# falcon-computing/bwa-flow

Hardware: AMD Instinct MI355X
Metric: million reads/sec (2×150 bp PE) end-to-end align; SW-extend GCUPS at 1/2/4/8 MI355X (higher is better)
Workload: dtype int32

## Files before the change

### bwa-flow_amd/csrc/capi.hip

```cpp
#include <hip/hip_runtime.h>
#include <string.h>

#include <algorithm>
#include <chrono>
#include <cstdio>
#include <mutex>
#include <new>
#include <string>
#include <thread>
#include <vector>

#include "batch_host.h"
#include "ctx.h"
#include "engine.h"
#include "regpost.h"

using namespace bwagpu;

namespace {


__global__ void side_probe_spin(uint64_t ticks) {
  const uint64_t t0 = __builtin_amdgcn_s_memrealtime();
  while (__builtin_amdgcn_s_memrealtime() - t0 < ticks) __builtin_amdgcn_s_sleep(8);
}
__global__ void side_probe_nop() {}

bool streams_concurrent(hipStream_t a, hipStream_t b) {
  hipEvent_t ea = nullptr, eb = nullptr;
  if (hipEventCreateWithFlags(&ea, hipEventDisableTiming) != hipSuccess) return false;
  if (hipEventCreateWithFlags(&eb, hipEventDisableTiming) != hipSuccess) {
    (void)hipEventDestroy(ea);
    return false;
  }
  hipLaunchKernelGGL(side_probe_spin, dim3(1), dim3(64), 0, a, (uint64_t)15000);
  bool conc = false;
  if (hipGetLastError() == hipSuccess && hipEventRecord(ea, a) == hipSuccess) {
    hipLaunchKernelGGL(side_probe_nop, dim3(1), dim3(64), 0, b);
    if (hipGetLastError() == hipSuccess && hipEventRecord(eb, b) == hipSuccess &&
        hipEventSynchronize(eb) == hipSuccess)
      conc = hipEventQuery(ea) == hipErrorNotReady;
  }
  (void)hipEventSynchronize(ea);
  (void)hipEventDestroy(ea);
  (void)hipEventDestroy(eb);
  return conc;
}

constexpr int kDenseScanBlock = 1024;
__global__ void __launch_bounds__(kDenseScanBlock) dense_scan_kernel(const int32_t* __restrict__ n, int nr,
                                                                     int32_t* __restrict__ off,
                                                                     int32_t* __restrict__ h_off) {
  __shared__ int32_t part[kDenseScanBlock];
  const int t = (int)threadIdx.x;
  const int per = (nr + kDenseScanBlock - 1) / kDenseScanBlock;
  const int r0 = min(t * per, nr), r1 = min(r0 + per, nr);
  int sum = 0;
  for (int r = r0; r < r1; ++r) sum += n[r];
  part[t] = sum;
  __syncthreads();
  for (int d = 1; d < kDenseScanBlock; d <<= 1) {
    const int v = t >= d ? part[t - d] : 0;
    __syncthreads();
    part[t] += v;
    __syncthreads();
  }
  int run = part[t] - sum;
  for (int r = r0; r < r1; ++r) {
    off[r] = run;
    h_off[r] = run;
    run += n[r];
  }
  if (t == kDenseScanBlock - 1) {
    off[nr] = part[t];
    h_off[nr] = part[t];
  }
}

__global__ void __launch_bounds__(256) dense_copy_kernel(const bwagpu_alnreg_t* __restrict__ out,
                                                         const int32_t* __restrict__ n,
                                                         const int32_t* __restrict__ off,
                                                         const int32_t* __restrict__ rco,
                                                         const int32_t* __restrict__ cso, int nr,
                                                         bwagpu_alnreg_t* __restrict__ dense) {
  constexpr int kW = (int)(sizeof(bwagpu_alnreg_t) / 8);
  const int r = (int)((blockIdx.x * 256u + threadIdx.x) >> 4), l = (int)(threadIdx.x & 15);
  if (r >= nr) return;
  const int words = n[r] * kW;
  const uint2* src = reinterpret_cast<const uint2*>(out + cso[rco[r]]);
  uint2* dst = reinterpret_cast<uint2*>(dense + off[r]);
  for (int w = l; w < words; w += 16) dst[w] = src[w];
}

}

namespace {

bool make_opt(const bwagpu_opt_t* o, DevOpt* d, std::string* why) {
  if (!o) { *why = "opt is NULL"; return false; }
  if (o->e_del <= 0 || o->e_ins <= 0) { *why = "gap extension penalties must be > 0"; return false; }
  if (o->w < 0 || o->a < 0) { *why = "negative band width or match score"; return false; }
  if (o->a > 127 || o->e_del > 65535 || o->e_ins > 65535 || o->o_del < 0 || o->o_del > 65535 || o->o_ins < 0 ||
      o->o_ins > 65535 || o->pen_clip5 < 0 || o->pen_clip5 >= (1 << 20) || o->pen_clip3 < 0 ||
      o->pen_clip3 >= (1 << 20) || o->w > (1 << 20)) {
    *why = "scoring option out of range";
    return false;
  }
  memset(d, 0, sizeof(*d));
  d->a = o->a;
  d->o_del = o->o_del;
  d->e_del = o->e_del;
  d->o_ins = o->o_ins;
  d->e_ins = o->e_ins;
  d->oe_del = o->o_del + o->e_del;
  d->oe_ins = o->o_ins + o->e_ins;
  d->pen_clip5 = o->pen_clip5;
  d->pen_clip3 = o->pen_clip3;
  d->w = o->w;
  d->zdrop = o->zdrop;
  int mx = 0;
  for (int i = 0; i < 25; ++i) mx = std::max<int>(mx, o->mat[i]);
  d->max_mat = mx;
  d->row_bound = 1;
  memcpy(d->mat, o->mat, 25);
  for (int q = 0; q < 5; ++q) {
    uint32_t w = 0;
    for (int t = 0; t < 4; ++t) w |= (uint32_t)(uint8_t)o->mat[t * 5 + q] << (8 * t);
    d->qprof[q] = w;
    d->qprof4[q] = o->mat[20 + q];
  }
  return true;
}

int create_common(int device, const bwagpu_opt_t* opt, const bwagpu_bns_t* bns, bwagpu_ctx_t** out,
                  bwagpu_ctx_t** made) {
  if (!out || !bns || bns->l_pac <= 0 || bns->n_seqs <= 0 || !bns->ann_offset || !bns->ann_len)
    return BWAGPU_E_INVAL;
  int n = 0;
  if (hipGetDeviceCount(&n) != hipSuccess || n <= 0) return BWAGPU_E_NODEVICE;
  if (device < 0 || device >= n) return BWAGPU_E_NODEVICE;
  bwagpu_ctx_t* ctx = new (std::nothrow) bwagpu_ctx_t();
  if (!ctx) return BWAGPU_E_NOMEM;
  std::string why;
  if (!make_opt(opt, &ctx->opt, &why)) {
    delete ctx;
    return BWAGPU_E_INVAL;
  }
  ctx->device = device;
  ctx->opt_b = opt->b;
  ctx->ext_form = set_ext_form(-1);
  ctx->ext_short = ext_short_default();
  ctx->ext_short_fill = ext_short_fill_default();
  ctx->light_pack = light_pack_default();
  ctx->ungapped = ungapped_default();
  ctx->emu_finish = emu_finish_default();
  *made = ctx;
  HIPC(hipSetDevice(device), "hipSetDevice");
  HIPC(hipMalloc(&ctx->d_ann_off, sizeof(int64_t) * bns->n_seqs), "hipMalloc(ann_offset)");
  HIPC(hipMalloc(&ctx->d_ann_len, sizeof(int32_t) * bns->n_seqs), "hipMalloc(ann_len)");
  HIPC(hipMemcpy(ctx->d_ann_off, bns->ann_offset, sizeof(int64_t) * bns->n_seqs, hipMemcpyHostToDevice),
       "upload ann_offset");
  HIPC(hipMemcpy(ctx->d_ann_len, bns->ann_len, sizeof(int32_t) * bns->n_seqs, hipMemcpyHostToDevice),
       "upload ann_len");
  for (auto& s : ctx->slot) {
    HIPC(hipEventCreate(&s.ev0), "hipEventCreate");
    HIPC(hipEventCreate(&s.ev1), "hipEventCreate");
    HIPC(hipEventCreate(&s.ev2), "hipEventCreate");
    HIPC(hipEventCreate(&s.ev3), "hipEventCreate");
  }
  ctx->ref.l_pac = bns->l_pac;
  ctx->ref.n_seqs = bns->n_seqs;
  ctx->ref.ann_offset = ctx->d_ann_off;
  ctx->ref.ann_len = ctx->d_ann_len;
  return BWAGPU_OK;
}

std::vector<Slot*> all_slots(bwagpu_ctx_t* ctx) {
  std::vector<Slot*> v;
  for (auto& x : ctx->slot) v.push_back(&x);
  for (auto& x : ctx->dev_scratch) v.push_back(&x);
  v.push_back(&ctx->ch_slot);
  return v;
}

void destroy_ctx(bwagpu_ctx_t* ctx) {
  if (!ctx) return;
  (void)hipSetDevice(ctx->device);
  std::vector<hipStream_t> busy = ctx->side_graveyard;
  for (Slot* s : all_slots(ctx)) busy.insert(busy.end(), {s->stream, s->spec.side});
  busy.insert(busy.end(), ctx->dev_stream, ctx->dev_stream + BWAGPU_NUM_SLOTS);
  busy.insert(busy.end(), ctx->a2_st, ctx->a2_st + bwagpu_ctx::kA2Streams);
  busy.insert(busy.end(), ctx->ch_cs.side, ctx->ch_cs.side + 2);
  for (hipStream_t x : busy)
    if (x) (void)hipStreamSynchronize(x);
  if (ctx->sdh_done) (void)hipEventSynchronize(ctx->sdh_done);
  if (ctx->r2d_done && ctx->r2d_pending) (void)hipEventSynchronize(ctx->r2d_done);
  std::vector<hipStream_t> own = ctx->side_graveyard;
  own.insert(own.end(), ctx->a2_st, ctx->a2_st + bwagpu_ctx::kA2Streams);
  own.insert(own.end(), ctx->ch_cs.side, ctx->ch_cs.side + 2);
  for (hipStream_t x : own)
    if (x) (void)hipStreamDestroy(x);
  std::vector<hipEvent_t> evs = ctx->prof_ev;
  evs.insert(evs.end(), {ctx->sdh_done, ctx->r2d_done, ctx->r2d_ev[0], ctx->r2d_ev[1], ctx->a2_fork, ctx->ch_cs.fork,
                         ctx->ch_cs.join[0], ctx->ch_cs.join[1]});
  evs.insert(evs.end(), ctx->a2_join, ctx->a2_join + bwagpu_ctx::kA2Streams);
  evs.insert(evs.end(), ctx->rs_ev, ctx->rs_ev + 4 * kRescueMaxRounds);
  for (hipEvent_t e : evs)
    if (e) (void)hipEventDestroy(e);
  if (ctx->own_pac && ctx->d_pac) (void)hipFree(ctx->d_pac);
  if (ctx->d_ann_off) (void)hipFree(ctx->d_ann_off);
  if (ctx->d_ann_len) (void)hipFree(ctx->d_ann_len);
  delete ctx;
}

bool use_read_kernels() {
  const char* e = getenv("BWAGPU_C2A_PATH");
  return e && (strcmp(e, "fast") == 0 || strcmp(e, "read") == 0);
}

size_t variant_lds(const DevOpt& o, int v, int lq_max) {
  const Variant& vk = kVariants[v];
  const int lqv = std::min(lq_max, vk.max_len());
  const int tb = tb_bytes_for(o, std::max(lqv, 1));
  return vk.kind == VK_FAST ? (size_t)(kBlock / 64) * fast_wave_lds(tb) : (size_t)tb * (kBlock / vk.G);
}

}

int bwagpu::check_lds(bwagpu_ctx_t* ctx, int lq_max) {
  if (!use_read_kernels()) {
    if (spec_redo_cap(tb_bytes_for(ctx->opt, std::max(lq_max, 1))) < 64)
      return fail(ctx, BWAGPU_E_UNSUPPORTED, "LDS row buffer too large for these options (w, pen_clip, read length)");
    return BWAGPU_OK;
  }
  for (int v = 0; v < kNumVariants; ++v) {
    if (variant_lds(ctx->opt, v, lq_max) > 64 * 1024)
      return fail(ctx, BWAGPU_E_UNSUPPORTED, "LDS row buffer too large for these options (w, pen_clip, read length)");
  }
  return BWAGPU_OK;
}

namespace {

void register_caller_locked(bwagpu_ctx_t* ctx, hipStream_t st) {
  for (hipStream_t c : ctx->callers)
    if (c == st) return;
  for (Slot* x : all_slots(ctx))
    if (x->side_chosen && x->spec.side && hipStreamSynchronize(x->spec.side) == hipSuccess &&
        !streams_concurrent(x->spec.side, st)) {
      ctx->side_graveyard.push_back(x->spec.side);
      x->spec.side = nullptr;
      x->side_chosen = false;
    }
  ctx->callers.push_back(st);
}

hipError_t choose_side(bwagpu_ctx_t* ctx, Slot& s, hipStream_t st, SpecStreams* snap) {
  std::lock_guard<std::mutex> g(ctx->side_mu);
  register_caller_locked(ctx, st);
  if (s.side_chosen) {
    *snap = s.spec;
    return hipSuccess;
  }
  if (!s.spec.fork) {
    hipError_t e = hipEventCreateWithFlags(&s.spec.fork, hipEventDisableTiming);
    if (e == hipSuccess) e = hipEventCreateWithFlags(&s.spec.join, hipEventDisableTiming);
    if (e != hipSuccess) return e;
  }
  std::vector<hipStream_t> avoid = ctx->callers;
  for (Slot* x : all_slots(ctx))
    if (x != &s && x->side_chosen && x->spec.side) avoid.push_back(x->spec.side);
  std::vector<hipStream_t> tried;
  hipStream_t pick = nullptr;
  hipError_t e = hipSuccess;
  for (int t = 0; t < 6 && !pick; ++t) {
    hipStream_t c = nullptr;
    if ((e = hipStreamCreateWithFlags(&c, hipStreamNonBlocking)) != hipSuccess) break;
    bool ok = true;
    for (hipStream_t a : avoid)
      if (!streams_concurrent(c, a)) {
        ok = false;
        break;
      }
    if (ok) pick = c;
    else tried.push_back(c);
  }
  for (hipStream_t c : tried) (void)hipStreamDestroy(c);
  if (e != hipSuccess) return e;
  s.spec.side = pick;
  s.side_chosen = true;
  *snap = s.spec;
  return hipSuccess;
}

int enqueue_spec(bwagpu_ctx_t* ctx, Slot& s, const DevBatch& db, int lq_max, bwagpu_alnreg_t* d_out, int32_t* d_n,
                 int64_t* d_stats, hipStream_t st) {
  const size_t nc = (size_t)std::max(db.n_chains, 1), ns = (size_t)std::max(db.n_seeds, 1),
               nr = (size_t)std::max(db.n_reads, 1);
  const size_t n_tasks = kSpecBins * (nc + (kSpecRounds - 1) * ns);
  SpecArgs a;
  HIPC(s.d_win.get(a.win, nc), "hipMalloc(win)");
  HIPC(s.d_cread.get(a.chain_read, nc), "hipMalloc(chain_read)");
  HIPC(s.d_prog.get(a.prog, ns), "hipMalloc(prog)");
  HIPC(s.d_ext.get(a.ext, ns), "hipMalloc(ext)");
  HIPC(s.d_tasks.get(a.tasks, n_tasks), "hipMalloc(tasks)");
  HIPC(s.d_ctr.get(a.ctr, SPC_WORDS), "hipMalloc(ctr)");
  HIPC(s.d_regpos.get(a.regpos, ns), "hipMalloc(regpos)");
  HIPC(s.d_skipf.get(a.skipf, ns), "hipMalloc(skipf)");
  HIPC(s.d_heavy.get(a.heavy, nr), "hipMalloc(heavy)");
  HIPC(s.d_redo.get(a.redo, nr), "hipMalloc(redo)");
  HIPC(s.d_rbits.get(a.rbits, 2 * (nr / 32 + 1)), "hipMalloc(rbits)");
  a.fbits = a.rbits + (nr / 32 + 1);
  HIPC(s.d_rlist.get(a.rlist, nr), "hipMalloc(rlist)");
  HIPC(s.d_desc.get(a.rdesc, nr), "hipMalloc(desc)");
  HIPC(s.d_schain.get(a.seedchain, ns), "hipMalloc(seedchain)");
  HIPC(s.d_hinfo.get(a.hinfo, nr), "hipMalloc(hinfo)");
  HIPC(s.d_cov.get(a.cov, ns), "hipMalloc(cov)");
  HIPC(s.d_hflag.get(a.hflag, ns), "hipMalloc(hflag)");
  HIPC(s.d_colent.get(a.colent, ns), "hipMalloc(colent)");
  HIPC(s.d_longc.get(a.longc, nc), "hipMalloc(longc)");
  HIPC(s.d_qh.get(a.qh, kQHWords), "hipMalloc(qh)");
  HIPC(s.d_sorth.get(a.sorth, kSortWords), "hipMalloc(sorth)");
  HIPC(s.d_stasks.get(a.stasks, n_tasks), "hipMalloc(stasks)");
  HIPC(s.d_ftask.get(a.ftask, n_tasks), "hipMalloc(ftask)");
  HIPC(s.d_ftaskR.get(a.ftaskR, n_tasks), "hipMalloc(ftaskR)");
  a.ung = nullptr;
  if (ctx->ungapped && ctx->opt.row_bound) HIPC(s.d_ung.get(a.ung, n_tasks), "hipMalloc(ung)");
  HIPC(s.d_mat.get(a.mat, (size_t)std::max<int64_t>(1 << 20, 16 * (int64_t)ns)), "hipMalloc(mat)");
  a.mat_words = (int64_t)(s.d_mat.cap / sizeof(uint64_t));
  static const int ext_prefetch = [] {
    const char* e = getenv("BWAGPU_EXT_PREFETCH");
    return e ? std::max(0, atoi(e)) : 0;
  }();
  a.ext_prefetch = ext_prefetch;
  static const int risky_first = [] {
    const char* e = getenv("BWAGPU_LIGHT_RISKY_FIRST");
    return e && e[0] == '1';
  }();
  a.risky_first = risky_first;
  static const int emu_strict = [] {
    const char* e = getenv("BWAGPU_EMU_STRICT");
    return !(e && e[0] == '0');
  }();
  a.emu_strict = emu_strict;
  a.light_pack = ctx->light_pack;
  a.emu_finish = ctx->emu_finish;
  a.out = d_out;
  a.out_n = d_n;
  a.stats = d_stats;
  SpecStreams ss;
  HIPC(choose_side(ctx, s, st, &ss), "side stream");
  a.lq_bound = lq_max;
  const int tb = tb_bytes_for(ctx->opt, std::max(lq_max, 1));
  ss.form = ctx->ext_form;
  ss.short_q = ctx->ext_short;
  ss.short_fill = ctx->ext_short_fill;
  ss.pool = ctx->prof_ev.empty() ? nullptr : ctx->prof_ev.data();
  ss.pool_n = (int)ctx->prof_ev.size();
  ss.pool_used = &ctx->prof_used;
  HIPC(launch_spec_clear(a, db.n_reads, db.n_seeds, st), "spec clear");
  HIPC(launch_spec_chain2aln(ctx->opt, ctx->ref, db, a, tb, lq_max, st, ss), "spec chain2aln launch");
  return BWAGPU_OK;
}

}

int bwagpu::enqueue_chain2aln(bwagpu_ctx_t* ctx, Slot& s, const DevBatch& db, int lq_max, bwagpu_alnreg_t* d_out,
                              int32_t* d_n, int64_t* d_stats, hipStream_t st) {
  if (!use_read_kernels()) return enqueue_spec(ctx, s, db, lq_max, d_out, d_n, d_stats, st);
  ChainWin* win = nullptr;
  bwagpu_seed_t* prog = nullptr;
  ReadDesc* desc = nullptr;
  C2AArgs a;
  HIPC(s.d_win.get(win, (size_t)db.n_chains), "hipMalloc(win)");
  HIPC(s.d_srt.get(a.srt, (size_t)db.n_seeds), "hipMalloc(srt)");
  HIPC(s.d_prog.get(prog, (size_t)db.n_seeds), "hipMalloc(prog)");
  const size_t nr = (size_t)std::max(db.n_reads, 1);
  HIPC(s.d_desc.get(desc, nr), "hipMalloc(desc)");
  HIPC(s.d_lists.ensure(2 * sizeof(int32_t) * nr), "hipMalloc(lists)");
  int32_t* bins = s.d_lists.as<int32_t>();
  int32_t* read_list = bins + nr;
  HIPC(s.d_counts.get(a.counts, kCountWords), "hipMalloc(counts)");
  HIPC(hipMemsetAsync(a.counts, 0, sizeof(int32_t) * kCountWords, st), "memset counts");
  if (db.n_reads) HIPC(hipMemsetAsync(d_n, 0, sizeof(int32_t) * db.n_reads, st), "memset out_n");
  HIPC(launch_chain_prep(ctx->opt, ctx->ref, db, win, a.srt, prog, d_stats, st), "chain_prep launch");
  HIPC(launch_read_order(db, bins, a.counts + kHistOff, a.counts, desc, read_list, d_stats, st), "read order launch");
  a.read_list = read_list;
  a.desc = desc;
  a.win = win;
  a.prog = prog;
  a.out = d_out;
  a.out_n = d_n;
  a.stats = d_stats;
  for (int v = 0; v < kNumVariants; ++v) {
    const int lqv = std::min(lq_max, kVariants[v].max_len());
    const int tb = tb_bytes_for(ctx->opt, std::max(lqv, 1));
    HIPC(launch_chain2aln(v, ctx->opt, ctx->ref, db, db.n_reads, tb, a, st), "chain2aln launch");
  }
  return BWAGPU_OK;
}

extern "C" {

int bwagpu_abi_version(void) { return BWAGPU_ABI_VERSION; }

int bwagpu_device_count(int* n) {
  if (!n) return BWAGPU_E_INVAL;
  int k = 0;
  if (hipGetDeviceCount(&k) != hipSuccess) k = 0;
  *n = k;
  return k > 0 ? BWAGPU_OK : BWAGPU_E_NODEVICE;
}

int bwagpu_create(int device, const bwagpu_opt_t* opt, const bwagpu_bns_t* bns, const uint8_t* pac_host,
                  bwagpu_ctx_t** out) {
  if (!pac_host) return BWAGPU_E_INVAL;
  bwagpu_ctx_t* ctx = nullptr;
  int rc = create_common(device, opt, bns, out, &ctx);
  if (rc == BWAGPU_OK) {
    const size_t pac_bytes = (size_t)(bns->l_pac / 4 + 1);
    hipError_t e = hipMalloc(&ctx->d_pac, pac_bytes);
    if (e == hipSuccess) {
      ctx->own_pac = true;
      e = hipMemcpy(ctx->d_pac, pac_host, pac_bytes, hipMemcpyHostToDevice);
    }
    if (e != hipSuccess) rc = hip_fail(ctx, e, "pac upload");
    ctx->ref.pac = (const uint8_t*)ctx->d_pac;
  }
  if (rc != BWAGPU_OK) {
    destroy_ctx(ctx);
    return rc;
  }
  *out = ctx;
  return BWAGPU_OK;
}

int bwagpu_create_resident(int device, const bwagpu_opt_t* opt, const bwagpu_bns_t* bns, const void* pac_device,
                           bwagpu_ctx_t** out) {
  if (!pac_device) return BWAGPU_E_INVAL;
  bwagpu_ctx_t* ctx = nullptr;
  int rc = create_common(device, opt, bns, out, &ctx);
  if (rc != BWAGPU_OK) {
    destroy_ctx(ctx);
    return rc;
  }
  ctx->d_pac = (void*)pac_device;
  ctx->own_pac = false;
  ctx->ref.pac = (const uint8_t*)pac_device;
  *out = ctx;
  return BWAGPU_OK;
}

int bwagpu_destroy(bwagpu_ctx_t* ctx) {
  if (!ctx) return BWAGPU_E_INVAL;
  destroy_ctx(ctx);
  return BWAGPU_OK;
}

const char* bwagpu_last_error(const bwagpu_ctx_t* ctx) { return ctx ? ctx->err.c_str() : "NULL context"; }

int bwagpu_set_watchdog_ms(bwagpu_ctx_t* ctx, int ms) {
  if (!ctx || ms < 0) return BWAGPU_E_INVAL;
  ctx->watchdog_ms = ms;
  return BWAGPU_OK;
}

namespace {
void expand_slots(const Slot& s, bwagpu_alnreg_t* dst) {
  const char* h = s.h_in.as<const char>();
  const int32_t* rco = s.kept ? s.keep_rco.data() : (const int32_t*)(h + s.in_rco);
  const int32_t* cso = s.kept ? s.keep_cso.data() : (const int32_t*)(h + s.in_cso);
  const int32_t* n = s.h_n.as<const int32_t>();
  const int32_t* off = s.h_off.as<const int32_t>();
  const bwagpu_alnreg_t* src = s.h_dense.as<const bwagpu_alnreg_t>();
  for (int32_t r = 0; r < s.n_reads; ++r)
    if (n[r]) memcpy(dst + cso[rco[r]], src + off[r], sizeof(bwagpu_alnreg_t) * (size_t)n[r]);
}
}

int bwagpu_chain2aln_submit(bwagpu_ctx_t* ctx, int slot, const bwagpu_batch_t* b) {
// ... 127 lines not shown
  const int64_t* st = s.h_stats.as<int64_t>();
  float k_ms = 0, t_ms = 0;
  (void)hipEventElapsedTime(&k_ms, s.ev1, s.ev2);
  (void)hipEventElapsedTime(&t_ms, s.ev0, s.ev3);
  s.last.kernel_ms = k_ms;
  s.last.total_ms = t_ms;
  s.last.cells = st[ST_CELLS];
  s.last.rows = st[ST_ROWS];
  s.last.ext_calls = st[ST_CALLS];
  const int32_t* off = s.h_off.as<int32_t>();
  s.d2h = (int64_t)sizeof(bwagpu_alnreg_t) * off[s.n_reads] + (int64_t)sizeof(int32_t) * (2 * (int64_t)s.n_reads + 1);
  s.last.h2d_bytes = s.h2d;
  s.last.d2h_bytes = s.d2h;
  if (st[ST_ERR] & ERR_LEN) return fail(ctx, BWAGPU_E_UNSUPPORTED, "read longer than BWAGPU_MAX_READ_LEN");
  if (out_n && s.n_reads) memcpy(out_n, s.h_n.p, sizeof(int32_t) * (size_t)s.n_reads);
  if (out_regs && s.n_seeds) expand_slots(s, out_regs);
  if (st[ST_ERR] & ERR_POST) return fail(ctx, BWAGPU_E_UNSUPPORTED, "a patch candidate's window exceeds 4096 bases");
  if (st[ST_ERR] & ERR_RID)
    return fail(ctx, BWAGPU_E_RESULTS, "a chain's first seed is not inside contig chain_rid (bwamem.c:669 assert)");
  return BWAGPU_OK;
}

int bwagpu_chain2aln_stage(bwagpu_ctx_t* ctx, int slot, int32_t n_reads, int32_t n_chains, int32_t n_seeds,
                           int64_t seq_bytes, bwagpu_batch_t* view) {
  if (!ctx || slot < 0 || slot >= BWAGPU_NUM_SLOTS || !view || n_reads < 0 || n_chains < 0 || n_seeds < 0 ||
      seq_bytes < 0)
    return BWAGPU_E_INVAL;
  Slot& s = ctx->slot[slot];
  if (s.busy) return fail(ctx, BWAGPU_E_INVAL, "slot already has a batch in flight");
  bwagpu_batch_t b{};
  b.n_reads = n_reads;
  b.n_chains = n_chains;
  b.n_seeds = n_seeds;
  b.seq_bytes = seq_bytes;
  InLayout L;
  L.make(b);
  HIPC(hipSetDevice(ctx->device), "hipSetDevice");
  if (s.has_results && !s.slot_view && !s.kept && s.n_reads) {
    const char* hp = s.h_in.as<const char>();
    const int32_t* rco = (const int32_t*)(hp + s.in_rco);
    s.keep_rco.assign(rco, rco + s.n_reads + 1);
    const int32_t* cso = (const int32_t*)(hp + s.in_cso);
    s.keep_cso.assign(cso, cso + s.n_chains + 1);
    s.kept = true;
  }
  HIPC(s.h_in.ensure(L.total), "hipHostMalloc(in)");
  char* h = s.h_in.as<char>();
  b.seq_off = (const int64_t*)(h + L.seq_off);
  b.seq = (const uint8_t*)(h + L.seq);
  b.read_chain_off = (const int32_t*)(h + L.rco);
  b.chain_seed_off = (const int32_t*)(h + L.cso);
  b.chain_rid = (const int32_t*)(h + L.rid);
  b.chain_frac_rep = (const float*)(h + L.frac);
  b.seeds = (const bwagpu_seed_t*)(h + L.seeds);
  *view = b;
  return BWAGPU_OK;
}

int bwagpu_chain2aln_results(bwagpu_ctx_t* ctx, int slot, const bwagpu_alnreg_t** regs, const int32_t** n) {
  if (!ctx || slot < 0 || slot >= BWAGPU_NUM_SLOTS || !regs || !n) return BWAGPU_E_INVAL;
  Slot& s = ctx->slot[slot];
  if (s.busy) return fail(ctx, BWAGPU_E_INVAL, "slot's batch still in flight (wait first)");
  if (!s.has_results) return fail(ctx, BWAGPU_E_INVAL, "slot has no results");
  if (!s.slot_view) {
    bwagpu_alnreg_t* h_out = nullptr;
    HIPC(s.h_out.get(h_out, (size_t)s.n_seeds), "hipHostMalloc(out)");
    if (s.n_seeds) expand_slots(s, h_out);
    s.slot_view = true;
  }
  *regs = s.h_out.as<const bwagpu_alnreg_t>();
  *n = s.h_n.as<const int32_t>();
  return BWAGPU_OK;
}

int bwagpu_chain2aln_results_dense(bwagpu_ctx_t* ctx, int slot, const bwagpu_alnreg_t** regs, const int32_t** n,
                                   const int32_t** off) {
  if (!ctx || slot < 0 || slot >= BWAGPU_NUM_SLOTS || !regs || !n || !off) return BWAGPU_E_INVAL;
  Slot& s = ctx->slot[slot];
  if (s.busy) return fail(ctx, BWAGPU_E_INVAL, "slot's batch still in flight (wait first)");
  if (!s.has_results || !s.h_dense.p || !s.h_off.p) return fail(ctx, BWAGPU_E_INVAL, "slot has no results");
  *regs = s.h_dense.as<const bwagpu_alnreg_t>();
  *n = s.h_n.as<const int32_t>();
  *off = s.h_off.as<const int32_t>();
  return BWAGPU_OK;
}

int bwagpu_chain2aln(bwagpu_ctx_t* ctx, const bwagpu_batch_t* b, bwagpu_alnreg_t* out_regs, int32_t* out_n) {
  int rc = bwagpu_chain2aln_submit(ctx, 0, b);
  if (rc) return rc;
  return bwagpu_chain2aln_wait(ctx, 0, out_regs, out_n);
}

int bwagpu_chain2aln_device(bwagpu_ctx_t* ctx, const bwagpu_batch_t* db_in, bwagpu_alnreg_t* dev_out,
                            int32_t* dev_n, int64_t* dev_stats, void* stream) {
  if (!ctx || !db_in || !dev_out || !dev_n) return BWAGPU_E_INVAL;
  HIPC(hipSetDevice(ctx->device), "hipSetDevice");
  const int lq_bound = use_read_kernels() ? BWAGPU_MAX_READ_LEN : ctx->dev_read_len;
  int rc = check_lds(ctx, lq_bound);
  if (rc) return rc;
  hipStream_t st = (hipStream_t)stream;
  if (!st) HIPC(lazy_stream(ctx->slot[0], &st), "hipStreamCreate");
  int k = 0;
  while (k < BWAGPU_NUM_SLOTS && ctx->dev_stream[k] && ctx->dev_stream[k] != st) ++k;
  if (k == BWAGPU_NUM_SLOTS) return fail(ctx, BWAGPU_E_INVAL, "more than BWAGPU_NUM_SLOTS streams on one context");
  ctx->dev_stream[k] = st;
  Slot& s = ctx->dev_scratch[k];
  DevBatch db;
  db.n_reads = db_in->n_reads;
  db.n_chains = db_in->n_chains;
  db.n_seeds = db_in->n_seeds;
  db.seq_off = db_in->seq_off;
  db.seq = db_in->seq;
  db.read_chain_off = db_in->read_chain_off;
  db.chain_seed_off = db_in->chain_seed_off;
  db.chain_rid = db_in->chain_rid;
  db.chain_frac_rep = db_in->chain_frac_rep;
  db.seeds = db_in->seeds;
  int64_t* stats = dev_stats;
  if (!stats) {
    HIPC(s.d_stats.get(stats, ST_N), "hipMalloc(stats)");
    HIPC(hipMemsetAsync(stats, 0, sizeof(int64_t) * ST_N, st), "memset stats");
  }
  return enqueue_chain2aln(ctx, s, db, lq_bound, dev_out, dev_n, stats, st);
}

int bwagpu_set_device_read_len(bwagpu_ctx_t* ctx, int32_t max_len) {
  if (!ctx || max_len < 1 || max_len > BWAGPU_MAX_READ_LEN) return BWAGPU_E_INVAL;
  ctx->dev_read_len = max_len;
  return BWAGPU_OK;
}

int bwagpu_debug_set_trace(bwagpu_ctx_t* ctx, void* dev_ptr) {
  if (!ctx) return BWAGPU_E_INVAL;
  HIPC(hipSetDevice(ctx->device), "hipSetDevice");
  HIPC(set_trace(dev_ptr), "set trace");
  HIPC(set_trace_spec(dev_ptr), "set trace");
  return BWAGPU_OK;
}

int bwagpu_debug_fail_wait(bwagpu_ctx_t* ctx, int after_n_waits, int code) {
  if (!ctx || code <= 0) return BWAGPU_E_INVAL;
  ctx->fail_after = after_n_waits;
  ctx->fail_code = code;
  return BWAGPU_OK;
}

int bwagpu_debug_live_buffers(int64_t* n, int64_t* bytes) {
  if (!n || !bytes) return BWAGPU_E_INVAL;
  *n = g_live_bufs.load(std::memory_order_relaxed);
  *bytes = g_live_bytes.load(std::memory_order_relaxed);
  return BWAGPU_OK;
}

int bwagpu_debug_occupancy(bwagpu_ctx_t* ctx, void* stream, int64_t* out) {
  if (!ctx || !out) return BWAGPU_E_INVAL;
  hipStream_t st = nullptr;
  if (int rc = entry_stream(ctx, stream, &st)) return rc;
  int k = 0;
  while (k < BWAGPU_NUM_SLOTS && ctx->dev_stream[k] != st) ++k;
  if (k == BWAGPU_NUM_SLOTS || !ctx->dev_scratch[k].d_ctr.p) return fail(ctx, BWAGPU_E_INVAL, "no device-entry batch on this stream");
  HIPC(hipStreamSynchronize(st), "hipStreamSynchronize");
  int32_t c[SPC_WORDS];
  HIPC(hipMemcpy(c, ctx->dev_scratch[k].d_ctr.p, sizeof c, hipMemcpyDeviceToHost), "hipMemcpy(ctr)");
  memcpy(out, c + 32, 14 * sizeof(int64_t));
#ifdef BWAGPU_OCC_DIAG
  return BWAGPU_OK;
#else
  return fail(ctx, BWAGPU_E_UNSUPPORTED, "built without BWAGPU_OCC_DIAG");
#endif
}

int bwagpu_debug_spec_counters(bwagpu_ctx_t* ctx, void* stream, int64_t* out) {
  if (!ctx || !out) return BWAGPU_E_INVAL;
  hipStream_t st = nullptr;
  if (int rc = entry_stream(ctx, stream, &st)) return rc;
  int k = 0;
  while (k < BWAGPU_NUM_SLOTS && ctx->dev_stream[k] != st) ++k;
  if (k == BWAGPU_NUM_SLOTS || !ctx->dev_scratch[k].d_ctr.p) return fail(ctx, BWAGPU_E_INVAL, "no device-entry batch on this stream");
  HIPC(hipStreamSynchronize(st), "hipStreamSynchronize");
  int32_t c[SPC_WORDS];
  HIPC(hipMemcpy(c, ctx->dev_scratch[k].d_ctr.p, sizeof c, hipMemcpyDeviceToHost), "hipMemcpy(ctr)");
  for (int r = 0; r < kSpecRounds; ++r) {
    out[r] = 0;
    for (int b = 0; b < kSpecBins; ++b) out[r] += c[SPC_CNT + r * kSpecBins + b];
  }
  int64_t spec = 0;
  memcpy(&spec, c + SPC_SPEC64, 8);
  out[3] = spec;
  out[4] = c[SPC_MISS];
  out[5] = c[SPC_HEAVY_N];
  out[6] = c[SPC_REDO_N];
  out[7] = c[SPC_HCOLS];
  return BWAGPU_OK;
}

int bwagpu_debug_spec_ext(bwagpu_ctx_t* ctx, void* stream, void* host_out, int32_t n) {
  if (!ctx || !host_out || n < 0) return BWAGPU_E_INVAL;
  hipStream_t st = nullptr;
  if (int rc = entry_stream(ctx, stream, &st)) return rc;
  int k = 0;
  while (k < BWAGPU_NUM_SLOTS && ctx->dev_stream[k] != st) ++k;
  if (k == BWAGPU_NUM_SLOTS || !ctx->dev_scratch[k].d_ext.p || ctx->dev_scratch[k].d_ext.cap < sizeof(SeedExt) * (size_t)n)
    return fail(ctx, BWAGPU_E_INVAL, "no device-entry batch of that size on this stream");
  HIPC(hipStreamSynchronize(st), "hipStreamSynchronize");
  HIPC(hipMemcpy(host_out, ctx->dev_scratch[k].d_ext.p, sizeof(SeedExt) * (size_t)n, hipMemcpyDeviceToHost),
       "hipMemcpy(ext)");
  return BWAGPU_OK;
}

int bwagpu_debug_ext_form(int form) { return set_ext_form(form); }

int bwagpu_streams_concurrent(void* a, void* b) {
  if (!a || !b || a == b) return BWAGPU_E_INVAL;
  return streams_concurrent((hipStream_t)a, (hipStream_t)b) ? 1 : 0;
}

int bwagpu_ctx_ext_form(bwagpu_ctx_t* ctx, int form) {
  if (!ctx) return BWAGPU_E_INVAL;
  const int prev = ctx->ext_form;
  if (form >= 0) ctx->ext_form = form > 2 ? 1 : form;
  return prev;
}

int bwagpu_ctx_ext_short(bwagpu_ctx_t* ctx, int q) {
  if (!ctx) return BWAGPU_E_INVAL;
  const int prev = ctx->ext_short;
  if (q >= 0) ctx->ext_short = q > 63 ? 63 : q;
  return prev;
}

int bwagpu_ctx_ext_short_fill(bwagpu_ctx_t* ctx, int percent) {
  if (!ctx) return BWAGPU_E_INVAL;
  const int prev = ctx->ext_short_fill;
  if (percent >= 0) ctx->ext_short_fill = percent > 100000 ? 100000 : percent;
  return prev;
}

int bwagpu_ctx_light_pack(bwagpu_ctx_t* ctx, int on) {
  if (!ctx) return BWAGPU_E_INVAL;
  const int prev = ctx->light_pack;
  if (on >= 0) ctx->light_pack = on != 0;
  return prev;
}

int bwagpu_debug_spec_short(bwagpu_ctx_t* ctx, void* stream, int64_t* out) {
  if (!ctx || !out) return BWAGPU_E_INVAL;
  hipStream_t st = nullptr;
  if (int rc = entry_stream(ctx, stream, &st)) return rc;
  int k = 0;
  while (k < BWAGPU_NUM_SLOTS && ctx->dev_stream[k] != st) ++k;
  if (k == BWAGPU_NUM_SLOTS || !ctx->dev_scratch[k].d_ctr.p) return fail(ctx, BWAGPU_E_INVAL, "no device-entry batch on this stream");
  HIPC(hipStreamSynchronize(st), "hipStreamSynchronize");
  int32_t c[SPC_WORDS];
  HIPC(hipMemcpy(c, ctx->dev_scratch[k].d_ctr.p, sizeof c, hipMemcpyDeviceToHost), "hipMemcpy(ctr)");
  out[0] = c[SPC_SHORT_N];
  for (int r = 0; r < 2; ++r) {
    const int l = r * kSpecBins;
    out[1 + 4 * r] = c[SPC_LCNT + l];
    out[2 + 4 * r] = c[SPC_LLONG + l];
    out[3 + 4 * r] = c[SPC_RCNT + l];
    out[4 + 4 * r] = c[SPC_RLONG + l];
  }
  return BWAGPU_OK;
}

int bwagpu_ctx_ungapped(bwagpu_ctx_t* ctx, int on) {
  if (!ctx) return BWAGPU_E_INVAL;
  const int prev = ctx->ungapped;
  if (on >= 0) ctx->ungapped = on ? 1 : 0;
  return prev;
}

int bwagpu_debug_spec_ungapped(bwagpu_ctx_t* ctx, void* stream, int64_t* out) {
  if (!ctx || !out) return BWAGPU_E_INVAL;
  hipStream_t st = nullptr;
  if (int rc = entry_stream(ctx, stream, &st)) return rc;
  int k = 0;
  while (k < BWAGPU_NUM_SLOTS && ctx->dev_stream[k] != st) ++k;
  if (k == BWAGPU_NUM_SLOTS || !ctx->dev_scratch[k].d_ctr.p) return fail(ctx, BWAGPU_E_INVAL, "no device-entry batch on this stream");
  HIPC(hipStreamSynchronize(st), "hipStreamSynchronize");
  int32_t c[SPC_WORDS];
  HIPC(hipMemcpy(c, ctx->dev_scratch[k].d_ctr.p, sizeof c, hipMemcpyDeviceToHost), "hipMemcpy(ctr)");
  for (int r = 0; r < kSpecRounds; ++r) {
    out[4 * r + 0] = c[SPC_UNG_N + r];
    out[4 * r + 1] = c[SPC_UNG_Q + r];
    out[4 * r + 2] = out[4 * r + 3] = 0;
    for (int bin = 0; bin < kSpecBins; ++bin) {
      out[4 * r + 2] += c[SPC_LCNT + r * kSpecBins + bin];
      out[4 * r + 3] += c[SPC_RCNT + r * kSpecBins + bin];
    }
  }
  return BWAGPU_OK;
}

int bwagpu_ctx_emu_finish(bwagpu_ctx_t* ctx, int on) {
  if (!ctx) return BWAGPU_E_INVAL;
  const int prev = ctx->emu_finish;
  if (on >= 0) ctx->emu_finish = on ? 1 : 0;
  return prev;
}

int bwagpu_debug_spec_finish(bwagpu_ctx_t* ctx, void* stream, int64_t* out) {
  if (!ctx || !out) return BWAGPU_E_INVAL;
  hipStream_t st = nullptr;
  if (int rc = entry_stream(ctx, stream, &st)) return rc;
  int k = 0;
  while (k < BWAGPU_NUM_SLOTS && ctx->dev_stream[k] != st) ++k;
  if (k == BWAGPU_NUM_SLOTS || !ctx->dev_scratch[k].d_ctr.p) return fail(ctx, BWAGPU_E_INVAL, "no device-entry batch on this stream");
  HIPC(hipStreamSynchronize(st), "hipStreamSynchronize");
  int32_t c[SPC_WORDS];
  HIPC(hipMemcpy(c, ctx->dev_scratch[k].d_ctr.p, sizeof c, hipMemcpyDeviceToHost), "hipMemcpy(ctr)");
  out[0] = c[SPC_FIN_NAR];
  out[1] = c[SPC_FIN_WIDE];
  out[2] = c[SPC_LIST_N];
  out[3] = c[SPC_LIGHT_N];
  return BWAGPU_OK;
}

int bwagpu_ctx_row_bound(bwagpu_ctx_t* ctx, int on) {
  if (!ctx) return BWAGPU_E_INVAL;
  const int prev = ctx->opt.row_bound;
  if (on >= 0) ctx->opt.row_bound = on ? 1 : 0;
  return prev;
}

int bwagpu_debug_ext_kernel(bwagpu_ctx_t* ctx, int32_t lq_max) {
  if (!ctx || lq_max < 1 || lq_max > BWAGPU_MAX_READ_LEN) return BWAGPU_E_INVAL;
  return ext_kernel_for(ctx->opt, ctx->ext_form, tb_bytes_for(ctx->opt, lq_max));
}

int bwagpu_prof_start(bwagpu_ctx_t* ctx, int max_launches) {
  if (!ctx || max_launches < 0) return BWAGPU_E_INVAL;
  HIPC(hipSetDevice(ctx->device), "hipSetDevice");
  for (hipEvent_t e : ctx->prof_ev) HIPC(hipEventSynchronize(e), "hipEventSynchronize");
  for (hipEvent_t e : ctx->prof_ev) (void)hipEventDestroy(e);
  ctx->prof_ev.clear();
  ctx->prof_used = 0;
  for (int i = 0; i < 2 * max_launches; ++i) {
    hipEvent_t e = nullptr;
    HIPC(hipEventCreate(&e), "hipEventCreate");
    ctx->prof_ev.push_back(e);
  }
  return BWAGPU_OK;
}

int bwagpu_prof_read(bwagpu_ctx_t* ctx, double* total_ms, int32_t* launches) {
  if (!ctx || !total_ms || !launches) return BWAGPU_E_INVAL;
  HIPC(hipSetDevice(ctx->device), "hipSetDevice");
  double t = 0;
  for (int i = 0; i + 1 < ctx->prof_used; i += 2) {
    HIPC(hipEventSynchronize(ctx->prof_ev[i + 1]), "hipEventSynchronize");
    float ms = 0;
    HIPC(hipEventElapsedTime(&ms, ctx->prof_ev[i], ctx->prof_ev[i + 1]), "hipEventElapsedTime");
    t += ms;
  }
  *total_ms = t;
  *launches = ctx->prof_used / 2;
  return BWAGPU_OK;
}

int bwagpu_prof_intervals(bwagpu_ctx_t* ctx, double* start_ms, double* end_ms, int32_t max, int32_t* n) {
  if (!ctx || !n || max < 0 || (max && (!start_ms || !end_ms))) return BWAGPU_E_INVAL;
  HIPC(hipSetDevice(ctx->device), "hipSetDevice");
  int k = 0;
  for (int i = 0; i + 1 < ctx->prof_used && k < max; i += 2, ++k) {
    HIPC(hipEventSynchronize(ctx->prof_ev[i + 1]), "hipEventSynchronize");
    float a = 0, b = 0;
    HIPC(hipEventElapsedTime(&a, ctx->prof_ev[0], ctx->prof_ev[i]), "hipEventElapsedTime");
    HIPC(hipEventElapsedTime(&b, ctx->prof_ev[0], ctx->prof_ev[i + 1]), "hipEventElapsedTime");
    start_ms[k] = a;
    end_ms[k] = b;
  }
  *n = k;
  return BWAGPU_OK;
}

int bwagpu_last_stats(const bwagpu_ctx_t* ctx, int slot, bwagpu_stats_t* out) {
  if (!ctx || !out || slot < 0 || slot >= BWAGPU_NUM_SLOTS) return BWAGPU_E_INVAL;
  *out = ctx->slot[slot].last;
  return BWAGPU_OK;
}

}
```

### bwa-flow_amd/csrc/ctx.h

```cpp
#pragma once
#include <hip/hip_runtime.h>
#include <stdint.h>

#include <algorithm>
#include <atomic>
#include <chrono>
#include <mutex>
#include <string>
#include <type_traits>
#include <vector>

#include "bwagpu.h"
#include "chain.h"
#include "engine.h"
#include "rescue.h"
#include "seed.h"
#include "stage_host.h"
#include "task_host.h"

namespace bwagpu {

inline std::atomic<int64_t> g_live_bufs{0}, g_live_bytes{0};

template <bool kPinned>
struct GrowBuf {
  void* p = nullptr;
  size_t cap = 0;
  GrowBuf() = default;
  GrowBuf(const GrowBuf&) = delete;
  GrowBuf& operator=(const GrowBuf&) = delete;
  ~GrowBuf() { release(); }
  hipError_t ensure(size_t n) {
    if (n <= cap) return hipSuccess;
    release();
    const size_t want = std::max<size_t>(n + n / 4, 4096);
    const hipError_t e = kPinned ? hipHostMalloc(&p, want, hipHostMallocDefault) : hipMalloc(&p, want);
    if (e != hipSuccess) {
      p = nullptr;
      return e;
    }
    cap = want;
    g_live_bufs.fetch_add(1, std::memory_order_relaxed);
    g_live_bytes.fetch_add((int64_t)want, std::memory_order_relaxed);
    return e;
  }
  template <class T>
  hipError_t get(T*& out, size_t n) {
    const hipError_t e = ensure(sizeof(T) * std::max<size_t>(n, 1));
    out = e == hipSuccess ? (T*)p : nullptr;
    return e;
  }
  void release() {
    if (p) {
      (void)(kPinned ? hipHostFree(p) : hipFree(p));
      g_live_bufs.fetch_sub(1, std::memory_order_relaxed);
      g_live_bytes.fetch_sub((int64_t)cap, std::memory_order_relaxed);
    }
    p = nullptr;
    cap = 0;
  }
  template <class T>
  T* as() const { return (T*)p; }
};
using DevBuf = GrowBuf<false>;
using HostBuf = GrowBuf<true>;
static_assert(!std::is_copy_constructible<DevBuf>::value, "a copy would free the buffer twice");

struct Slot {
  hipStream_t stream = nullptr;
  std::once_flag stream_once;
  hipError_t stream_err = hipSuccess;
  hipEvent_t ev0 = nullptr, ev1 = nullptr, ev2 = nullptr, ev3 = nullptr;
  DevBuf d_in, d_win, d_srt, d_prog, d_desc, d_out, d_n, d_stats, d_lists, d_counts;
  DevBuf d_cread, d_ext, d_tasks, d_ctr, d_regpos, d_skipf, d_heavy, d_redo, d_rbits, d_rlist;
  DevBuf d_schain, d_hinfo, d_mat, d_cov, d_hflag, d_colent, d_qh, d_longc, d_sorth, d_stasks, d_ftask, d_ftaskR, d_ung;
  SpecStreams spec;
  bool side_chosen = false;
  HostBuf h_in, h_out, h_n, h_stats;
  HostBuf h_dense, h_off;
  DevBuf d_off;
  size_t in_rco = 0, in_cso = 0;
  bool slot_view = false;
  bool busy = false;
  bool has_results = false;
  bool kept = false;
  std::vector<int32_t> keep_rco, keep_cso;
  int32_t n_reads = 0, n_chains = 0, n_seeds = 0;
  std::chrono::steady_clock::time_point t_submit;
  bwagpu_stats_t last{};
  int64_t h2d = 0, d2h = 0;
  ~Slot() {
    for (hipStream_t x : {stream, spec.side})
      if (x) {
        (void)hipStreamSynchronize(x);
        (void)hipStreamDestroy(x);
      }
    for (hipEvent_t e : {ev0, ev1, ev2, ev3, spec.fork, spec.join})
      if (e) (void)hipEventDestroy(e);
  }
};

inline hipError_t lazy_stream(Slot& s, hipStream_t* st) {
  std::call_once(s.stream_once, [&s] { s.stream_err = hipStreamCreateWithFlags(&s.stream, hipStreamNonBlocking); });
  *st = s.stream;
  return s.stream_err;
}

struct Staging {
  DevBuf regs, out_regs;
  DevBuf seq;
  DevBuf seq_off, reg_off, out_off;
  DevBuf n, out_n, n_pri, status, n_sw, mapq, sel;
  DevBuf pes;
};

}

struct bwagpu_ctx {
  using DevBuf = bwagpu::DevBuf;
  using HostBuf = bwagpu::HostBuf;
  using Slot = bwagpu::Slot;
  int device = 0;
  std::mutex side_mu;
  std::vector<hipStream_t> callers, side_graveyard;
  bwagpu::DevOpt opt{};
  bwagpu::DevRef ref{};
  bool own_pac = false;
  void* d_pac = nullptr;
  int64_t* d_ann_off = nullptr;
  int32_t* d_ann_len = nullptr;
  int watchdog_ms = 10000;
  int ext_form = 0;
  int ext_short = 0;
  int light_pack = 0;
  int ext_short_fill = 0;
  int ungapped = 1;
  int emu_finish = 1;
  Slot slot[BWAGPU_NUM_SLOTS];
  hipStream_t dev_stream[BWAGPU_NUM_SLOTS] = {};
  Slot dev_scratch[BWAGPU_NUM_SLOTS];
  DevBuf ex_tasks, ex_list, ex_q, ex_t, ex_res, ex_stats;
  DevBuf a2_tasks, a2_q, a2_t, a2_out, a2_scratch, a2_lists, a2_counts, a2_boff;
  DevBuf r2_tasks, r2_q, r2_out, r2_cig, r2_md, r2_lists, r2_z, r2_stats;
  DevBuf r2d_keys, r2d_lists, r2d_tab, r2d_z, r2d_sums;
  HostBuf r2d_htab;
  hipEvent_t r2d_done = nullptr, r2d_ev[2] = {};
  bool r2d_pending = false, r2d_timing = false, r2d_timed = false;
  double r2d_wait_ms = 0, r2d_call_ms = 0;
  int32_t r2d_jobs = 0;
  static constexpr int kA2Streams = 4;
  hipStream_t a2_st[kA2Streams] = {};
  hipEvent_t a2_fork = nullptr, a2_join[kA2Streams] = {};
  DevBuf bwt_words, sa_d, sa_in, sa_out, occ_d, sup_d, sa_full;
  bwagpu::DevBwt bwt{};
  bool has_bwt = false;
  DevBuf sd_off, sd_seq, sd_out, sd_n, sd_scratch, sd_poff, sd_pack, sd_heavy, sd_dbg;
  DevBuf ch_npos, ch_posoff, ch_frac, ch_nout, ch_noseed, ch_nsw, ch_need, ch_swtab, ch_alt;
  DevBuf ch_kpos, ch_rbeg, ch_qinfo, ch_label, ch_score, ch_slist, ch_ord, ch_chains, ch_nodes;
  DevBuf ch_ochains, ch_oslist, ch_bins, ch_dbg;
  DevBuf ch_swoff, ch_swtasks, ch_swt, ch_swskip, ch_swres, ch_swscr;
  DevBuf ch_ocoff, ch_osoff, ch_rco, ch_cso, ch_rid, ch_cfrac, ch_out, ch_seeds;
  DevBuf ch_regoff, ch_regc;
  HostBuf chh_tot, chh_rco, chh_cso, chh_chains, chh_seeds, chh_regs, chh_n;
  HostBuf sdh_in;
  hipEvent_t sdh_done = nullptr;
  Slot ch_slot;
  bwagpu::ChainStreams ch_cs{};
  bool has_alt = false;
  bwagpu::Staging stg;
  int opt_b = 0;
  bwagpu_postopt_t post_opt{};
  int32_t post_flags = 0;
  int64_t post_id0 = 0;
  DevBuf rp_stats;
  DevBuf pe_isize, pe_cnt;
  DevBuf rs_pair, rs_soff, rs_tab, rs_toff, rs_boff, rs_qpool, rs_ctr, rs_scr;
  DevBuf rs_tasks[bwagpu::kRescueMaxRounds], rs_tpool[bwagpu::kRescueMaxRounds], rs_res[bwagpu::kRescueMaxRounds];
  int32_t rescue_drop = 0;
  hipEvent_t rs_ev[4 * bwagpu::kRescueMaxRounds] = {};
  int rs_ev_rounds = 0;
  hipStream_t rs_ev_stream = nullptr;
  DevBuf ps_scratch, ps_log, ps_erfc;
  bool ps_log_ready = false;
  DevBuf st_buf, st_start, st_q, st_tasks, st_lists, st_seen, st_ctr, st_out;
  int seed_budget = 1024;
  int sup_shift = 32;
  int dev_read_len = BWAGPU_MAX_READ_LEN;
  int fail_after = -1, fail_code = 0;
  std::vector<hipEvent_t> prof_ev;
  int prof_used = 0;
  std::string err;
};

namespace bwagpu {

inline int fail(bwagpu_ctx_t* c, int code, const std::string& msg) {
  if (c) c->err = msg;
  return code;
}

inline int hip_fail(bwagpu_ctx_t* c, hipError_t e, const char* what) {
  std::string m = std::string(what) + ": " + hipGetErrorString(e);
  if (e == hipErrorOutOfMemory || e == hipErrorMemoryAllocation) return fail(c, BWAGPU_E_NOMEM, m);
  return fail(c, BWAGPU_E_DEVICE, m);
}

#define HIPC(call, what)                             \
  do {                                               \
    hipError_t e_ = (call);                          \
    if (e_ != hipSuccess) return hip_fail(ctx, e_, what); \
  } while (0)
#define TRY(call)                     \
  do {                                \
    if (int rc_ = (call)) return rc_; \
  } while (0)

inline int refuse(bwagpu_ctx_t* c, int code, const char* why) { return why && *why ? fail(c, code, why) : code; }

inline int entry_stream(bwagpu_ctx_t* ctx, void* stream, hipStream_t* st) {
  HIPC(hipSetDevice(ctx->device), "hipSetDevice");
  *st = (hipStream_t)stream;
  if (!*st) HIPC(lazy_stream(ctx->slot[0], st), "hipStreamCreate");
  return BWAGPU_OK;
}

inline int side_fork(bwagpu_ctx_t* ctx, hipStream_t st, size_t n_launches, int* used) {
  for (int i = 0; i < bwagpu_ctx::kA2Streams; ++i) {
    if (!ctx->a2_st[i]) HIPC(hipStreamCreateWithFlags(&ctx->a2_st[i], hipStreamNonBlocking), "stream");
    if (!ctx->a2_join[i]) HIPC(hipEventCreateWithFlags(&ctx->a2_join[i], hipEventDisableTiming), "event");
  }
  if (!ctx->a2_fork) HIPC(hipEventCreateWithFlags(&ctx->a2_fork, hipEventDisableTiming), "event");
  *used = (int)std::min<size_t>(bwagpu_ctx::kA2Streams, n_launches);
  HIPC(hipEventRecord(ctx->a2_fork, st), "event");
  for (int i = 0; i < *used; ++i) HIPC(hipStreamWaitEvent(ctx->a2_st[i], ctx->a2_fork, 0), "stream wait");
  return BWAGPU_OK;
}
inline int side_join(bwagpu_ctx_t* ctx, hipStream_t st, int used) {
  for (int i = 0; i < used; ++i) {
    HIPC(hipEventRecord(ctx->a2_join[i], ctx->a2_st[i]), "event");
    HIPC(hipStreamWaitEvent(st, ctx->a2_join[i], 0), "stream wait");
  }
  return BWAGPU_OK;
}

struct EventPair {
  hipEvent_t e0 = nullptr, e1 = nullptr;
  EventPair() = default;
  EventPair(const EventPair&) = delete;
  EventPair& operator=(const EventPair&) = delete;
  ~EventPair() {
    if (e0) (void)hipEventDestroy(e0);
    if (e1) (void)hipEventDestroy(e1);
  }
  hipError_t start(hipStream_t st) {
    hipError_t e = hipEventCreate(&e0);
    if (e == hipSuccess) e = hipEventCreate(&e1);
    return e == hipSuccess ? hipEventRecord(e0, st) : e;
  }
  hipError_t stop(hipStream_t st) { return hipEventRecord(e1, st); }
  float ms() const {
    float t = 0;
    (void)hipEventElapsedTime(&t, e0, e1);
    return t;
  }
};

int enqueue_regpost(bwagpu_ctx_t* ctx, const bwagpu_postopt_t& po, int32_t flags, int64_t id0, int32_t n_reads,
                    const int64_t* seq_off, const uint8_t* seq, const int64_t* reg_off, const int32_t* rco,
                    const int32_t* cso, bwagpu_alnreg_t* regs, int32_t* n, int64_t* stats, hipStream_t st);

int check_lds(bwagpu_ctx_t* ctx, int lq_max);
int enqueue_chain2aln(bwagpu_ctx_t* ctx, Slot& s, const DevBatch& db, int lq_max, bwagpu_alnreg_t* d_out,
                      int32_t* d_n, int64_t* d_stats, hipStream_t st);

struct HostCall {
  bwagpu_ctx_t* ctx;
  Staging& g;
  hipStream_t st = nullptr;
  EventPair ev;
  int64_t h2d = 0, d2h = 0, hs[ST_N] = {};
  std::vector<int64_t> roff, soff, ooff;
  bool open = false;

  explicit HostCall(bwagpu_ctx_t* c) : ctx(c), g(c->stg) {}
  HostCall(const HostCall&) = delete;
  HostCall& operator=(const HostCall&) = delete;
  ~HostCall() {
    if (open) (void)hipStreamSynchronize(st);
  }
// ... 61 lines not shown
```

### bwa-flow_amd/csrc/engine.h

```cpp
#pragma once
#include <hip/hip_runtime.h>
#include <stdint.h>

#include "bwagpu.h"
#include "bwagpu_debug.h"
#include "pure.h"
#include "spec_plan.h"
#include "ungapped.h"

namespace bwagpu {

struct ReadDesc {
  int64_t qoff;
  int32_t rd;
  int32_t lq;
  int32_t c0;
  int32_t nch;
  int32_t s0;
  int32_t ns;
};

struct ChainWin {
  int64_t lo, hi;
};

struct DevBatch {
  int32_t n_reads, n_chains, n_seeds;
  const int64_t* seq_off;
  const uint8_t* seq;
  const int32_t* read_chain_off;
  const int32_t* chain_seed_off;
  const int32_t* chain_rid;
  const float* chain_frac_rep;
  const bwagpu_seed_t* seeds;
};

struct DevRef {
  int64_t l_pac;
  int32_t n_seqs;
  const uint8_t* pac;
  const int64_t* ann_offset;
  const int32_t* ann_len;
};

enum { ST_CELLS = 0, ST_ROWS = 1, ST_CALLS = 2, ST_ERR = 3, ST_N = 4 };
enum { ERR_RID = 1, ERR_LEN = 2, ERR_A2_RANGE = 4 };

constexpr int kFastMaxSeeds = 32;
constexpr int kFastMaxChains = 32;
constexpr int kSeqLds = 256;
constexpr int kNumVariants = 3;
extern const Variant kVariants[kNumVariants];
constexpr int kHistOff = 128;
constexpr int kCountWords = kHistOff + kNumVariants * 256;

hipError_t launch_chain_prep(const DevOpt& o, const DevRef& ref, const DevBatch& b, ChainWin* win, uint64_t* srt,
                             bwagpu_seed_t* prog, int64_t* stats, hipStream_t st);
hipError_t launch_read_order(const DevBatch& b, int32_t* bins, int32_t* hist, int32_t* counts, ReadDesc* desc,
                             int32_t* list, int64_t* stats, hipStream_t st);
struct C2AArgs {
  const int32_t* read_list;
  const ReadDesc* desc;
  int32_t* counts;
  const ChainWin* win;
  uint64_t* srt;
  const bwagpu_seed_t* prog;
  bwagpu_alnreg_t* out;
  int32_t* out_n;
  int64_t* stats;
};
hipError_t launch_chain2aln(int variant, const DevOpt& o, const DevRef& ref, const DevBatch& b, int32_t max_list,
                            int tb_bytes, const C2AArgs& a, hipStream_t st);
size_t fast_wave_lds(int tb);

hipError_t launch_extend(int variant, bool t5, const DevOpt& o, int32_t n_tasks,
                         const bwagpu_ext_task_t* tasks, const int32_t* task_list, int32_t n_list,
                         const uint8_t* qpool, const uint8_t* tpool, int tb_bytes,
                         bwagpu_ext_result_t* res, int64_t* stats, hipStream_t st);
hipError_t launch_extend4(const DevOpt& o, const bwagpu_ext_task_t* tasks, const int32_t* task_list, int32_t n_list,
                          const uint8_t* qpool, const uint8_t* tpool, int tb_bytes, bwagpu_ext_result_t* res,
                          int64_t* stats, hipStream_t st);

struct SeedExt {
  int64_t rb, re;
  int32_t qb, qe, score, truesc, w;
  int32_t cells, rows, calls;
};

constexpr int kSpecRounds = 3;
constexpr int kOrderLane = 8;
constexpr int kSelLight = 64;
constexpr int kSelRegLds = 256;
constexpr int kSelMatMaxSeeds = 4096;
enum {
  SPC_CNT = 0,
  SPC_HEAVY_N = 16,
  SPC_SEL_CUR = 17,
  SPC_REDO_N = 20,
  SPC_SPEC64 = 24,
  SPC_MISS = 26,
  SPC_MATW64 = 28,
  SPC_HCOLS = 30,
  SPC_LONG_N = 31,
  SPC_LCNT = 64,
  SPC_RCNT = 73,
  SPC_LIGHT_CUR = 82,
  SPC_LLONG = 84,
  SPC_RLONG = 93,
  SPC_SHORT_N = 102,
  SPC_UNG_N = 103,
  SPC_UNG_Q = 106,
  SPC_FIN_NAR = 109,
  SPC_FIN_WIDE = 110,
  SPC_LIST_N = 111,
  SPC_LIGHT_N = 112,
  SPC_WORDS = 128
};
constexpr int kQHStride = 32;
constexpr int kQHShort = 2 * kSpecRounds * kSpecBins * 8 * kQHStride;
constexpr int kQHWords = 2 * kQHShort;
constexpr int kSortKeys = 1024;
constexpr int kSortWordsR = kSpecRounds * 2 * kSortKeys;
constexpr int kSortWords = 2 * kSortWordsR;
__host__ __device__ inline size_t spec_list_off(int list, int n_chains, int n_seeds) {
  const int round = list / kSpecBins, bin = list % kSpecBins;
  return round == 0 ? (size_t)bin * n_chains
                    : (size_t)kSpecBins * n_chains + ((size_t)(round - 1) * kSpecBins + bin) * n_seeds;
}
struct FatTask {
  int64_t rbeg, qoff;
  int32_t pos;
  int32_t dlo, dhi;
  uint32_t qls;
};
static_assert(sizeof(FatTask) == 32, "FatTask layout");
static_assert(BWAGPU_MAX_READ_LEN < 1024, "FatTask packs qbeg / len / lq in 10 bits each");
struct UngRec {
  struct Side {
    int32_t ok;
    UngappedSide s;
  } side[2];
};
static_assert(sizeof(UngRec) == 32, "UngRec layout");
struct SpecArgs {
  int lq_bound;
  ChainWin* win;
  int32_t* chain_read;
  bwagpu_seed_t* prog;
  SeedExt* ext;
  int2* tasks;
  int32_t* ctr;
  int32_t* regpos;
  int32_t* skipf;
  int32_t* heavy;
  int32_t* redo;
  uint32_t* rbits;
  uint32_t* fbits;
  int32_t* rlist;
  ReadDesc* rdesc;
  int32_t* seedchain;
  int4* hinfo;
  int32_t* colent;
  int32_t* longc;
  uint64_t* mat;
  int64_t mat_words;
  int32_t* cov;
  int32_t* hflag;
  int32_t* qh;
  int32_t* sorth;
  int2* stasks;
  FatTask* ftask;
  FatTask* ftaskR;
  UngRec* ung;
  int risky_first;
  int emu_strict;
  int light_pack;
  int emu_finish;
  int ext_prefetch;
  bwagpu_alnreg_t* out;
  int32_t* out_n;
  int64_t* stats;
};
struct SpecStreams {
  hipStream_t side = nullptr;
  hipEvent_t fork = nullptr, join = nullptr;
  hipEvent_t* pool = nullptr;
  int pool_n = 0;
  int* pool_used = nullptr;
  int form = 0;
  int short_q = 0;
  int short_fill = 0;
};
int ungapped_default();
int emu_finish_default();
int set_ext_form(int form);
int ext_short_default();
int ext_short_fill_default();
int light_pack_default();
int ext_kernel_for(const DevOpt& o, int form, int tb_bytes);
hipError_t launch_spec_clear(const SpecArgs& a, int n_reads, int n_seeds, hipStream_t st);
hipError_t launch_spec_chain2aln(const DevOpt& o, const DevRef& ref, const DevBatch& b, const SpecArgs& a,
                                 int tb_bytes, int lq_max, hipStream_t st, const SpecStreams& ss);
size_t spec_select_lds(int tb_bytes);
int spec_redo_cap(int tb_bytes);

struct StreamTask {
  bwagpu_seed_t s;
  int64_t lo, hi;
  int64_t qoff;
  int32_t lq, pad_;
};
enum { STR_ERR_RECORD = 1, STR_ERR_TASK = 2, STR_ERR_DUP = 4, STR_ERR_SEED = 8, STR_ERR_BASE = 16 };
enum { kStrDecoded = 4, kStrMax = 5, kStrErr = 6, kStrHeads = 64 };
constexpr int kStrCtrWords = kStrHeads + kSpecBins * 8 * kQHStride;
struct StreamArgs {
  const int32_t* buf;
  const int64_t* rstart;
  int32_t n_reads, cap;
  int64_t l_pac;
  uint8_t* qpool;
  StreamTask* tasks;
  int32_t* lists;
  int32_t* seen;
  int32_t* ctr;
  int32_t* out;
};
hipError_t launch_sw_stream(const DevOpt& o, const DevRef& ref, const StreamArgs& a, int tb_bytes, hipStream_t st);

hipError_t set_trace(void* dev_ptr);
hipError_t set_trace_spec(void* dev_ptr);

}
```

### bwa-flow_amd/csrc/spec.hip

```cpp
#include "spec_dev.h"

namespace bwagpu {

__device__ uint32_t* g_trace = nullptr;
hipError_t set_trace_spec(void* p) { return hipMemcpyToSymbol(HIP_SYMBOL(g_trace), &p, sizeof(p)); }


__global__ void __launch_bounds__(256) spec_chain_kernel(DevOpt o, DevRef ref, DevBatch b, SpecArgs a) {
  sel_prio();
  const int c = blockIdx.x * blockDim.x + threadIdx.x;
  bool task = false, longc = false;
  int bin = 0, s0 = 0;
  if (c < b.n_chains) {
    const int rd = a.chain_read[c];
    s0 = b.chain_seed_off[c];
    const int ns = b.chain_seed_off[c + 1] - s0;
    const int lq = (int)(b.seq_off[rd + 1] - b.seq_off[rd]);
    if (ns <= 0) {
      a.win[c] = ChainWin{0, 0};
    } else {
      int64_t wlo = ref.l_pac << 1, whi = 0;
      longc = ns > kOrderLane;
      if (!longc) {
        uint64_t key[kOrderLane];
// ... 1908 lines not shown
          const uint64_t pw = lane64(pend_w, w);
          const int j = 64 * w + r;
          if ((pw >> r) & 1)
            a.tasks[spec_list_off(list, b.n_chains, b.n_seeds) + off + (int)__popcll(pw & lt_mask)] =
                make_int2(d.s0 + j, a.seedchain[d.s0 + j]);
          off += (int)__popcll(pw);
        }
      }
    } else {
      if (miss >= 0) {
        if (r == 0) {
          const int list = 2 * kSpecBins + spec_bin(d.lq);
          const int p = atomicAdd(&a.ctr[SPC_CNT + list], 1);
          a.tasks[spec_list_off(list, b.n_chains, b.n_seeds) + p] = make_int2(d.s0 + miss, a.seedchain[d.s0 + miss]);
          a.redo[atomicAdd(&a.ctr[SPC_REDO_N], 1)] = rd;
        }
        continue;
      }
      for (int w = 0; w < nw; ++w) {
        const uint64_t ew = (uint64_t)__builtin_amdgcn_readlane((uint32_t)(ext_w >> 32), w) << 32 |
                            (uint32_t)__builtin_amdgcn_readlane((uint32_t)ext_w, w);
        const int j = 64 * w + r;
        if ((ew >> r) & 1) {
          const int slot = nreg + (int)__popcll(ew & lt_mask);
          const SeedExt x = a.ext[d.s0 + j];
          const int c = a.seedchain[d.s0 + j];
          uint2* dst = reinterpret_cast<uint2*>(a.out + d.s0 + slot);
          dst[0] = make_uint2((uint32_t)x.rb, (uint32_t)((uint64_t)x.rb >> 32));
          dst[1] = make_uint2((uint32_t)x.re, (uint32_t)((uint64_t)x.re >> 32));
          dst[2] = make_uint2((uint32_t)x.qb, (uint32_t)x.qe);
          dst[3] = make_uint2((uint32_t)b.chain_rid[c], (uint32_t)x.score);
          dst[4] = make_uint2((uint32_t)x.truesc, 0u);
          dst[5] = make_uint2(0u, 0u);
          dst[6] = make_uint2(0u, (uint32_t)x.w);
          dst[7] = make_uint2((uint32_t)a.cov[d.s0 + j], 0u);
          dst[8] = make_uint2(0u, (uint32_t)a.prog[d.s0 + j].len);
          dst[9] = make_uint2(0u, __float_as_uint(b.chain_frac_rep[c]));
          dst[10] = make_uint2(0u, 0u);
          tl.cells += x.cells;
          tl.rows += x.rows;
          tl.calls += x.calls - 1;
        }
        nreg += (int)__popcll(ew);
      }
      if (r == 0) a.out_n[rd] = nreg;
    }
    trace_read(MODE, b.n_reads, rd, t_start, ns, nreg, 3);
  }
  if constexpr (WRITE) block_stats<64>(tl, a.stats);
}

constexpr int kScanGrid = 1024;

#ifndef BWAGPU_LIGHT_PACK_DEFAULT
#define BWAGPU_LIGHT_PACK_DEFAULT 1
#endif
int light_pack_default() {
  static const int v = [] {
    const char* e = getenv("BWAGPU_LIGHT_PACK");
    return e && e[0] ? (atoi(e) != 0 ? 1 : 0) : BWAGPU_LIGHT_PACK_DEFAULT;
  }();
  return v;
}
#ifndef BWAGPU_LIGHT_PACK_WGS_DEFAULT
#define BWAGPU_LIGHT_PACK_WGS_DEFAULT 2
#endif
static int light_pack_wgs() {
  static const int v = [] {
    const char* e = getenv("BWAGPU_LIGHT_PACK_WGS");
    return std::min(std::max(e && e[0] ? atoi(e) : BWAGPU_LIGHT_PACK_WGS_DEFAULT, 1), 64);
  }();
  return v;
}
#ifndef BWAGPU_LIGHT_LIST_DIV_DEFAULT
#define BWAGPU_LIGHT_LIST_DIV_DEFAULT 4
#endif
static int light_list_div() {
  static const int v = [] {
    const char* e = getenv("BWAGPU_LIGHT_LIST_DIV");
    return std::min(std::max(e && e[0] ? atoi(e) : BWAGPU_LIGHT_LIST_DIV_DEFAULT, 1), 64);
  }();
  return v;
}
static int device_cus() {
  int dev = 0, ncu = 0;
  if (hipGetDevice(&dev) != hipSuccess ||
      hipDeviceGetAttribute(&ncu, hipDeviceAttributeMultiprocessorCount, dev) != hipSuccess || ncu < 1)
    return 256;
  return ncu;
}

template <int MODE>
static void launch_select(const DevOpt& o, const DevRef& ref, const DevBatch& b, const SpecArgs& a, int tb_bytes,
                          hipStream_t st, const SpecStreams& ss) {
  hipStream_t hs = st;
  if (MODE != SEL_REDO && ss.side) {
    (void)hipEventRecord(ss.fork, st);
    (void)hipStreamWaitEvent(ss.side, ss.fork, 0);
    hs = ss.side;
  }
  if (MODE != SEL_REDO) {
    const size_t lds = BWAGPU_LIGHT_INLINE && MODE == SEL_FINAL ? (size_t)(kBlock / 64) * 2 * tb_bytes : 0;
    int nb = resident_blocks(spec_select_light<MODE>, lds);
    if (a.light_pack && !(MODE == SEL_FINAL && a.risky_first)) {
      const int octets = (b.n_reads + kPackW - 1) / kPackW, per_wg = kBlock / 64;
      nb = std::min(nb, std::max(1, std::min((octets + per_wg - 1) / per_wg, light_pack_wgs() * device_cus())));
      if (MODE == SEL_FINAL && a.emu_finish) nb = std::max(1, nb / light_list_div());
    }
    hipLaunchKernelGGL((spec_select_light<MODE>), dim3(nb), dim3(kBlock), lds, st, o, ref, b, a, tb_bytes);
  }
  if (MODE != SEL_REDO) {
    const int nb = resident_blocks(spec_pairs_kernel<MODE>, 0);
    hipLaunchKernelGGL((spec_pairs_kernel<MODE>), dim3(nb), dim3(kBlock), 0, hs, o, b, a);
    hipLaunchKernelGGL((spec_scan_kernel<MODE>), dim3(kScanGrid), dim3(64), (size_t)kScanLds + 2 * (size_t)tb_bytes, hs, o,
                       ref, b, a, tb_bytes);
  }
  hipLaunchKernelGGL((spec_select_kernel<MODE, true>), dim3(MODE == SEL_REDO ? 256 : 1024), dim3(64),
                     (size_t)kSelHeavyLds, hs, o, ref, b, a, tb_bytes);
  if (hs != st) {
    (void)hipEventRecord(ss.join, hs);
    (void)hipStreamWaitEvent(st, ss.join, 0);
  }
}

static std::atomic<int> g_ext_form{0};
int ext_kernel_for(const DevOpt& o, int form, int tb_bytes) { return ext_plan(o, form, tb_bytes, 0).bin[0].code; }
int set_ext_form(int form) {
  const int prev = g_ext_form.load(std::memory_order_relaxed);
  if (form >= 0) g_ext_form.store(form > 2 ? 1 : form, std::memory_order_relaxed);
  return prev;
}

#ifndef BWAGPU_EXT_SHORT_Q_DEFAULT
#define BWAGPU_EXT_SHORT_Q_DEFAULT 63
#endif
int ext_short_default() {
  static const int q = [] {
    const char* e = getenv("BWAGPU_EXT_SHORT_Q");
    const int v = e && e[0] ? atoi(e) : BWAGPU_EXT_SHORT_Q_DEFAULT;
    return std::min(std::max(v, 0), kShortQMax);
  }();
  return q;
}
#ifndef BWAGPU_EXT_SHORT_FILL_DEFAULT
#define BWAGPU_EXT_SHORT_FILL_DEFAULT 150
#endif
int ungapped_default() {
  static const int on = [] {
    const char* e = getenv("BWAGPU_UNGAPPED");
    return !(e && e[0] == '0');
  }();
  return on;
}
int emu_finish_default() {
  static const int on = [] {
    const char* e = getenv("BWAGPU_EMU_FINISH");
    return !(e && e[0] == '0');
  }();
  return on;
}
int ext_short_fill_default() {
  static const int f = [] {
    const char* e = getenv("BWAGPU_EXT_SHORT_FILL");
    return std::min(std::max(e && e[0] ? atoi(e) : BWAGPU_EXT_SHORT_FILL_DEFAULT, 0), 100000);
  }();
  return f;
}


static void launch_sort(const ExtBin& k, const ExtRound& r, int bin0, int nbins, int short_q, int short_fill) {
  if (k.phased) launch_side_sort(r, bin0, nbins, short_q, short_fill);
  else launch_task_sort(r, bin0, nbins);
}
static void launch_ext_bin(const ExtBin& k, const ExtRound& r, int list, const ExtPlan& p, int short_fill) {
  if (k.family == SIDE4) launch_side_bin(k, r, list, p, short_fill);
  else launch_task_bin(k, r, list, p.quad);
}

static void launch_ext_round(const DevOpt& o, const DevRef& ref, const DevBatch& b, const SpecArgs& a, int round,
                             int tb_bytes, int lq_max, hipStream_t st, const SpecStreams& ss) {
  const int l = round * kSpecBins;
  const bool bin1 = lq_max > kSpecBinLen[0], bin2 = lq_max > kSpecBinLen[1];
  const ExtPlan plan = ext_plan(o, ss.form, tb_bytes, ss.short_q);
  const ExtRound r{o, ref, b, a, round, tb_bytes, st};
  if (!bin1 || plan.bin[0].phased == plan.bin[1].phased) {
    launch_sort(plan.bin[0], r, 0, bin1 ? 2 : 1, plan.short_q, ss.short_fill);
  } else {
    launch_sort(plan.bin[0], r, 0, 1, plan.short_q, ss.short_fill);
    launch_sort(plan.bin[1], r, 1, 1, 0, ss.short_fill);
  }
  const bool prof = ss.pool && *ss.pool_used + 2 <= ss.pool_n;
  if (prof) (void)hipEventRecord(ss.pool[*ss.pool_used], st);
  launch_ext_bin(plan.bin[0], r, l + 0, plan, ss.short_fill);
  if (prof) {
    (void)hipEventRecord(ss.pool[*ss.pool_used + 1], st);
    *ss.pool_used += 2;
  }
  if (!bin1) return;
  launch_ext_bin(plan.bin[1], r, l + 1, plan, ss.short_fill);
  if (bin2) launch_task_long(r, l + 2);
}

hipError_t launch_spec_chain2aln(const DevOpt& o, const DevRef& ref, const DevBatch& b, const SpecArgs& a,
                                 int tb_bytes, int lq_max, hipStream_t st, const SpecStreams& ss) {
  if (b.n_reads == 0) return hipSuccess;
  hipLaunchKernelGGL(spec_reads_kernel, dim3((b.n_reads + 255) / 256), dim3(256), 0, st, b, a);
  if (b.n_chains) {
    hipLaunchKernelGGL(spec_chain_kernel, dim3((b.n_chains + 255) / 256), dim3(256), 0, st, o, ref, b, a);
    hipLaunchKernelGGL(spec_order_kernel, dim3(kOrderBlocks), dim3(256), 0, st, o, ref, b, a);
  }
  if (b.n_chains) {
    launch_ext_round(o, ref, b, a, 0, tb_bytes, lq_max, st, ss);
    launch_select<SEL_EMULATE>(o, ref, b, a, tb_bytes, st, ss);
    launch_ext_round(o, ref, b, a, 1, tb_bytes, lq_max, st, ss);
  }
  SpecArgs af = a;
  if (!b.n_chains) af.emu_finish = 0;
  launch_select<SEL_FINAL>(o, ref, b, af, tb_bytes, st, ss);
  if (b.n_chains && lq_max > kSpecBinLen[0] && !a.emu_strict) launch_ext_round(o, ref, b, a, 2, tb_bytes, lq_max, st, ss);
  if (b.n_chains) launch_select<SEL_REDO>(o, ref, b, a, tb_bytes, st, ss);
  return hipGetLastError();
}

__global__ void __launch_bounds__(256) spec_clear_kernel(SpecArgs a, int nr, int ns) {
  const int t0 = (int)(blockIdx.x * 256 + threadIdx.x), nt = (int)(gridDim.x * 256);
  switch (blockIdx.y) {
    case 0:
      for (int i = t0; i < 3 * ns; i += nt) reinterpret_cast<uint4*>(a.ext)[i] = make_uint4(0, 0, 0, 0);
      break;
    case 1:
      for (int i = t0; i < nr; i += nt) a.out_n[i] = 0;
      break;
    case 2:
      for (int i = t0; i < nr / 32 + 1; i += nt) a.rbits[i] = a.fbits[i] = 0;
      break;
    case 3:
      for (int i = t0; i < kQHWords; i += nt) a.qh[i] = 0;
      break;
    case 4:
      for (int i = t0; i < kSortWords; i += nt) a.sorth[i] = 0;
      break;
    default:
      for (int i = t0; i < SPC_WORDS; i += nt) a.ctr[i] = 0;
  }
}
static_assert(sizeof(SeedExt) == 48, "spec_clear_kernel clears SeedExt as three uint4");

hipError_t launch_spec_clear(const SpecArgs& a, int n_reads, int n_seeds, hipStream_t st) {
  hipLaunchKernelGGL(spec_clear_kernel, dim3(256, 6), dim3(256), 0, st, a, n_reads, n_seeds);
  return hipGetLastError();
}

size_t spec_select_lds(int tb_bytes) { return (size_t)kSelHeavyLds + 0 * tb_bytes; }
int spec_redo_cap(int tb_bytes) { return sel_heavy_cap(SEL_REDO, tb_bytes); }

}
```

### bwa-flow_amd/csrc/spec_side.hip

```cpp
#include "spec_dev.h"

namespace bwagpu {

__device__ __forceinline__ int side_key(int qlen) { return 255 - min(qlen, 255); }


struct UngSide {
  const uint8_t* rd;
  int64_t x0;
  int p0, d, qlen, lq;
};
struct UngPass {
  uint64_t qw[2], tw;
  int64_t fa, b0;
  int base, last, ws;
  bool fast, rev;
};
__device__ __forceinline__ UngPass ung_load(const UngSide& s, const DevRef& ref, int base) {
  UngPass p;
  p.base = base;
  p.last = min(base + 15, s.qlen - 1);
  p.fast = false;
  if (base >= s.qlen) return p;
  const int64_t two1 = (ref.l_pac << 1) - 1, pac_bytes = (ref.l_pac >> 2) + 1;
  const int64_t xa = s.x0 + (int64_t)s.d * base, xb = s.x0 + (int64_t)s.d * p.last;
  p.rev = xa >= ref.l_pac;
  p.fa = p.rev ? two1 - xa : xa;
  const int64_t fb = p.rev ? two1 - xb : xb;
  p.fast = s.lq >= 16 && pac_bytes >= 8 && (xb >= ref.l_pac) == p.rev;
  if (p.fast) {
    p.ws = min(max(min(s.p0 + s.d * base, s.p0 + s.d * (base + 15)), 0), s.lq - 16);
    p.b0 = min(min(p.fa, fb) >> 2, pac_bytes - 8);
    __builtin_memcpy(p.qw, s.rd + p.ws, 16);
    __builtin_memcpy(&p.tw, ref.pac + p.b0, 8);
  }
  return p;
}
__device__ __forceinline__ void ung_eat(const UngSide& s, const DevRef& ref, const UngPass& p, const int8_t* mat,
                                        int max_mat, UngappedScan& sc) {
  if (p.base >= s.qlen) return;
  if (p.fast) {
#pragma unroll
    for (int m = 0; m < 16; ++m)
      if (p.base + m <= p.last) {
        const int k = s.p0 + s.d * (p.base + m) - p.ws;
        const int qv = (int)(p.qw[k >> 3] >> ((k & 7) * 8)) & 255;
        const int64_t fm = p.fa + (p.rev ? -s.d : s.d) * m;
        const int byte = (int)(p.tw >> (((fm >> 2) - p.b0) * 8)) & 255;
        const int bse = (byte >> ((~fm & 3) << 1)) & 3;
        sc.step(p.base + m, mat[(p.rev ? 3 - bse : bse) * 5 + min(qv, 4)], max_mat);
      }
  } else {
    for (int j = p.base; j <= p.last; ++j)
      sc.step(j, mat[pac_base2(ref.pac, ref.l_pac, s.x0 + (int64_t)s.d * j) * 5 + min((int)s.rd[s.p0 + s.d * j], 4)],
              max_mat);
  }
}

__global__ void __launch_bounds__(256) spec_ungapped_kernel(DevOpt o, DevRef ref, DevBatch b, SpecArgs a, int round,
                                                            int bin0, int keep_short) {
  sel_prio();
  __shared__ int8_t mat[25];
  if (threadIdx.x < 25) mat[threadIdx.x] = o.mat[threadIdx.x];
  __syncthreads();
  const int bin = bin0 + (int)blockIdx.y;
  const int list = round * kSpecBins + bin;
  const int n = __hip_atomic_load(&a.ctr[SPC_CNT + list], __ATOMIC_RELAXED, __HIP_MEMORY_SCOPE_AGENT);
  const size_t off = spec_list_off(list, b.n_chains, b.n_seeds);
  const int2* tl = a.tasks + off;
  const int oe_min = ungapped_oe_min(o.o_del, o.e_del, o.o_ins, o.e_ins);
  const int keep = bin == 0 ? keep_short : 0;
  const int chunk = (n + (int)gridDim.x - 1) / (int)gridDim.x;
  const int i0 = (int)blockIdx.x * chunk, i1 = min(n, i0 + chunk);
  for (int k = 2 * i0 + (int)threadIdx.x; k < 2 * i1; k += 256) {
    const int i = k >> 1, right = k & 1;
    const FatTask f = fat_task(b, a, tl[i]);
    const int qb = (int)(f.qls & 1023u), ln = (int)((f.qls >> 10) & 1023u), lq = (int)(f.qls >> 20);
    const int64_t xr = f.rbeg + ln;
    const int qlen = right ? lq - qb - ln : qb;
    const int tlen = right ? (int)(f.rbeg + f.dhi - xr) : f.dlo;
    UngRec::Side rec{0, {0, 0, 0}};
    if (qlen > keep && ungapped_band_ok(o.w) &&
        ungapped_call_ok(qlen, tlen, ln * o.a, o.w, o.zdrop, o.max_mat, oe_min)) {
      UngSide sd;
      sd.rd = b.seq + f.qoff;
      sd.p0 = right ? qb + ln : qb - 1;
      sd.d = right ? 1 : -1;
      sd.x0 = right ? xr : f.rbeg - 1;
      sd.qlen = qlen;
      sd.lq = lq;
      UngappedScan sc;
      for (int base = 0; base < qlen && !sc.dead(oe_min); base += 16)
        ung_eat(sd, ref, ung_load(sd, ref, base), mat, o.max_mat, sc);
      if (!sc.dead(oe_min)) rec = UngRec::Side{1, sc.side()};
    }
    a.ung[off + i].side[right] = rec;
  }
}

struct SideLists {
  bool cl, cr, in_l, in_r;
};
__device__ __forceinline__ SideLists side_lists(const SpecArgs& a, size_t slot, int qb, int qr) {
  SideLists s{false, false, qb > 0, qr > 0};
  if (a.ung) {
    s.cl = qb > 0 && a.ung[slot].side[0].ok;
    s.in_l = qb > 0 && !s.cl;
    s.cr = qr > 0 && a.ung[slot].side[1].ok && !s.in_l;
    s.in_r = qr > 0 && !s.cr;
  }
  return s;
}

__device__ __forceinline__ SeedExt settle_sides(const DevOpt& o, const FatTask& f, const UngRec& u, bool right) {
  const int qb = (int)(f.qls & 1023u), ln = (int)((f.qls >> 10) & 1023u), lq = (int)(f.qls >> 20);
  const int qr = lq - qb - ln;
  SeedExt e;
  int calls = 0;
  e.rb = f.rbeg;
  e.qb = 0;
  e.score = e.truesc = ln * o.a;
  if (qb > 0) {
    const UngappedOut x = ungapped_result(ln * o.a, qb, u.side[0].s);
    const bool local = x.gscore <= 0 || x.gscore <= x.score - o.pen_clip5;
    e.rb = f.rbeg - (local ? x.tle : x.gtle);
    e.qb = local ? qb - x.qle : 0;
    e.score = x.score;
    e.truesc = local ? x.score : x.gscore;
    ++calls;
  }
  e.re = f.rbeg + ln;
  e.qe = lq;
  if (right) {
    const int h0 = e.score;
    const UngappedOut x = ungapped_result(h0, qr, u.side[1].s);
    const bool local = x.gscore <= 0 || x.gscore <= x.score - o.pen_clip3;
    e.qe = local ? qb + ln + x.qle : lq;
    e.re = f.rbeg + ln + (local ? x.tle : x.gtle);
    e.score = x.score;
    e.truesc += (local ? x.score : x.gscore) - h0;
    ++calls;
  } else if (qr > 0) {
    e.re = 0;
    e.qe = 0;
  }
  e.w = o.w;
  e.cells = e.rows = 0;
  e.calls = calls + (right || qr == 0 ? 1 : 0);
  return e;
}

__global__ void __launch_bounds__(256) spec_sort2_count(DevBatch b, SpecArgs a, int round, int bin0) {
  sel_prio();
  __shared__ int hist[2][256];
  __shared__ int tot[2];
  const int bin = bin0 + (int)blockIdx.y;
  const int list = round * kSpecBins + bin;
  int32_t* ghL = a.sorth + (round * 2 + bin) * kSortKeys;
  int32_t* ghR = ghL + kSortWordsR;
  for (int k = threadIdx.x; k < 2 * 256; k += 256) hist[k >> 8][k & 255] = 0;
  if (threadIdx.x < 2) tot[threadIdx.x] = 0;
  __syncthreads();
  const int n = __hip_atomic_load(&a.ctr[SPC_CNT + list], __ATOMIC_RELAXED, __HIP_MEMORY_SCOPE_AGENT);
  const size_t off = spec_list_off(list, b.n_chains, b.n_seeds);
  const int2* tl = a.tasks + off;
  const int chunk = (n + (int)gridDim.x - 1) / (int)gridDim.x;
  const int i0 = (int)blockIdx.x * chunk, i1 = min(n, i0 + chunk);
  for (int i = i0 + (int)threadIdx.x; i < i1; i += 256) {
    const FatTask f = fat_task(b, a, tl[i]);
    const int qb = (int)(f.qls & 1023u), ln = (int)((f.qls >> 10) & 1023u), lq = (int)(f.qls >> 20);
    const int qr = lq - qb - ln;
    const SideLists sl = side_lists(a, off + i, qb, qr);
    if (sl.in_l) atomicAdd(&hist[0][side_key(qb)], 1);
    if (sl.in_r) atomicAdd(&hist[1][side_key(qr)], 1);
  }
  __syncthreads();
  for (int k = threadIdx.x; k < 2 * 256; k += 256) {
    const int c = hist[k >> 8][k & 255];
    if (c) {
      atomicAdd((k >> 8) ? &ghR[k & 255] : &ghL[k & 255], c);
      atomicAdd(&tot[k >> 8], c);
    }
  }
  __syncthreads();
  if (threadIdx.x < 2 && tot[threadIdx.x])
    atomicAdd(&a.ctr[(threadIdx.x ? SPC_RCNT : SPC_LCNT) + list], tot[threadIdx.x]);
}

__global__ void __launch_bounds__(256) spec_sort2_scan(SpecArgs a, int round, int bin0, int nbins, int short_q) {
  sel_prio();
  __shared__ int part[256];
  const int bin = bin0 + (int)blockIdx.x % nbins, side = (int)blockIdx.x / nbins;
  int32_t* gh = a.sorth + (round * 2 + bin) * kSortKeys + side * kSortWordsR;
  const int t = (int)threadIdx.x;
  const int v = gh[t];
  part[t] = v;
  __syncthreads();
  for (int o = 1; o < 256; o <<= 1) {
    const int x = t >= o ? part[t - o] : 0;
    __syncthreads();
    part[t] += x;
    __syncthreads();
  }
  gh[t] = part[t] - v;
  if (short_q > 0 && bin == 0 && t == side_key(short_q))
    a.ctr[(side ? SPC_RLONG : SPC_LLONG) + round * kSpecBins + bin] = part[t] - v;
}

__global__ void __launch_bounds__(256) spec_sort2_scatter(DevOpt o, DevBatch b, SpecArgs a, int round, int bin0) {
  sel_prio();
  __shared__ int cnt[2][256];
  __shared__ int ung[2];
  const int bin = bin0 + (int)blockIdx.y;
  const int list = round * kSpecBins + bin;
  int32_t* ghL = a.sorth + (round * 2 + bin) * kSortKeys;
  int32_t* ghR = ghL + kSortWordsR;
  for (int k = threadIdx.x; k < 2 * 256; k += 256) cnt[k >> 8][k & 255] = 0;
  if (threadIdx.x < 2) ung[threadIdx.x] = 0;
  __syncthreads();
  const int n = __hip_atomic_load(&a.ctr[SPC_CNT + list], __ATOMIC_RELAXED, __HIP_MEMORY_SCOPE_AGENT);
  const size_t off = spec_list_off(list, b.n_chains, b.n_seeds);
  const int2* tl = a.tasks + off;
  FatTask* foL = a.ftask + off;
  FatTask* foR = a.ftaskR + off;
  const int chunk = (n + (int)gridDim.x - 1) / (int)gridDim.x;
  const int i0 = (int)blockIdx.x * chunk, i1 = min(n, i0 + chunk);
  constexpr int kPer = 8;
  int kl[kPer], kr[kPer], rl[kPer], rr[kPer];
  FatTask ft[kPer];
  for (int base = i0; base < i1; base += 256 * kPer) {
#pragma unroll
    for (int m = 0; m < kPer; ++m) {
      const int i = base + m * 256 + (int)threadIdx.x;
      kl[m] = kr[m] = -1;
      if (i < i1) {
        ft[m] = fat_task(b, a, tl[i]);
        const int qb = (int)(ft[m].qls & 1023u), ln = (int)((ft[m].qls >> 10) & 1023u), lq = (int)(ft[m].qls >> 20);
        const int qr = lq - qb - ln;
        const SideLists sl = side_lists(a, off + i, qb, qr);
        if (sl.in_l) {
          kl[m] = side_key(qb);
          rl[m] = atomicAdd(&cnt[0][kl[m]], 1);
        }
        if (sl.in_r) {
          kr[m] = side_key(qr);
          rr[m] = atomicAdd(&cnt[1][kr[m]], 1);
        }
        if (!sl.in_l) {
          if (qb > 0 || !sl.in_r)
            a.ext[ft[m].pos] = settle_sides(o, ft[m], sl.cl || sl.cr ? a.ung[off + i] : UngRec{}, sl.cr);
          if (sl.cl || sl.cr) {
            atomicAdd(&ung[0], (sl.cl ? 1 : 0) + (sl.cr ? 1 : 0));
            atomicAdd(&ung[1], (sl.cl ? qb : 0) + (sl.cr ? qr : 0));
          }
        }
      }
    }
    __syncthreads();
    for (int k = threadIdx.x; k < 2 * 256; k += 256) {
      const int c = cnt[k >> 8][k & 255];
      cnt[k >> 8][k & 255] = c ? atomicAdd((k >> 8) ? &ghR[k & 255] : &ghL[k & 255], c) : 0;
    }
    __syncthreads();
#pragma unroll
    for (int m = 0; m < kPer; ++m) {
      if (kl[m] >= 0) foL[cnt[0][kl[m]] + rl[m]] = ft[m];
      if (kr[m] >= 0) foR[cnt[1][kr[m]] + rr[m]] = ft[m];
    }
    __syncthreads();
    for (int k = threadIdx.x; k < 2 * 256; k += 256) cnt[k >> 8][k & 255] = 0;
    __syncthreads();
  }
  if (threadIdx.x < 2 && ung[threadIdx.x])
    atomicAdd(&a.ctr[(threadIdx.x ? SPC_UNG_Q : SPC_UNG_N) + round], ung[threadIdx.x]);
}

struct SideTask {
  int64_t rbeg, qoff, rb;
  int32_t pos, dlo, dhi, qbeg, len, lq;
  int32_t tt, score, h0, truesc, qb, aw0, cells, rows, calls, pad_;
};
static_assert(sizeof(SideTask) <= 96, "SideTask layout");
typedef __attribute__((address_space(3))) SideTask LdsS;
#define SIDE_FIELDS(X) X(rbeg) X(qoff) X(rb) X(pos) X(dlo) X(dhi) X(qbeg) X(len) X(lq) X(tt) X(score) X(h0) \
  X(truesc) X(qb) X(aw0) X(cells) X(rows) X(calls)
__device__ __forceinline__ void spark(LdsS* p, const SideTask& t) {
#define X(f) p->f = t.f;
  SIDE_FIELDS(X)
#undef X
  asm volatile("" ::: "memory");
}
__device__ __forceinline__ SideTask sload(LdsS* p) {
  asm volatile("" ::: "memory");
  SideTask t;
#define X(f) t.f = p->f;
  SIDE_FIELDS(X)
#undef X
  return t;
}
#undef SIDE_FIELDS

template <int G, bool RIGHT>
__device__ __forceinline__ void side_start(SideTask& t, const DevOpt& o, const DevRef& ref, const SpecArgs& a,
                                           const FatTask& f, uint8_t* tb) {
  t.rbeg = f.rbeg;
  t.qoff = f.qoff;
  t.pos = f.pos;
  t.dlo = f.dlo;
  t.dhi = f.dhi;
  t.qbeg = (int)(f.qls & 1023u);
  t.len = (int)((f.qls >> 10) & 1023u);
  t.lq = (int)(f.qls >> 20);
  t.tt = 0;
  const int64_t pac_bytes = (ref.l_pac >> 2) + 1;
  const int r = (int)(threadIdx.x & (G - 1));
  if constexpr (!RIGHT) {
    const int n = rows_needed(o, t.qbeg, t.dlo, o.w << 1, o.pen_clip5);
    const int R = (n + G - 1) / G;
    if (R <= 32) fill_side_run<G>(tb, t.rbeg - 1, -1, r * R, min(r * R + R, n), ref, pac_bytes);
    else fill_two_half<G>(tb, t.rbeg - 1, n, tb, 0, 0, ref);
    t.score = -1;
    t.h0 = t.len * o.a;
    t.truesc = -1;
    t.qb = 0;
    t.rb = t.rbeg;
    t.aw0 = o.w;
    t.cells = t.rows = t.calls = 0;
  } else {
    const int64_t x0 = t.rbeg + t.len;
    const int qr = t.lq - t.qbeg - t.len;
    const int n = rows_needed(o, qr, (int)(t.rbeg + t.dhi - x0), o.w << 1, o.pen_clip3);
    const int R = (n + G - 1) / G;
    if (R <= 32) fill_side_run<G>(tb, x0, 1, r * R, min(r * R + R, n), ref, pac_bytes);
    else fill_two_half<G>(tb, 0, 0, tb, x0, n, ref);
    if (t.qbeg > 0) {
      const SeedExt e = a.ext[t.pos];
      t.score = e.score;
      t.truesc = e.truesc;
      t.qb = e.qb;
      t.rb = e.rb;
      t.aw0 = e.w;
      t.cells = e.cells;
      t.rows = e.rows;
      t.calls = e.calls;
    } else {
      t.score = t.truesc = t.len * o.a;
      t.qb = 0;
      t.rb = t.rbeg;
      t.aw0 = o.w;
      t.cells = t.rows = t.calls = 0;
    }
    t.h0 = t.score;
  }
  __builtin_amdgcn_fence(__ATOMIC_RELEASE, "wavefront");
  __builtin_amdgcn_wave_barrier();
  __builtin_amdgcn_fence(__ATOMIC_ACQUIRE, "wavefront");
}

template <bool RIGHT>
__device__ __forceinline__ QCall side_call(const SideTask& t, const DevOpt& o, const uint8_t* seq, const uint8_t* tb) {
  QCall q;
  if constexpr (!RIGHT) {
    q.qlen = t.qbeg;
    q.tlen = t.dlo;
    q.qa = t.qbeg - 1;
    q.qd = -1;
    q.eb = o.pen_clip5;
  } else {
    const int64_t x0 = t.rbeg + t.len;
    q.qlen = t.lq - t.qbeg - t.len;
    q.tlen = (int)(t.rbeg + t.dhi - x0);
    q.qa = t.qbeg + t.len;
    q.qd = 1;
    q.eb = o.pen_clip3;
  }
  q.h0 = t.h0;
  q.w = o.w << t.tt;
  q.zdrop = o.zdrop;
  q.q = seq + t.qoff;
  q.tb = tb;
  q.tlen = rows_needed(o, q.qlen, q.tlen, q.w, q.eb);
  return q;
}

template <int G, bool RIGHT>
__device__ __forceinline__ bool side_advance(SideTask& t, const DevOpt& o, const SpecArgs& a, const ExtOut& x,
                                             const Tally32& tl, long long& spec_cells) {
  t.cells += tl.cells;
  t.rows += tl.rows;
  t.calls += tl.calls;
  const int prev = t.score;
  t.score = x.score;
  const int aw = o.w << t.tt;
  if (t.tt == 0 && !(x.score == prev || x.max_off < (aw >> 1) + (aw >> 2))) {
    t.tt = 1;
    return false;
  }
  const int eb = RIGHT ? o.pen_clip3 : o.pen_clip5;
  const bool local = x.gscore <= 0 || x.gscore <= x.score - eb;
  SeedExt e;
  if constexpr (!RIGHT) {
    const int qr = t.lq - t.qbeg - t.len;
    e.rb = t.rbeg - (local ? x.tle : x.gtle);
    e.qb = local ? t.qbeg - x.qle : 0;
    e.score = t.score;
    e.truesc = local ? x.score : x.gscore;
    if (qr != 0) {
      e.re = 0;
      e.qe = 0;
      e.w = aw;
      e.cells = t.cells;
      e.rows = t.rows;
      e.calls = t.calls;
    } else {
      e.re = t.rbeg + t.len;
      e.qe = t.lq;
      e.w = max(aw, o.w);
      e.cells = t.cells;
      e.rows = t.rows;
      e.calls = t.calls + 1;
      spec_cells += t.cells;
    }
  } else {
    e.rb = t.rb;
    e.qb = t.qb;
    e.qe = local ? t.qbeg + t.len + x.qle : t.lq;
    e.re = t.rbeg + t.len + (local ? x.tle : x.gtle);
// ... 32 lines not shown
  constexpr int QB = PMAX * G;
  uint8_t* const ta_ = wlds + (size_t)((threadIdx.x & 63) / G) * (2 * (size_t)tb_bytes + 2 * kSideLds + 2 * QB);
  uint8_t* const tb_ = ta_ + tb_bytes;
  LdsS* const sa = (LdsS*)(tb_ + tb_bytes);
  LdsS* const sb = (LdsS*)(tb_ + tb_bytes + kSideLds);
  uint8_t* const qa_ = tb_ + tb_bytes + 2 * kSideLds;
  uint8_t* const qb_ = qa_ + QB;
  ShardQ qq;
  qq.init(heads, n);
  bool ha = false, hb = false, more = n > 0;
  int started = 0;
  for (;;) {
#ifdef BWAGPU_OCC_DIAG
    const unsigned long long c0 = __builtin_amdgcn_s_memtime();
#endif
    if (more) {
      const uint64_t na = __builtin_amdgcn_ballot_w64(!ha) & kLead, nb = __builtin_amdgcn_ballot_w64(!hb) & kLead;
      const int nn = __popcll(na) + __popcll(nb);
      if (nn > 0) {
        int m0, cap;
        if (qq.claim(nn, m0, cap)) {
          const int ia = m0 + __popcll(na & below) + __popcll(nb & below), ib = ia + (ha ? 0 : 1);
          if (!ha && ia < cap) {
            SideTask t;
            const FatTask f = fl[qq.shard + 8 * ia];
            side_query<G, RIGHT>(b, f, qa_, QB);
            side_start<G, RIGHT>(t, o, ref, a, f, ta_);
            spark(sa, t);
            ha = true;
            ++started;
          }
          if (!hb && ib < cap) {
            SideTask t;
            const FatTask f = fl[qq.shard + 8 * ib];
            side_query<G, RIGHT>(b, f, qb_, QB);
            side_start<G, RIGHT>(t, o, ref, a, f, tb_);
            spark(sb, t);
            hb = true;
            ++started;
          }
        } else {
          more = false;
        }
      }
    }
#ifdef BWAGPU_OCC_DIAG
    const unsigned long long c1 = __builtin_amdgcn_s_memtime();
    tw[0] += c1 - c0;
#endif
    if (!__builtin_amdgcn_ballot_w64(ha || hb)) {
      if (!more) break;
      continue;
    }
    QCall ca = quad_idle(qa_, ta_), cb = quad_idle(qb_, tb_);
    if (ha) {
      ca = side_call<RIGHT>(sload(sa), o, b.seq, ta_);
      ca.q = qa_;
      ca.qa = 0;
      ca.qd = 1;
    }
    if (hb) {
      cb = side_call<RIGHT>(sload(sb), o, b.seq, tb_);
      cb.q = qb_;
      cb.qa = 0;
      cb.qd = 1;
    }
    ExtOut xa, xb;
    Tally32 tla{0, 0, 0}, tlb{0, 0, 0};
#ifdef BWAGPU_OCC_DIAG
    const unsigned long long c2 = __builtin_amdgcn_s_memtime();
    tw[1] += c2 - c1;
#endif
    extend_quad_dispatch<G, PMAX, K8>(o, ca, cb, xa, xb, tla, tlb);
#ifdef BWAGPU_OCC_DIAG
    const unsigned long long c3 = __builtin_amdgcn_s_memtime();
    tw[2] += c3 - c2;
    occ_diag<G>(occ, ca, cb, tla, tlb);
#endif
    if (ha) {
      SideTask t = sload(sa);
      if (side_advance<G, RIGHT>(t, o, a, xa, tla, spec_cells)) ha = false;
      else spark(sa, t);
    }
    if (hb) {
      SideTask t = sload(sb);
      if (side_advance<G, RIGHT>(t, o, a, xb, tlb, spec_cells)) hb = false;
      else spark(sb, t);
    }
#ifdef BWAGPU_OCC_DIAG
    tw[3] += __builtin_amdgcn_s_memtime() - c3;
#endif
  }
  return started;
}

template <int G, int PMAX, bool K8, bool RIGHT>
__global__ void __launch_bounds__(kBlock) spec_side4_kernel(DevOpt o, DevRef ref, DevBatch b, SpecArgs a, int list,
                                                            int tb_bytes, int wave_lds, int short_q, int tb_short,
                                                            int short_fill) {
  extern __shared__ __attribute__((aligned(16))) uint8_t lds[];
  uint8_t* const wlds = lds + (size_t)(threadIdx.x >> 6) * (size_t)wave_lds;
  const int n = uni(__hip_atomic_load(&a.ctr[(RIGHT ? SPC_RCNT : SPC_LCNT) + list], __ATOMIC_RELAXED,
                                      __HIP_MEMORY_SCOPE_AGENT));
  const FatTask* fl = (RIGHT ? a.ftaskR : a.ftask) + spec_list_off(list, b.n_chains, b.n_seeds);
  constexpr bool kShort = G == 16 && K8;
  int n_long = n;
  if constexpr (kShort) {
    if (short_q > 0) {
      n_long = min(n, uni(__hip_atomic_load(&a.ctr[(RIGHT ? SPC_RLONG : SPC_LLONG) + list], __ATOMIC_RELAXED,
                                            __HIP_MEMORY_SCOPE_AGENT)));
      const long long slots = (long long)gridDim.x * (kBlock / 64) * (128 / kShortG);
      if ((long long)(n - n_long) * 100 < slots * short_fill) n_long = n;
    }
  }
  const int hl = RIGHT ? kSpecRounds * kSpecBins + list : list;
  long long spec_cells = 0;
#ifdef BWAGPU_OCC_DIAG
  unsigned long long tw[6] = {0, 0, 0, 0, 0, 0}, occ[8] = {0, 0, 0, 0, 0, 0, 0, 0};
  (void)side_loop<G, PMAX, K8, RIGHT>(o, ref, b, a, fl, n_long, a.qh + 8 * kQHStride * hl, wlds, tb_bytes, spec_cells,
                                      tw, occ);
#else
  (void)side_loop<G, PMAX, K8, RIGHT>(o, ref, b, a, fl, n_long, a.qh + 8 * kQHStride * hl, wlds, tb_bytes, spec_cells);
#endif
  if constexpr (kShort) {
    if (n_long < n) {
      int32_t* const hs = a.qh + kQHShort + 8 * kQHStride * hl;
      long long cells_s = 0;
#ifdef BWAGPU_OCC_DIAG
      const int ns = side_loop<kShortG, kShortPmax, true, RIGHT>(o, ref, b, a, fl + n_long, n - n_long, hs, wlds,
                                                                 tb_short, cells_s, tw, occ);
#else
      const int ns = side_loop<kShortG, kShortPmax, true, RIGHT>(o, ref, b, a, fl + n_long, n - n_long, hs, wlds,
                                                                 tb_short, cells_s);
#endif
      if ((threadIdx.x & (kShortG - 1)) == 0 && ns) {
        atomicAdd(&a.ctr[SPC_SHORT_N], ns);
        atomicAdd(reinterpret_cast<unsigned long long*>(a.ctr + SPC_SPEC64), (unsigned long long)cells_s);
      }
    }
  }
#ifdef BWAGPU_OCC_DIAG
  if ((threadIdx.x & 63) == 0) {
    for (int k = 0; k < 8; ++k) atomicAdd(reinterpret_cast<unsigned long long*>(a.ctr + 32) + k, occ[k]);
    for (int k = 0; k < 4; ++k) atomicAdd(reinterpret_cast<unsigned long long*>(a.ctr + 48) + k, tw[k]);
  }
#endif
  if ((threadIdx.x & (G - 1)) == 0 && spec_cells)
    atomicAdd(reinterpret_cast<unsigned long long*>(a.ctr + SPC_SPEC64), (unsigned long long)spec_cells);
}


void launch_side_sort(const ExtRound& r, int bin0, int nbins, int short_q, int short_fill) {
  if (r.a.ung)
    hipLaunchKernelGGL(spec_ungapped_kernel, dim3(1024, nbins), dim3(256), 0, r.st, r.o, r.ref, r.b, r.a, r.round, bin0,
                       short_fill == 0 ? short_q : 0);
  hipLaunchKernelGGL(spec_sort2_count, dim3(256, nbins), dim3(256), 0, r.st, r.b, r.a, r.round, bin0);
  hipLaunchKernelGGL(spec_sort2_scan, dim3(2 * nbins), dim3(256), 0, r.st, r.a, r.round, bin0, nbins, short_q);
  hipLaunchKernelGGL(spec_sort2_scatter, dim3(256, nbins), dim3(256), 0, r.st, r.o, r.b, r.a, r.round, bin0);
}

template <int G, int PMAX, bool K8>
static void launch_side_pair(const ExtRound& r, int list, const ExtPlan& p, int short_fill) {
  const size_t lds = (size_t)(kBlock / 64) * p.wave_lds;
  const int nb = resident_blocks(spec_side4_kernel<G, PMAX, K8, false>, lds);
  const int gr = r.round == 2 ? std::min(nb, 64) : std::min(nb, ext2_grid(1 << 30, true));
  if (!(G == 16 && K8)) short_fill = 0;
  hipLaunchKernelGGL((spec_side4_kernel<G, PMAX, K8, false>), dim3(gr), dim3(kBlock), lds, r.st, r.o, r.ref, r.b, r.a,
                     list, r.tb_bytes, (int)p.wave_lds, p.short_q, p.tb_short, short_fill);
  hipLaunchKernelGGL((spec_side4_kernel<G, PMAX, K8, true>), dim3(gr), dim3(kBlock), lds, r.st, r.o, r.ref, r.b, r.a,
                     list, r.tb_bytes, (int)p.wave_lds, p.short_q, p.tb_short, short_fill);
}

void launch_side_bin(const ExtBin& k, const ExtRound& r, int list, const ExtPlan& p, int short_fill) {
  switch (ext_key(k.family, k.G, k.PMAX, k.K8)) {
    case ext_key(SIDE4, 16, 10, true): return launch_side_pair<16, 10, true>(r, list, p, short_fill);
    case ext_key(SIDE4, 32, 5, true): return launch_side_pair<32, 5, true>(r, list, p, short_fill);
    case ext_key(SIDE4, 32, 8, false): return launch_side_pair<32, 8, false>(r, list, p, short_fill);
    default: abort();
  }
}

}
```

### bwa-flow_amd/csrc/ungapped.h

```cpp
#pragma once
#include <stdint.h>

#ifdef __HIPCC__
#define BWAGPU_UNG_HD __host__ __device__
#else
#define BWAGPU_UNG_HD
#endif

namespace bwagpu {

struct UngappedSide {
  int32_t M;
  int32_t am;
  int32_t cl;
};

struct UngappedOut {
  int32_t score, qle, tle, gtle, gscore, max_off;
};

BWAGPU_UNG_HD inline int ungapped_oe_min(int o_del, int e_del, int o_ins, int e_ins) {
  const int d = o_del + e_del, i = o_ins + e_ins;
  return d < i ? d : i;
}

BWAGPU_UNG_HD inline bool ungapped_call_ok(int qlen, int tlen, int h0, int w, int zdrop, int max_mat, int oe_min) {
  return qlen >= 1 && tlen >= qlen && max_mat >= 1 && oe_min >= 1 && h0 >= oe_min && w >= 0 &&
         (zdrop <= 0 || zdrop >= oe_min);
}
BWAGPU_UNG_HD inline bool ungapped_band_ok(int w) { return (w >> 1) + (w >> 2) > 0; }

struct UngappedScan {
  int c = 0, P = 0, M = 0, am = 0;
  BWAGPU_UNG_HD void step(int i, int s, int max_mat) {
    P += max_mat - s;
    c += s;
    if (c > M) {
      M = c;
      am = i + 1;
    }
  }
  BWAGPU_UNG_HD bool dead(int oe_min) const { return P >= oe_min; }
  BWAGPU_UNG_HD UngappedSide side() const { return UngappedSide{M, am, c}; }
};

template <class Score>
BWAGPU_UNG_HD inline bool ungapped_scan(int qlen, int max_mat, int oe_min, Score score, UngappedSide* u) {
  UngappedScan sc;
  for (int i = 0; i < qlen; ++i) {
    sc.step(i, score(i), max_mat);
    if (sc.dead(oe_min)) return false;
  }
  *u = sc.side();
  return true;
}

BWAGPU_UNG_HD inline UngappedOut ungapped_result(int h0, int qlen, const UngappedSide& u) {
  UngappedOut x;
  x.score = h0 + u.M;
  x.qle = x.tle = u.am;
  x.gscore = h0 + u.cl;
  x.gtle = qlen;
  x.max_off = 0;
  return x;
}

}
```

### bwa-flow_amd/python/bwagpu/abi.py

```python
from __future__ import annotations

import ctypes as C
import os

import numpy as np

HERE = os.path.dirname(os.path.abspath(__file__))
PKG_ROOT = os.path.normpath(os.path.join(HERE, "..", ".."))
REPO_ROOT = os.path.normpath(os.path.join(PKG_ROOT, ".."))
LIB_DIR = os.path.join(PKG_ROOT, "lib")

ABI_VERSION = 1
OK, E_INVAL, E_NOMEM, E_DEVICE, E_HANG, E_RESULTS, E_UNSUPPORTED, E_NODEVICE = range(8)
ERR_NAMES = {
    OK: "OK", E_INVAL: "E_INVAL", E_NOMEM: "E_NOMEM", E_DEVICE: "E_DEVICE", E_HANG: "E_HANG",
    E_RESULTS: "E_RESULTS", E_UNSUPPORTED: "E_UNSUPPORTED", E_NODEVICE: "E_NODEVICE",
}
MAX_READ_LEN = 1023
NUM_SLOTS = 4

SEED_DTYPE = np.dtype([("rbeg", "<i8"), ("qbeg", "<i4"), ("len", "<i4"), ("score", "<i4"),
                       ("pad", "<i4")])
ALNREG_DTYPE = np.dtype([
    ("rb", "<i8"), ("re", "<i8"), ("qb", "<i4"), ("qe", "<i4"), ("rid", "<i4"), ("score", "<i4"),
# ... 35 lines not shown
class BatchC(C.Structure):
    _fields_ = [("n_reads", C.c_int32), ("n_chains", C.c_int32), ("n_seeds", C.c_int32),
                ("pad_", C.c_int32), ("seq_bytes", C.c_int64), ("seq_off", C.c_void_p),
                ("seq", C.c_void_p), ("read_chain_off", C.c_void_p), ("chain_seed_off", C.c_void_p),
                ("chain_rid", C.c_void_p), ("chain_frac_rep", C.c_void_p), ("seeds", C.c_void_p)]


class Stats(C.Structure):
    _fields_ = [("kernel_ms", C.c_double), ("total_ms", C.c_double), ("cells", C.c_int64),
                ("rows", C.c_int64), ("ext_calls", C.c_int64), ("h2d_bytes", C.c_int64),
                ("d2h_bytes", C.c_int64)]


class BwtC(C.Structure):
    _fields_ = [("primary", C.c_uint64), ("L2", C.c_uint64 * 5), ("seq_len", C.c_uint64),
                ("bwt_size", C.c_uint64), ("bwt", C.c_void_p), ("sa_intv", C.c_int32), ("pad_", C.c_int32),
                ("n_sa", C.c_uint64), ("sa", C.c_void_p)]


class SeedOpt(C.Structure):
    _fields_ = [("min_seed_len", C.c_int32), ("split_width", C.c_int32), ("max_mem_intv", C.c_int32),
                ("split_factor", C.c_float)]


INTV_DTYPE = np.dtype([("x", "<u8", (3,)), ("info", "<u8")])
assert INTV_DTYPE.itemsize == 32

CHAIN_DTYPE = np.dtype([("pos", "<i8"), ("rid", "<i4"), ("n", "<i4"), ("w", "<i4"), ("kept", "<i4"),
                        ("first", "<i4"), ("is_alt", "<i4"), ("frac_rep", "<f4"), ("pad_", "<i4")])
assert CHAIN_DTYPE.itemsize == 40


class ChainOpt(C.Structure):
    _fields_ = [("max_occ", C.c_int32), ("max_chain_gap", C.c_int32), ("min_chain_weight", C.c_int32),
                ("max_chain_extend", C.c_int32), ("mask_level", C.c_float), ("drop_ratio", C.c_float)]


class ChainsC(C.Structure):
    _fields_ = [("n_reads", C.c_int32), ("n_chains", C.c_int32), ("n_seeds", C.c_int64),
                ("read_chain_off", C.c_void_p), ("chain_seed_off", C.c_void_p), ("chains", C.c_void_p),
                ("seeds", C.c_void_p)]


class PostOpt(C.Structure):
    _fields_ = [("max_chain_gap", C.c_int32), ("mask_level_redun", C.c_float), ("mask_level", C.c_float),
                ("pad_", C.c_int32)]


POST_DEDUP_PATCH, POST_MARK_ALT, POST_PRIMARY = 1, 2, 4


def default_postopt() -> PostOpt:
    return PostOpt(10000, 0.95, 0.50, 0)


class PairOpt(C.Structure):
    _fields_ = [("max_ins", C.c_int32), ("max_matesw", C.c_int32), ("pen_unpaired", C.c_int32),
                ("min_seed_len", C.c_int32), ("max_chain_gap", C.c_int32), ("mask_level_redun", C.c_float),
                ("mask_level", C.c_float), ("max_rounds", C.c_int32)]


def default_pairopt() -> PairOpt:
    return PairOpt(10000, 50, 17, 19, 10000, 0.95, 0.50, 3)


PESTAT_DTYPE = np.dtype([("low", "<i4"), ("high", "<i4"), ("failed", "<i4"), ("pad", "<i4"), ("avg", "<f8"),
                         ("std", "<f8")])
assert PESTAT_DTYPE.itemsize == 32 and C.sizeof(PairOpt) == 32
RESCUE_DONE, RESCUE_UNFINISHED, RESCUE_OVERFLOW, RESCUE_UNSUPPORTED = 0, 1, 2, 3


class SelOpt(C.Structure):
    _fields_ = [("T", C.c_int32), ("pen_unpaired", C.c_int32), ("min_seed_len", C.c_int32),
                ("mapQ_coef_len", C.c_float), ("mapQ_coef_fac", C.c_int32), ("mask_level", C.c_float),
                ("drop_ratio", C.c_float), ("flags", C.c_int32)]


def default_selopt(flags: int = 0) -> SelOpt:
    return SelOpt(30, 17, 19, 50.0, 3, 0.50, 0.50, int(flags))


MEM_F_NOPAIRING, MEM_F_ALL, MEM_F_NO_MULTI, MEM_F_PRIMARY5, MEM_F_KEEP_SUPP_MAPQ = 0x4, 0x8, 0x10, 0x800, 0x1000
SEL_MAX_REGS = 512
SEL_DONE, SEL_TOO_MANY, SEL_SKIPPED = 0, 1, 2
SEL_NO_PAIRING, SEL_PAIRED = 0, 1
PAIRSEL_DTYPE = np.dtype([("status", "<i4"), ("branch", "<i4"), ("n_pri", "<i4", (2,)), ("z", "<i4", (2,)),
                          ("mapq", "<i4", (2,)), ("alt", "<i4", (2,)), ("extra_flag", "<i4"), ("o", "<i4"),
                          ("subo", "<i4"), ("n_sub", "<i4"), ("pad", "<i4", (2,))])
assert PAIRSEL_DTYPE.itemsize == 64 and C.sizeof(SelOpt) == 32


class SamOpt(C.Structure):
    _fields_ = [("flags", C.c_int32), ("XA_drop_ratio", C.c_float), ("max_XA_hits", C.c_int32),
                ("max_XA_hits_alt", C.c_int32)]


def default_samopt(flags: int = 0) -> SamOpt:
    return SamOpt(int(flags), 0.80, 5, 200)


def default_chainopt() -> dict:
    return dict(max_occ=500, max_chain_gap=10000, min_chain_weight=0, max_chain_extend=1 << 30, mask_level=0.5,
                drop_ratio=0.5)

_VP = C.c_void_p
PROTOS = {
    "bwagpu_abi_version": (C.c_int, []),
    "bwagpu_device_count": (C.c_int, [C.POINTER(C.c_int)]),
    "bwagpu_create": (C.c_int, [C.c_int, C.POINTER(Opt), C.POINTER(Bns), _VP, C.POINTER(_VP)]),
    "bwagpu_create_resident": (C.c_int, [C.c_int, C.POINTER(Opt), C.POINTER(Bns), _VP, C.POINTER(_VP)]),
    "bwagpu_destroy": (C.c_int, [_VP]),
    "bwagpu_last_error": (C.c_char_p, [_VP]),
    "bwagpu_set_watchdog_ms": (C.c_int, [_VP, C.c_int]),
    "bwagpu_chain2aln_submit": (C.c_int, [_VP, C.c_int, C.POINTER(BatchC)]),
    "bwagpu_chain2aln_wait": (C.c_int, [_VP, C.c_int, _VP, _VP]),
    "bwagpu_chain2aln_stage": (C.c_int, [_VP, C.c_int, C.c_int32, C.c_int32, C.c_int32, C.c_int64,
                                         C.POINTER(BatchC)]),
    "bwagpu_chain2aln_results": (C.c_int, [_VP, C.c_int, C.POINTER(_VP), C.POINTER(_VP)]),
    "bwagpu_chain2aln_results_dense": (C.c_int, [_VP, C.c_int, C.POINTER(_VP), C.POINTER(_VP), C.POINTER(_VP)]),
    "bwagpu_chain2aln": (C.c_int, [_VP, C.POINTER(BatchC), _VP, _VP]),
    "bwagpu_chain2aln_device": (C.c_int, [_VP, C.POINTER(BatchC), _VP, _VP, _VP, _VP]),
    "bwagpu_extend_batch": (C.c_int, [_VP, C.c_int32, _VP, _VP, C.c_int64, _VP, C.c_int64, _VP]),
    "bwagpu_align2_batch": (C.c_int, [_VP, C.c_int32, _VP, _VP, C.c_int64, _VP, C.c_int64, _VP]),
    "bwagpu_align2_device": (C.c_int, [_VP, C.c_int32, _VP, _VP, _VP, _VP, _VP, _VP]),
    "bwagpu_reg2aln_batch": (C.c_int, [_VP, C.c_int32, _VP, _VP, C.c_int64, C.c_int32, C.c_int32, _VP, _VP, _VP]),
    "bwagpu_reg2aln_device": (C.c_int, [_VP, C.c_int32, _VP, _VP, _VP, C.c_int64, C.c_int32, C.c_int32, _VP, _VP,
                                        _VP, _VP]),
    "bwagpu_reg2aln_jobs_device": (C.c_int, [_VP, C.c_int32, _VP, _VP, _VP, _VP, _VP, C.c_int32, _VP, _VP, _VP, _VP]),
    "bwagpu_xa_select_device": (C.c_int, [_VP, C.POINTER(SamOpt), C.c_int32, _VP, _VP, _VP, _VP, _VP, _VP, _VP, _VP]),
    "bwagpu_debug_reg2aln_times": (C.c_int, [_VP, _VP]),
    "bwagpu_last_stats": (C.c_int, [_VP, C.c_int, C.POINTER(Stats)]),
    "bwagpu_debug_set_trace": (C.c_int, [_VP, _VP]),
    "bwagpu_prof_start": (C.c_int, [_VP, C.c_int]),
    "bwagpu_debug_fail_wait": (C.c_int, [_VP, C.c_int, C.c_int]),
    "bwagpu_debug_live_buffers": (C.c_int, [C.POINTER(C.c_int64), C.POINTER(C.c_int64)]),
    "bwagpu_debug_spec_counters": (C.c_int, [_VP, _VP, _VP]),
    "bwagpu_debug_occupancy": (C.c_int, [_VP, _VP, _VP]),
    "bwagpu_debug_spec_ext": (C.c_int, [_VP, _VP, _VP, C.c_int32]),
    "bwagpu_prof_read": (C.c_int, [_VP, C.POINTER(C.c_double), C.POINTER(C.c_int32)]),
    "bwagpu_prof_intervals": (C.c_int, [_VP, _VP, _VP, C.c_int32, C.POINTER(C.c_int32)]),
    "bwagpu_set_bwt": (C.c_int, [_VP, C.POINTER(BwtC)]),
    "bwagpu_debug_seed_budget": (C.c_int, [_VP, C.c_int32]),
    "bwagpu_debug_sup_shift": (C.c_int, [_VP, C.c_int32]),
    "bwagpu_set_device_read_len": (C.c_int, [_VP, C.c_int32]),
    "bwagpu_debug_ext_form": (C.c_int, [C.c_int]),
    "bwagpu_ctx_ext_form": (C.c_int, [_VP, C.c_int]),
    "bwagpu_ctx_ext_short": (C.c_int, [_VP, C.c_int]),
    "bwagpu_ctx_ext_short_fill": (C.c_int, [_VP, C.c_int]),
    "bwagpu_ctx_light_pack": (C.c_int, [_VP, C.c_int]),
    "bwagpu_debug_spec_short": (C.c_int, [_VP, _VP, _VP]),
    "bwagpu_ctx_row_bound": (C.c_int, [_VP, C.c_int]),
    "bwagpu_ctx_ungapped": (C.c_int, [_VP, C.c_int]),
    "bwagpu_debug_spec_ungapped": (C.c_int, [_VP, _VP, _VP]),
    "bwagpu_ctx_emu_finish": (C.c_int, [_VP, C.c_int]),
    "bwagpu_debug_spec_finish": (C.c_int, [_VP, _VP, _VP]),
    "bwagpu_debug_ext_kernel": (C.c_int, [_VP, C.c_int32]),
    "bwagpu_streams_concurrent": (C.c_int, [_VP, _VP]),
    "bwagpu_bwt_sa": (C.c_int, [_VP, C.c_int64, _VP, _VP]),
    "bwagpu_sw_stream": (C.c_int, [_VP, _VP, C.c_int64, _VP, C.c_int32, C.POINTER(C.c_int32)]),
    "bwagpu_collect_intv": (C.c_int, [_VP, C.POINTER(SeedOpt), C.c_int32, _VP, _VP, C.c_int32, _VP, C.c_int64,
                                       _VP]),
    "bwagpu_set_alt": (C.c_int, [_VP, _VP]),
    "bwagpu_seqs2chains": (C.c_int, [_VP, C.POINTER(SeedOpt), C.POINTER(ChainOpt), C.c_int32, _VP, _VP, C.c_int32,
                                      C.POINTER(ChainsC)]),
    "bwagpu_seqs2regions": (C.c_int, [_VP, C.POINTER(SeedOpt), C.POINTER(ChainOpt), C.c_int32, _VP, _VP, _VP,
                                       C.POINTER(_VP), C.POINTER(C.c_int64)]),
    "bwagpu_regs_post": (C.c_int, [_VP, C.POINTER(PostOpt), C.c_int32, C.c_int64, C.c_int32, _VP, _VP, _VP, _VP,
                                    _VP]),
    "bwagpu_regs_post_device": (C.c_int, [_VP, C.POINTER(PostOpt), C.c_int32, C.c_int64, C.POINTER(BatchC), _VP,
                                           _VP, _VP, _VP]),
    "bwagpu_set_regs_post": (C.c_int, [_VP, C.POINTER(PostOpt), C.c_int32, C.c_int64]),
    "bwagpu_pestat": (C.c_int, [_VP, C.POINTER(PairOpt), C.c_int32, _VP, _VP, _VP, _VP]),
    "bwagpu_pestat_device": (C.c_int, [_VP, C.POINTER(PairOpt), C.c_int32, _VP, _VP, _VP, _VP, _VP]),
    "bwagpu_mate_rescue": (C.c_int, [_VP, C.POINTER(PairOpt), _VP, C.c_int32, _VP, _VP, _VP, _VP, _VP, _VP, _VP, _VP,
                                      _VP, _VP]),
    "bwagpu_mate_rescue_device": (C.c_int, [_VP, C.POINTER(PairOpt), _VP, C.POINTER(BatchC), _VP, _VP, _VP, _VP, _VP,
                                             _VP, _VP, _VP, _VP]),
    "bwagpu_mark_primary": (C.c_int, [_VP, C.POINTER(SelOpt), C.c_int64, C.c_int32, _VP, _VP, _VP, _VP, _VP]),
    "bwagpu_mark_primary_device": (C.c_int, [_VP, C.POINTER(SelOpt), C.c_int64, C.c_int32, _VP, _VP, _VP, _VP, _VP,
                                              _VP]),
    "bwagpu_pair_select": (C.c_int, [_VP, C.POINTER(SelOpt), _VP, C.c_int64, C.c_int32, _VP, _VP, _VP, _VP, _VP, _VP,
                                      _VP]),
    "bwagpu_pair_select_device": (C.c_int, [_VP, C.POINTER(SelOpt), _VP, C.c_int64, C.c_int32, _VP, _VP, _VP, _VP,
                                             _VP, _VP, _VP, _VP]),
    "bwagpu_debug_rescue_drop": (C.c_int, [_VP, C.c_int32]),
    "bwagpu_debug_rescue_times": (C.c_int, [_VP, _VP]),
}

_lib = None


def lib_path() -> str:
    return os.environ.get("BWAGPU_LIB", os.path.join(LIB_DIR, "libbwagpu.so"))


def load() -> C.CDLL:
    global _lib
    if _lib is not None:
        return _lib
    p = lib_path()
    if os.environ.get("BWAGPU_NO_TORCH") != "1":
        try:
            import torch
        except Exception:
            pass
    if not os.path.exists(p):
        raise RuntimeError(f"bwagpu: HIP engine library missing at {p}; run __graft_entry__.build()")
    lib = C.CDLL(p)
    for name, (res, args) in PROTOS.items():
        if (name.startswith("bwagpu_debug_") or name in ("bwagpu_ctx_light_pack", "bwagpu_ctx_ungapped", "bwagpu_ctx_emu_finish")) and not hasattr(lib, name):
            continue
        fn = getattr(lib, name)
        fn.restype = res
        fn.argtypes = args
    if lib.bwagpu_abi_version() != ABI_VERSION:
        raise RuntimeError("bwagpu: ABI version mismatch")
    _lib = lib
    return lib


def opt_from_dict(d: dict) -> Opt:
    o = Opt()
    for k in ("a", "b", "o_del", "e_del", "o_ins", "e_ins", "pen_clip5", "pen_clip3", "w", "zdrop"):
        setattr(o, k, int(d[k]))
    mat = d.get("mat")
    if mat is None:
        mat = fill_scmat(int(d["a"]), int(d["b"]))
    for i in range(25):
        o.mat[i] = int(mat[i])
    return o


def fill_scmat(a: int, b: int) -> np.ndarray:
    m = np.full((5, 5), -1, np.int8)
    for i in range(4):
        for j in range(4):
            m[i, j] = a if i == j else -b
    return m.reshape(-1)


def default_opt() -> dict:
    return dict(a=1, b=4, o_del=6, e_del=1, o_ins=6, e_ins=1, pen_clip5=5, pen_clip3=5, w=100,
                zdrop=100, mat=fill_scmat(1, 4))
```

### bwa-flow_amd/python/bwagpu/engine.py

```python
from __future__ import annotations

import ctypes as C
from dataclasses import dataclass

import numpy as np

from . import abi


class BwaGpuError(RuntimeError):
    def __init__(self, code: int, msg: str):
        super().__init__(f"{abi.ERR_NAMES.get(code, code)}: {msg}")
        self.code = code


def _ptr(a: np.ndarray | None):
    return None if a is None or a.size == 0 else a.ctypes.data_as(C.c_void_p)


@dataclass
class Batch:
    seq_off: np.ndarray
    seq: np.ndarray
    read_chain_off: np.ndarray
# ... 142 lines not shown
        return regs[:batch.n_seeds], n[:batch.n_reads]

    def wait_dense(self, slot: int, batch: Batch, out=None):
        self._check(self.lib.bwagpu_chain2aln_wait(self.ctx, slot, None, None), "wait")
        rp, np_, op = C.c_void_p(), C.c_void_p(), C.c_void_p()
        self._check(self.lib.bwagpu_chain2aln_results_dense(self.ctx, slot, C.byref(rp), C.byref(np_), C.byref(op)),
                    "results_dense")
        nr = batch.n_reads
        if nr == 0:
            return np.zeros(0, abi.ALNREG_DTYPE), np.zeros(0, np.int32)
        cnt = np.ctypeslib.as_array(C.cast(np_, C.POINTER(C.c_int32)), (nr,))
        tot = int(np.ctypeslib.as_array(C.cast(op, C.POINTER(C.c_int32)), (nr + 1,))[nr])
        view = (np.ctypeslib.as_array(C.cast(rp, C.POINTER(C.c_uint8)), (tot * abi.ALNREG_DTYPE.itemsize,))
                .view(abi.ALNREG_DTYPE) if tot else np.zeros(0, abi.ALNREG_DTYPE))
        if out is None:
            return view, cnt
        regs, n = out
        if len(regs) < tot or len(n) < nr:
            raise ValueError("wait_dense: out arrays too small")
        n[:nr] = cnt
        regs[:tot] = view
        return regs[:tot], n[:nr]

    def chain2aln_device(self, dev_batch: abi.BatchC, dev_out: int, dev_n: int, dev_stats: int | None,
                         stream: int | None):
        self._check(self.lib.bwagpu_chain2aln_device(self.ctx, C.byref(dev_batch), C.c_void_p(dev_out),
                                                     C.c_void_p(dev_n),
                                                     C.c_void_p(dev_stats) if dev_stats else None,
                                                     C.c_void_p(stream) if stream else None),
                    "chain2aln_device")

    def extend_batch(self, tasks: np.ndarray, qpool: np.ndarray, tpool: np.ndarray) -> np.ndarray:
        tasks = np.ascontiguousarray(tasks, abi.EXT_TASK_DTYPE)
        qpool = np.ascontiguousarray(qpool, np.uint8)
        tpool = np.ascontiguousarray(tpool, np.uint8)
        res = np.zeros(max(len(tasks), 1), abi.EXT_RES_DTYPE)
        self._check(self.lib.bwagpu_extend_batch(self.ctx, len(tasks), _ptr(tasks), _ptr(qpool), len(qpool),
                                                 _ptr(tpool), len(tpool), _ptr(res)), "extend_batch")
        return res[:len(tasks)]

    def align2_batch(self, tasks: np.ndarray, qpool: np.ndarray, tpool: np.ndarray) -> np.ndarray:
        tasks = np.ascontiguousarray(tasks, abi.ALIGN2_TASK_DTYPE)
        qpool = np.ascontiguousarray(qpool, np.uint8)
        tpool = np.ascontiguousarray(tpool, np.uint8)
        res = np.zeros(max(len(tasks), 1), abi.KSWR_DTYPE)
        self._check(self.lib.bwagpu_align2_batch(self.ctx, len(tasks), _ptr(tasks), _ptr(qpool), len(qpool),
                                                 _ptr(tpool), len(tpool), _ptr(res)), "align2_batch")
        return res[:len(tasks)]

    def align2_device(self, n: int, dev_tasks: int, dev_q: int, dev_t: int, dev_out: int, dev_scratch: int,
                      stream: int | None = None):
        self._check(self.lib.bwagpu_align2_device(self.ctx, n, dev_tasks, dev_q, dev_t, dev_out, dev_scratch,
                                                  stream), "align2_device")

    def reg2aln_batch(self, tasks: np.ndarray, qpool: np.ndarray, max_ops: int = 64, max_md: int = 512):
        tasks = np.ascontiguousarray(tasks, abi.REG2ALN_TASK_DTYPE)
        qpool = np.ascontiguousarray(qpool, np.uint8)
        n = len(tasks)
        out = np.zeros(max(n, 1), abi.ALN_DTYPE)
        cig = np.zeros((max(n, 1), max_ops), np.uint32)
        md = np.zeros((max(n, 1), max_md), np.uint8)
        self._check(self.lib.bwagpu_reg2aln_batch(self.ctx, n, _ptr(tasks), _ptr(qpool), len(qpool), max_ops, max_md,
                                                  _ptr(out), _ptr(cig), _ptr(md)), "reg2aln_batch")
        return out[:n], cig[:n], md[:n]

    def reg2aln_device(self, n_cap: int, dev_tasks: int, dev_qpool: int, qpool_len: int, dev_out: int,
                       dev_cigar: int, dev_md: int, max_ops: int = 64, max_md: int = 512,
                       dev_n_tasks: int | None = None, stream: int | None = None):
        self._check(self.lib.bwagpu_reg2aln_device(
            self.ctx, int(n_cap), C.c_void_p(dev_n_tasks) if dev_n_tasks else None, C.c_void_p(dev_tasks),
            C.c_void_p(dev_qpool) if dev_qpool else None, int(qpool_len), int(max_ops), int(max_md),
            C.c_void_p(dev_out), C.c_void_p(dev_cigar), C.c_void_p(dev_md),
            C.c_void_p(stream) if stream else None), "reg2aln_device")

    def reg2aln_jobs_device(self, n_reads: int, dev_reg_off: int, dev_regs: int, dev_n: int, dev_select: int,
                            dev_seq_off: int, job_cap: int, dev_tasks: int, dev_job_of: int, dev_n_jobs: int,
                            stream: int | None = None):
        self._check(self.lib.bwagpu_reg2aln_jobs_device(
            self.ctx, int(n_reads), C.c_void_p(dev_reg_off), C.c_void_p(dev_regs), C.c_void_p(dev_n),
            C.c_void_p(dev_select), C.c_void_p(dev_seq_off), int(job_cap),
            C.c_void_p(dev_tasks) if dev_tasks else None, C.c_void_p(dev_job_of), C.c_void_p(dev_n_jobs),
            C.c_void_p(stream) if stream else None), "reg2aln_jobs_device")

    def xa_select_device(self, n_reads: int, dev_reg_off: int, dev_regs: int, dev_n: int, dev_sel: int,
                         dev_out_mapq: int, dev_xa_of: int, dev_job_select: int, xopt: abi.SamOpt | None = None,
                         stream: int | None = None):
        xo = abi.default_samopt() if xopt is None else xopt
        self._check(self.lib.bwagpu_xa_select_device(
            self.ctx, C.byref(xo), int(n_reads), C.c_void_p(dev_reg_off), C.c_void_p(dev_regs), C.c_void_p(dev_n),
            C.c_void_p(dev_sel), C.c_void_p(dev_out_mapq), C.c_void_p(dev_xa_of), C.c_void_p(dev_job_select),
            C.c_void_p(stream) if stream else None), "xa_select_device")

    def debug_reg2aln_times(self) -> dict:
        out = np.zeros(4, np.float64)
        self._check(self.lib.bwagpu_debug_reg2aln_times(self.ctx, _ptr(out)), "debug_reg2aln_times")
        return dict(wait_ms=float(out[0]), bins_ms=float(out[1]), call_ms=float(out[2]), jobs=int(out[3]))

    def set_bwt(self, hdr, words, sa=None, sa_intv: int = 32):
        hdr = np.asarray(hdr, np.int64)
        self._bwt_words = np.ascontiguousarray(words, np.uint32)
        self._bwt_sa = None if sa is None else np.ascontiguousarray(sa, np.uint64)
        b = abi.BwtC()
        b.primary = int(hdr[0])
        for i in range(5):
            b.L2[i] = int(hdr[1 + i])
        b.seq_len = int(hdr[6])
        b.bwt_size = len(self._bwt_words)
        b.bwt = self._bwt_words.ctypes.data
        if self._bwt_sa is not None:
            b.sa_intv = sa_intv
            b.n_sa = len(self._bwt_sa)
            b.sa = self._bwt_sa.ctypes.data
        self._check(self.lib.bwagpu_set_bwt(self.ctx, C.byref(b)), "set_bwt")

    def bwt_sa(self, ks) -> np.ndarray:
        ks = np.ascontiguousarray(ks, np.uint64)
        out = np.zeros(max(len(ks), 1), np.uint64)
        self._check(self.lib.bwagpu_bwt_sa(self.ctx, len(ks), _ptr(ks), _ptr(out)), "bwt_sa")
        return out[:len(ks)]

    def sw_stream(self, words: np.ndarray, cap_tasks: int) -> np.ndarray:
        words = np.ascontiguousarray(words, np.int32)
        out = np.zeros((max(cap_tasks, 1), 10), np.int16)
        n = C.c_int32(0)
        self._check(self.lib.bwagpu_sw_stream(self.ctx, _ptr(words), len(words), _ptr(out), int(cap_tasks),
                                              C.byref(n)), "sw_stream")
        return out[:n.value]

    EXT_KERNELS = {2: "spec_ext2_kernel<5>",
                   18: "spec_side4_kernel<16, 10, true>", 14: "spec_side4_kernel<32, 5, true>",
                   15: "spec_side4_kernel<32, 8, false>"}

    def ext_kernel(self, lq_max: int = 256) -> str:
        k = self.lib.bwagpu_debug_ext_kernel(self.ctx, int(lq_max))
        if k not in self.EXT_KERNELS:
            raise BwaGpuError(k, "debug_ext_kernel")
        return self.EXT_KERNELS[k]

    def ext_form(self, form: int = -1) -> int:
        return self.lib.bwagpu_ctx_ext_form(self.ctx, int(form))

    def ext_short(self, q: int = -1) -> int:
        return self.lib.bwagpu_ctx_ext_short(self.ctx, int(q))

    def ext_short_fill(self, percent: int = -1) -> int:
        return self.lib.bwagpu_ctx_ext_short_fill(self.ctx, int(percent))

    def light_pack(self, on: int = -1) -> int:
        return self.lib.bwagpu_ctx_light_pack(self.ctx, int(on))

    def ungapped(self, on: int = -1) -> int:
        return self.lib.bwagpu_ctx_ungapped(self.ctx, int(on))

    def emu_finish(self, on: int = -1) -> int:
        return self.lib.bwagpu_ctx_emu_finish(self.ctx, int(on))

    def row_bound(self, on: int = -1) -> int:
        return self.lib.bwagpu_ctx_row_bound(self.ctx, int(on))

    def set_device_read_len(self, max_len: int):
        self._check(self.lib.bwagpu_set_device_read_len(self.ctx, int(max_len)), "set_device_read_len")

    def sup_shift(self, shift: int):
        self._check(self.lib.bwagpu_debug_sup_shift(self.ctx, shift), "sup_shift")

    def seed_budget(self, budget: int):
        self._check(self.lib.bwagpu_debug_seed_budget(self.ctx, budget), "seed_budget")

    def collect_intv(self, seq_off: np.ndarray, seq: np.ndarray, min_seed_len: int = 19, split_width: int = 10,
                     max_mem_intv: int = 20, split_factor: float = 1.5, max_per_read: int = 256,
                     out_cap: int | None = None, out: np.ndarray | None = None):
        seq_off = np.ascontiguousarray(seq_off, np.int64)
        seq = np.ascontiguousarray(seq, np.uint8)
        n = len(seq_off) - 1
        o = abi.SeedOpt(min_seed_len, split_width, max_mem_intv, split_factor)
        if out is not None:
            if out.dtype != abi.INTV_DTYPE or not out.flags.c_contiguous:
                raise ValueError("out must be a contiguous INTV_DTYPE array")
            cap = len(out)
        else:
            cap = max(n, 1) * max_per_read if out_cap is None else out_cap
            out = np.zeros(max(cap, 1), abi.INTV_DTYPE)
        cnt = np.zeros(max(n, 1), np.int32)
        self._check(self.lib.bwagpu_collect_intv(self.ctx, C.byref(o), n, _ptr(seq_off), _ptr(seq), max_per_read,
                                                 _ptr(out), cap, _ptr(cnt)), "collect_intv")
        cnt = cnt[:n]
        return cnt, out[:int(cnt.sum())]

    def set_alt(self, is_alt):
        self._alt = None if is_alt is None else np.ascontiguousarray(is_alt, np.uint8)
        self._check(self.lib.bwagpu_set_alt(self.ctx, None if self._alt is None else _ptr(self._alt)), "set_alt")

    @staticmethod
    def _seed_chain_opts(seedopt, split_factor, chainopt):
        so = np.asarray(seedopt, np.int32)
        co = abi.default_chainopt() if chainopt is None else chainopt
        return (abi.SeedOpt(int(so[0]), int(so[1]), int(so[2]), float(split_factor)),
                abi.ChainOpt(int(co["max_occ"]), int(co["max_chain_gap"]), int(co["min_chain_weight"]),
                             int(co["max_chain_extend"]), float(co["mask_level"]), float(co["drop_ratio"])))

    def seqs2chains(self, seq_off, seq, seedopt=(19, 10, 20), split_factor: float = 1.5, chainopt: dict | None = None,
                    raw: bool = False, copy: bool = True):
        seq_off = np.ascontiguousarray(seq_off, np.int64)
        seq = np.ascontiguousarray(seq, np.uint8)
        n = len(seq_off) - 1
        so, co = self._seed_chain_opts(seedopt, split_factor, chainopt)
        out = abi.ChainsC()
        self._check(self.lib.bwagpu_seqs2chains(self.ctx, C.byref(so), C.byref(co), n, _ptr(seq_off), _ptr(seq),
                                                int(raw), C.byref(out)), "seqs2chains")
        nc, ns = out.n_chains, out.n_seeds

        def view(p, dt, k):
            if k == 0:
                return np.zeros(0, dt)
            v = np.frombuffer((C.c_char * (k * np.dtype(dt).itemsize)).from_address(p), dt)
            return v.copy() if copy else v
        return (view(out.read_chain_off, np.int32, n + 1), view(out.chains, abi.CHAIN_DTYPE, nc),
                view(out.chain_seed_off, np.int32, nc + 1), view(out.seeds, abi.SEED_DTYPE, ns))

    def seqs2regions(self, seq_off, seq, seedopt=(19, 10, 20), split_factor: float = 1.5,
                     chainopt: dict | None = None, copy: bool = True):
        seq_off = np.ascontiguousarray(seq_off, np.int64)
        seq = np.ascontiguousarray(seq, np.uint8)
        n = len(seq_off) - 1
        so, co = self._seed_chain_opts(seedopt, split_factor, chainopt)
        cnt = np.zeros(max(n, 1), np.int32)
        regs, nreg = C.c_void_p(), C.c_int64()
        self._check(self.lib.bwagpu_seqs2regions(self.ctx, C.byref(so), C.byref(co), n, _ptr(seq_off), _ptr(seq),
                                                 _ptr(cnt), C.byref(regs), C.byref(nreg)), "seqs2regions")
        k = nreg.value
        out = np.zeros(0, abi.ALNREG_DTYPE) if k == 0 else np.frombuffer(
            (C.c_char * (k * abi.ALNREG_DTYPE.itemsize)).from_address(regs.value), abi.ALNREG_DTYPE)
        return cnt[:n], (out.copy() if copy else out)

    def regs_post(self, seq_off, seq, reg_off, regs, n, flags: int, id0: int = 0, popt: abi.PostOpt | None = None):
        seq_off = np.ascontiguousarray(seq_off, np.int64)
        seq = np.ascontiguousarray(seq, np.uint8)
        reg_off = np.ascontiguousarray(reg_off, np.int64)
        regs = np.array(regs, abi.ALNREG_DTYPE, order="C")
        n = np.array(n, np.int32, order="C")
        nr = len(seq_off) - 1
        if len(reg_off) < nr or len(n) < nr:
            raise ValueError("regs_post: reg_off / n shorter than the batch")
        po = abi.default_postopt() if popt is None else popt
        self._check(self.lib.bwagpu_regs_post(self.ctx, C.byref(po), int(flags), int(id0), nr, _ptr(seq_off),
                                              _ptr(seq), _ptr(reg_off), _ptr(regs), _ptr(n)), "regs_post")
        return regs, n

    def regs_post_device(self, dev_batch: abi.BatchC, dev_reg_off: int | None, dev_regs: int, dev_n: int,
                         flags: int, id0: int = 0, popt: abi.PostOpt | None = None, stream: int | None = None):
        po = abi.default_postopt() if popt is None else popt
        self._check(self.lib.bwagpu_regs_post_device(self.ctx, C.byref(po), int(flags), int(id0), C.byref(dev_batch),
                                                     C.c_void_p(dev_reg_off) if dev_reg_off else None,
                                                     C.c_void_p(dev_regs), C.c_void_p(dev_n),
                                                     C.c_void_p(stream) if stream else None), "regs_post_device")

    def set_regs_post(self, flags: int, id0: int = 0, popt: abi.PostOpt | None = None):
        po = abi.default_postopt() if popt is None else popt
        self._check(self.lib.bwagpu_set_regs_post(self.ctx, C.byref(po), int(flags), int(id0)), "set_regs_post")

    def pestat(self, reg_off, regs, n, popt: abi.PairOpt | None = None) -> np.ndarray:
        reg_off = np.ascontiguousarray(reg_off, np.int64)
        regs = np.ascontiguousarray(regs, abi.ALNREG_DTYPE)
        n = np.ascontiguousarray(n, np.int32)
        if len(reg_off) != len(n):
            raise ValueError("pestat: reg_off and n differ in length")
        po = abi.default_pairopt() if popt is None else popt
        pes = np.zeros(4, abi.PESTAT_DTYPE)
        self._check(self.lib.bwagpu_pestat(self.ctx, C.byref(po), len(n), _ptr(reg_off), _ptr(regs), _ptr(n),
                                           _ptr(pes)), "pestat")
        return pes

    def pestat_device(self, n_reads: int, dev_reg_off: int, dev_regs: int, dev_n: int, dev_pes: int,
                      popt: abi.PairOpt | None = None, stream: int | None = None):
        po = abi.default_pairopt() if popt is None else popt
        self._check(self.lib.bwagpu_pestat_device(self.ctx, C.byref(po), int(n_reads), C.c_void_p(dev_reg_off),
                                                  C.c_void_p(dev_regs), C.c_void_p(dev_n), C.c_void_p(dev_pes),
                                                  C.c_void_p(stream) if stream else None), "pestat_device")

    def mate_rescue(self, pes, seq_off, seq, reg_off, regs, n, out_off, popt: abi.PairOpt | None = None):
        pes = np.ascontiguousarray(pes, abi.PESTAT_DTYPE)
        seq_off = np.ascontiguousarray(seq_off, np.int64)
        seq = np.ascontiguousarray(seq, np.uint8)
        reg_off = np.ascontiguousarray(reg_off, np.int64)
        regs = np.ascontiguousarray(regs, abi.ALNREG_DTYPE)
        n = np.ascontiguousarray(n, np.int32)
        out_off = np.ascontiguousarray(out_off, np.int64)
        nr = len(seq_off) - 1
        if len(pes) != 4 or len(reg_off) < nr or len(n) < nr or len(out_off) != nr + 1:
            raise ValueError("mate_rescue: pes / reg_off / n / out_off do not fit the batch")
        po = abi.default_pairopt() if popt is None else popt
        out = np.zeros(max(int(out_off[-1]), 1), abi.ALNREG_DTYPE)
        out_n = np.zeros(max(nr, 1), np.int32)
        status = np.zeros(max(nr // 2, 1), np.int32)
        n_sw = np.zeros(max(nr // 2, 1), np.int32)
        self._check(self.lib.bwagpu_mate_rescue(self.ctx, C.byref(po), _ptr(pes), nr, _ptr(seq_off), _ptr(seq),
                                                _ptr(reg_off), _ptr(regs), _ptr(n), _ptr(out_off), _ptr(out),
                                                _ptr(out_n), _ptr(status), _ptr(n_sw)), "mate_rescue")
        return out, out_n[:nr], status[:nr // 2], n_sw[:nr // 2]

    def mate_rescue_device(self, dev_pes: int, dev_batch: abi.BatchC, dev_reg_off: int, dev_regs: int, dev_n: int,
                           dev_out_off: int, dev_out_regs: int, dev_out_n: int, dev_status: int, dev_n_sw: int,
                           popt: abi.PairOpt | None = None, stream: int | None = None):
        po = abi.default_pairopt() if popt is None else popt
        self._check(self.lib.bwagpu_mate_rescue_device(
            self.ctx, C.byref(po), C.c_void_p(dev_pes), C.byref(dev_batch), C.c_void_p(dev_reg_off),
# ... 95 lines not shown
```

### include/bwagpu_debug.h

```cpp
#ifndef BWAGPU_DEBUG_H
#define BWAGPU_DEBUG_H
#include "bwagpu.h"

#ifdef __cplusplus
extern "C" {
#endif

int bwagpu_debug_seed_budget(bwagpu_ctx_t *ctx, int32_t budget);

int bwagpu_debug_sup_shift(bwagpu_ctx_t *ctx, int32_t shift);

int bwagpu_debug_set_trace(bwagpu_ctx_t *ctx, void *dev_ptr);
int bwagpu_debug_fail_wait(bwagpu_ctx_t *ctx, int after_n_waits, int code);
int bwagpu_debug_live_buffers(int64_t *n, int64_t *bytes);

int bwagpu_prof_start(bwagpu_ctx_t *ctx, int max_launches);
int bwagpu_debug_spec_counters(bwagpu_ctx_t *ctx, void *stream, int64_t *out);
int bwagpu_debug_occupancy(bwagpu_ctx_t *ctx, void *stream, int64_t *out);
int bwagpu_debug_spec_ext(bwagpu_ctx_t *ctx, void *stream, void *host_out, int32_t n);
int bwagpu_prof_read(bwagpu_ctx_t *ctx, double *total_ms, int32_t *launches);
int bwagpu_debug_ext_form(int form);
int bwagpu_ctx_ext_form(bwagpu_ctx_t *ctx, int form);
int bwagpu_ctx_ext_short(bwagpu_ctx_t *ctx, int q);
int bwagpu_ctx_ext_short_fill(bwagpu_ctx_t *ctx, int percent);
int bwagpu_ctx_light_pack(bwagpu_ctx_t *ctx, int on);
int bwagpu_debug_spec_short(bwagpu_ctx_t *ctx, void *stream, int64_t *out);
int bwagpu_ctx_ungapped(bwagpu_ctx_t *ctx, int on);
int bwagpu_debug_spec_ungapped(bwagpu_ctx_t *ctx, void *stream, int64_t *out);
int bwagpu_ctx_emu_finish(bwagpu_ctx_t *ctx, int on);
int bwagpu_debug_spec_finish(bwagpu_ctx_t *ctx, void *stream, int64_t *out);
int bwagpu_ctx_row_bound(bwagpu_ctx_t *ctx, int on);
int bwagpu_debug_ext_kernel(bwagpu_ctx_t *ctx, int32_t lq_max);
int bwagpu_streams_concurrent(void *a, void *b);
int bwagpu_debug_rescue_drop(bwagpu_ctx_t *ctx, int32_t k);
int bwagpu_debug_rescue_times(bwagpu_ctx_t *ctx, double *out);
int bwagpu_debug_reg2aln_times(bwagpu_ctx_t *ctx, double *out);
int bwagpu_prof_intervals(bwagpu_ctx_t *ctx, double *start_ms, double *end_ms, int32_t max, int32_t *n);

#ifdef __cplusplus
}
#endif
#endif
```

### tools_dev/ungapped_share.py

```python
#!/usr/bin/env python3
import ctypes as C
import json
import os
import sys

import numpy as np
import torch

REPO = os.path.normpath(os.path.join(os.path.dirname(os.path.abspath(__file__)), ".."))
sys.path.insert(0, os.path.join(REPO, "bwa-flow_amd", "python"))
from bwagpu import abi, workload
from bwagpu.engine import Engine

nb = int(sys.argv[1]) if len(sys.argv) > 1 else 2
opt, ref, rbs = workload.load_fixture()
eng = Engine(0, opt, ref.l_pac, ref.ann_offset, ref.ann_len, pac=ref.pac)
dev = torch.device("cuda:0")
fields = ("seq_off", "seq", "read_chain_off", "chain_seed_off", "chain_rid", "chain_frac_rep", "seeds")
out = {"fixture": "c2_refseed", "batches": []}
for k, rb in enumerate(rbs[:nb]):
    b = rb.batch
    t = {f: torch.from_numpy(np.ascontiguousarray(getattr(b, f)).view(np.uint8).copy()).to(dev) for f in fields}
    regs = torch.zeros(max(b.n_seeds, 1) * 88, dtype=torch.uint8, device=dev)
    nn = torch.zeros(max(b.n_reads, 1), dtype=torch.int32, device=dev)
    c = abi.BatchC()
    c.n_reads, c.n_chains, c.n_seeds = b.n_reads, b.n_chains, b.n_seeds
    c.seq_bytes = int(b.seq_off[-1])
    for f in fields:
        setattr(c, f, t[f].data_ptr())
    st = torch.cuda.current_stream()
    eng.chain2aln_device(c, regs.data_ptr(), nn.data_ptr(), None, st.cuda_stream)
    torch.cuda.synchronize()
    ctr = np.zeros(12, np.int64)
    assert eng.lib.bwagpu_debug_spec_ungapped(eng.ctx, C.c_void_p(st.cuda_stream), ctr.ctypes.data_as(C.c_void_p)) == 0
    ok = rb.check(regs.cpu().numpy().view(abi.ALNREG_DTYPE)[:b.n_seeds], nn.cpu().numpy()[:b.n_reads])
    rounds = {}
    for r, name in enumerate("AB"):
        settled, bases, left, right = (int(x) for x in ctr[4 * r:4 * r + 4])
        rounds[name] = {"settled_sides": settled, "settled_bases": bases, "listed_left": left, "listed_right": right,
                        "settled_share_of_sides": round(settled / max(settled + left + right, 1), 4)}
    out["batches"].append({"batch": k, "reads": b.n_reads, "regions_match_reference": bool(ok), "rounds": rounds})
print(json.dumps(out))
```

Measured before the change: 69.39.

## Restructure ungapped side scan into per-pass parallel work and settle late right sides

Rewrites the ungapped extension kernel so each thread scores the first 16-base pass of one side, then uses a block-wide prefix scan to list the remaining 16-base passes in shared memory and spreads them across all threads. The per-pass scoring now uses SWAR byte tricks and a packed 8-wide score table instead of per-base branches. It also adds an on-by-default 'ungapped right' path that records right-side task info so right sides whose left side needs DP can still be settled later. This aims to cut serial per-side latency and DP work, at the cost of more shared memory, extra barriers and a possible overflow fallback when a block needs more passes than the shared list holds.

```diff
diff --git a/bwa-flow_amd/csrc/capi.hip b/bwa-flow_amd/csrc/capi.hip
--- a/bwa-flow_amd/csrc/capi.hip
+++ b/bwa-flow_amd/csrc/capi.hip
@@ -153,6 +153,7 @@
   ctx->ext_short_fill = ext_short_fill_default();
   ctx->light_pack = light_pack_default();
   ctx->ungapped = ungapped_default();
+  ctx->ungapped_right = ungapped_right_default();
   ctx->emu_finish = emu_finish_default();
   *made = ctx;
   HIPC(hipSetDevice(device), "hipSetDevice");
@@ -326,6 +327,8 @@
   HIPC(s.d_ftaskR.get(a.ftaskR, n_tasks), "hipMalloc(ftaskR)");
   a.ung = nullptr;
   if (ctx->ungapped && ctx->opt.row_bound) HIPC(s.d_ung.get(a.ung, n_tasks), "hipMalloc(ung)");
+  a.ungt = nullptr;
+  if (a.ung && ctx->ungapped_right) HIPC(s.d_ungt.get(a.ungt, n_tasks), "hipMalloc(ungt)");
   HIPC(s.d_mat.get(a.mat, (size_t)std::max<int64_t>(1 << 20, 16 * (int64_t)ns)), "hipMalloc(mat)");
   a.mat_words = (int64_t)(s.d_mat.cap / sizeof(uint64_t));
   static const int ext_prefetch = [] {
@@ -759,16 +762,21 @@
   return BWAGPU_OK;
 }
 
-int bwagpu_debug_occupancy(bwagpu_ctx_t* ctx, void* stream, int64_t* out) {
-  if (!ctx || !out) return BWAGPU_E_INVAL;
+static int spec_ctr_words(bwagpu_ctx_t* ctx, void* stream, int32_t* c) {
   hipStream_t st = nullptr;
   if (int rc = entry_stream(ctx, stream, &st)) return rc;
   int k = 0;
   while (k < BWAGPU_NUM_SLOTS && ctx->dev_stream[k] != st) ++k;
   if (k == BWAGPU_NUM_SLOTS || !ctx->dev_scratch[k].d_ctr.p) return fail(ctx, BWAGPU_E_INVAL, "no device-entry batch on this stream");
   HIPC(hipStreamSynchronize(st), "hipStreamSynchronize");
+  HIPC(hipMemcpy(c, ctx->dev_scratch[k].d_ctr.p, sizeof(int32_t) * SPC_WORDS, hipMemcpyDeviceToHost), "hipMemcpy(ctr)");
+  return BWAGPU_OK;
+}
+
+int bwagpu_debug_occupancy(bwagpu_ctx_t* ctx, void* stream, int64_t* out) {
+  if (!ctx || !out) return BWAGPU_E_INVAL;
   int32_t c[SPC_WORDS];
-  HIPC(hipMemcpy(c, ctx->dev_scratch[k].d_ctr.p, sizeof c, hipMemcpyDeviceToHost), "hipMemcpy(ctr)");
+  if (int rc = spec_ctr_words(ctx, stream, c)) return rc;
   memcpy(out, c + 32, 14 * sizeof(int64_t));
 #ifdef BWAGPU_OCC_DIAG
   return BWAGPU_OK;
@@ -779,14 +787,8 @@
 
 int bwagpu_debug_spec_counters(bwagpu_ctx_t* ctx, void* stream, int64_t* out) {
   if (!ctx || !out) return BWAGPU_E_INVAL;
-  hipStream_t st = nullptr;
-  if (int rc = entry_stream(ctx, stream, &st)) return rc;
-  int k = 0;
-  while (k < BWAGPU_NUM_SLOTS && ctx->dev_stream[k] != st) ++k;
-  if (k == BWAGPU_NUM_SLOTS || !ctx->dev_scratch[k].d_ctr.p) return fail(ctx, BWAGPU_E_INVAL, "no device-entry batch on this stream");
-  HIPC(hipStreamSynchronize(st), "hipStreamSynchronize");
   int32_t c[SPC_WORDS];
-  HIPC(hipMemcpy(c, ctx->dev_scratch[k].d_ctr.p, sizeof c, hipMemcpyDeviceToHost), "hipMemcpy(ctr)");
+  if (int rc = spec_ctr_words(ctx, stream, c)) return rc;
   for (int r = 0; r < kSpecRounds; ++r) {
     out[r] = 0;
     for (int b = 0; b < kSpecBins; ++b) out[r] += c[SPC_CNT + r * kSpecBins + b];
@@ -852,14 +854,8 @@
 
 int bwagpu_debug_spec_short(bwagpu_ctx_t* ctx, void* stream, int64_t* out) {
   if (!ctx || !out) return BWAGPU_E_INVAL;
-  hipStream_t st = nullptr;
-  if (int rc = entry_stream(ctx, stream, &st)) return rc;
-  int k = 0;
-  while (k < BWAGPU_NUM_SLOTS && ctx->dev_stream[k] != st) ++k;
-  if (k == BWAGPU_NUM_SLOTS || !ctx->dev_scratch[k].d_ctr.p) return fail(ctx, BWAGPU_E_INVAL, "no device-entry batch on this stream");
-  HIPC(hipStreamSynchronize(st), "hipStreamSynchronize");
   int32_t c[SPC_WORDS];
-  HIPC(hipMemcpy(c, ctx->dev_scratch[k].d_ctr.p, sizeof c, hipMemcpyDeviceToHost), "hipMemcpy(ctr)");
+  if (int rc = spec_ctr_words(ctx, stream, c)) return rc;
   out[0] = c[SPC_SHORT_N];
   for (int r = 0; r < 2; ++r) {
     const int l = r * kSpecBins;
@@ -880,14 +876,8 @@
 
 int bwagpu_debug_spec_ungapped(bwagpu_ctx_t* ctx, void* stream, int64_t* out) {
   if (!ctx || !out) return BWAGPU_E_INVAL;
-  hipStream_t st = nullptr;
-  if (int rc = entry_stream(ctx, stream, &st)) return rc;
-  int k = 0;
-  while (k < BWAGPU_NUM_SLOTS && ctx->dev_stream[k] != st) ++k;
-  if (k == BWAGPU_NUM_SLOTS || !ctx->dev_scratch[k].d_ctr.p) return fail(ctx, BWAGPU_E_INVAL, "no device-entry batch on this stream");
-  HIPC(hipStreamSynchronize(st), "hipStreamSynchronize");
   int32_t c[SPC_WORDS];
-  HIPC(hipMemcpy(c, ctx->dev_scratch[k].d_ctr.p, sizeof c, hipMemcpyDeviceToHost), "hipMemcpy(ctr)");
+  if (int rc = spec_ctr_words(ctx, stream, c)) return rc;
   for (int r = 0; r < kSpecRounds; ++r) {
     out[4 * r + 0] = c[SPC_UNG_N + r];
     out[4 * r + 1] = c[SPC_UNG_Q + r];
@@ -900,6 +890,24 @@
   return BWAGPU_OK;
 }
 
+int bwagpu_ctx_ungapped_right(bwagpu_ctx_t* ctx, int on) {
+  if (!ctx) return BWAGPU_E_INVAL;
+  const int prev = ctx->ungapped_right;
+  if (on >= 0) ctx->ungapped_right = on ? 1 : 0;
+  return prev;
+}
+
+int bwagpu_debug_spec_ungapped_right(bwagpu_ctx_t* ctx, void* stream, int64_t* out) {
+  if (!ctx || !out) return BWAGPU_E_INVAL;
+  int32_t c[SPC_WORDS];
+  if (int rc = spec_ctr_words(ctx, stream, c)) return rc;
+  for (int r = 0; r < kSpecRounds; ++r) {
+    out[2 * r + 0] = c[SPC_UNGR_N + r];
+    out[2 * r + 1] = c[SPC_UNGR_Q + r];
+  }
+  return BWAGPU_OK;
+}
+
 int bwagpu_ctx_emu_finish(bwagpu_ctx_t* ctx, int on) {
   if (!ctx) return BWAGPU_E_INVAL;
   const int prev = ctx->emu_finish;
@@ -909,14 +917,8 @@
 
 int bwagpu_debug_spec_finish(bwagpu_ctx_t* ctx, void* stream, int64_t* out) {
   if (!ctx || !out) return BWAGPU_E_INVAL;
-  hipStream_t st = nullptr;
-  if (int rc = entry_stream(ctx, stream, &st)) return rc;
-  int k = 0;
-  while (k < BWAGPU_NUM_SLOTS && ctx->dev_stream[k] != st) ++k;
-  if (k == BWAGPU_NUM_SLOTS || !ctx->dev_scratch[k].d_ctr.p) return fail(ctx, BWAGPU_E_INVAL, "no device-entry batch on this stream");
-  HIPC(hipStreamSynchronize(st), "hipStreamSynchronize");
   int32_t c[SPC_WORDS];
-  HIPC(hipMemcpy(c, ctx->dev_scratch[k].d_ctr.p, sizeof c, hipMemcpyDeviceToHost), "hipMemcpy(ctr)");
+  if (int rc = spec_ctr_words(ctx, stream, c)) return rc;
   out[0] = c[SPC_FIN_NAR];
   out[1] = c[SPC_FIN_WIDE];
   out[2] = c[SPC_LIST_N];
diff --git a/bwa-flow_amd/csrc/ctx.h b/bwa-flow_amd/csrc/ctx.h
--- a/bwa-flow_amd/csrc/ctx.h
+++ b/bwa-flow_amd/csrc/ctx.h
@@ -73,7 +73,7 @@
   hipEvent_t ev0 = nullptr, ev1 = nullptr, ev2 = nullptr, ev3 = nullptr;
   DevBuf d_in, d_win, d_srt, d_prog, d_desc, d_out, d_n, d_stats, d_lists, d_counts;
   DevBuf d_cread, d_ext, d_tasks, d_ctr, d_regpos, d_skipf, d_heavy, d_redo, d_rbits, d_rlist;
-  DevBuf d_schain, d_hinfo, d_mat, d_cov, d_hflag, d_colent, d_qh, d_longc, d_sorth, d_stasks, d_ftask, d_ftaskR, d_ung;
+  DevBuf d_schain, d_hinfo, d_mat, d_cov, d_hflag, d_colent, d_qh, d_longc, d_sorth, d_stasks, d_ftask, d_ftaskR, d_ung, d_ungt;
   SpecStreams spec;
   bool side_chosen = false;
   HostBuf h_in, h_out, h_n, h_stats;
@@ -135,6 +135,7 @@
   int light_pack = 0;
   int ext_short_fill = 0;
   int ungapped = 1;
+  int ungapped_right = 1;
   int emu_finish = 1;
   Slot slot[BWAGPU_NUM_SLOTS];
   hipStream_t dev_stream[BWAGPU_NUM_SLOTS] = {};
diff --git a/bwa-flow_amd/csrc/engine.h b/bwa-flow_amd/csrc/engine.h
--- a/bwa-flow_amd/csrc/engine.h
+++ b/bwa-flow_amd/csrc/engine.h
@@ -114,6 +114,8 @@
   SPC_FIN_WIDE = 110,
   SPC_LIST_N = 111,
   SPC_LIGHT_N = 112,
+  SPC_UNGR_N = 113,
+  SPC_UNGR_Q = 116,
   SPC_WORDS = 128
 };
 constexpr int kQHStride = 32;
@@ -142,6 +144,12 @@
   } side[2];
 };
 static_assert(sizeof(UngRec) == 32, "UngRec layout");
+struct UngTask {
+  int64_t rbeg;
+  int32_t pos;
+  uint32_t qls;
+};
+static_assert(sizeof(UngTask) == 16, "UngTask layout");
 struct SpecArgs {
   int lq_bound;
   ChainWin* win;
@@ -172,6 +180,7 @@
   FatTask* ftask;
   FatTask* ftaskR;
   UngRec* ung;
+  UngTask* ungt;
   int risky_first;
   int emu_strict;
   int light_pack;
@@ -192,6 +201,7 @@
   int short_fill = 0;
 };
 int ungapped_default();
+int ungapped_right_default();
 int emu_finish_default();
 int set_ext_form(int form);
 int ext_short_default();
diff --git a/bwa-flow_amd/csrc/spec.hip b/bwa-flow_amd/csrc/spec.hip
--- a/bwa-flow_amd/csrc/spec.hip
+++ b/bwa-flow_amd/csrc/spec.hip
@@ -2084,6 +2084,13 @@
   }();
   return on;
 }
+int ungapped_right_default() {
+  static const int on = [] {
+    const char* e = getenv("BWAGPU_UNGAPPED_RIGHT");
+    return !(e && e[0] == '0');
+  }();
+  return on;
+}
 int emu_finish_default() {
   static const int on = [] {
     const char* e = getenv("BWAGPU_EMU_FINISH");
diff --git a/bwa-flow_amd/csrc/spec_side.hip b/bwa-flow_amd/csrc/spec_side.hip
--- a/bwa-flow_amd/csrc/spec_side.hip
+++ b/bwa-flow_amd/csrc/spec_side.hip
@@ -10,58 +10,95 @@
   int64_t x0;
   int p0, d, qlen, lq;
 };
-struct UngPass {
-  uint64_t qw[2], tw;
-  int64_t fa, b0;
-  int base, last, ws;
-  bool fast, rev;
+__device__ __forceinline__ UngSeg ung_pass(const UngSide& s, const DevRef& ref, int base, const int8_t* mat,
+                                           const int8_t* mat8, int max_mat) {
+  const int last = min(base + 15, s.qlen - 1), cnt = last - base + 1;
+  const int64_t two1 = (ref.l_pac << 1) - 1, pac_bytes = (ref.l_pac >> 2) + 1;
+  const int64_t xa = s.x0 + (int64_t)s.d * base, xb = s.x0 + (int64_t)s.d * last;
+  const bool rev = xa >= ref.l_pac;
+  const int64_t fa = rev ? two1 - xa : xa, fb = rev ? two1 - xb : xb;
+  UngSeg g;
+  if (s.lq >= 16 && pac_bytes >= 8 && (xb >= ref.l_pac) == rev) {
+    const int qa = s.p0 + s.d * base;
+    const int ws = min(max(min(qa, qa + 15 * s.d), 0), s.lq - 16);
+    const int64_t b0 = min(min(fa, fb) >> 2, pac_bytes - 8);
+    uint64_t q[2], tw;
+    __builtin_memcpy(q, s.rd + ws, 16);
+    __builtin_memcpy(&tw, ref.pac + b0, 8);
+    uint64_t lo = q[0], hi = q[1];
+    int sh = qa - ws;
+    if (s.d < 0) {
+      lo = __builtin_bswap64(q[1]);
+      hi = __builtin_bswap64(q[0]);
+      sh = 15 - sh;
+    }
+    if (sh >= 8) {
+      lo = hi;
+      hi = 0;
+    }
+    const int sb = (sh & 7) * 8;
+    if (sb) {
+      lo = (lo >> sb) | (hi << (64 - sb));
+      hi >>= sb;
+    }
+    constexpr uint64_t k7f = 0x7f7f7f7f7f7f7f7full, k80 = 0x8080808080808080ull, k04 = 0x0404040404040404ull,
+                       k05 = 0x0505050505050505ull;
+    uint64_t ge = ((((lo & k7f) + (k7f - k04)) | lo) & k80) >> 7;
+    lo = (lo & ~(ge * 255)) | (ge * 4);
+    ge = ((((hi & k7f) + (k7f - k04)) | hi) & k80) >> 7;
+    hi = (hi & ~(ge * 255)) | (ge * 4);
+    if (cnt < 8) lo = (lo & ~(~0ull << (8 * cnt))) | (k05 << (8 * cnt));
+    if (cnt <= 8) hi = k05;
+    else if (cnt < 16) hi = (hi & ~(~0ull << (8 * (cnt - 8)))) | (k05 << (8 * (cnt - 8)));
+    const uint64_t T = __builtin_bswap64(tw);
+    const int f0 = (int)(fa - (b0 << 2));
+    uint32_t w;
+    if ((s.d > 0) != rev) {
+      w = __builtin_bitreverse32((uint32_t)((T << (2 * f0)) >> 32));
+      w = ((w & 0x55555555u) << 1) | ((w >> 1) & 0x55555555u);
+    } else {
+      w = (uint32_t)(T >> (62 - 2 * f0));
+    }
+    if (rev) w = ~w;
+    const uint32_t qw[4] = {(uint32_t)lo, (uint32_t)(lo >> 32), (uint32_t)hi, (uint32_t)(hi >> 32)};
+    int c = 0, key = 31;
+#pragma unroll
+    for (int m = 0; m < 16; ++m) {
+      const uint32_t qv = (qw[m >> 2] >> ((m & 3) * 8)) & 255u, tv = (w >> (2 * m)) & 3u;
+      c += mat8[(tv << 3) | qv];
+      key = max(key, c * 32 + 30 - m);
+    }
+    g.n = cnt;
+    g.c = c;
+    g.P = cnt * max_mat - c;
+    g.M = key >> 5;
+    g.am = 31 - (key & 31);
+  } else {
+    for (int j = base; j <= last; ++j)
+      g = ungseg_combine(g, ungseg_base(mat[pac_base2(ref.pac, ref.l_pac, s.x0 + (int64_t)s.d * j) * 5 +
+                                            min((int)s.rd[s.p0 + s.d * j], 4)], max_mat));
+  }
+  return g;
+}
+
+constexpr int kUngTasks = 128;
+constexpr int kUngPassCap = 256 * 9;
+struct UngSeg16 {
+  int16_t c, P, M, am;
 };
-__device__ __forceinline__ UngPass ung_load(const UngSide& s, const DevRef& ref, int base) {
-  UngPass p;
-  p.base = base;
-  p.last = min(base + 15, s.qlen - 1);
-  p.fast = false;
-  if (base >= s.qlen) return p;
-  const int64_t two1 = (ref.l_pac << 1) - 1, pac_bytes = (ref.l_pac >> 2) + 1;
-  const int64_t xa = s.x0 + (int64_t)s.d * base, xb = s.x0 + (int64_t)s.d * p.last;
-  p.rev = xa >= ref.l_pac;
-  p.fa = p.rev ? two1 - xa : xa;
-  const int64_t fb = p.rev ? two1 - xb : xb;
-  p.fast = s.lq >= 16 && pac_bytes >= 8 && (xb >= ref.l_pac) == p.rev;
-  if (p.fast) {
-    p.ws = min(max(min(s.p0 + s.d * base, s.p0 + s.d * (base + 15)), 0), s.lq - 16);
-    p.b0 = min(min(p.fa, fb) >> 2, pac_bytes - 8);
-    __builtin_memcpy(p.qw, s.rd + p.ws, 16);
-    __builtin_memcpy(&p.tw, ref.pac + p.b0, 8);
-  }
-  return p;
-}
-__device__ __forceinline__ void ung_eat(const UngSide& s, const DevRef& ref, const UngPass& p, const int8_t* mat,
-                                        int max_mat, UngappedScan& sc) {
-  if (p.base >= s.qlen) return;
-  if (p.fast) {
-#pragma unroll
-    for (int m = 0; m < 16; ++m)
-      if (p.base + m <= p.last) {
-        const int k = s.p0 + s.d * (p.base + m) - p.ws;
-        const int qv = (int)(p.qw[k >> 3] >> ((k & 7) * 8)) & 255;
-        const int64_t fm = p.fa + (p.rev ? -s.d : s.d) * m;
-        const int byte = (int)(p.tw >> (((fm >> 2) - p.b0) * 8)) & 255;
-        const int bse = (byte >> ((~fm & 3) << 1)) & 3;
-        sc.step(p.base + m, mat[(p.rev ? 3 - bse : bse) * 5 + min(qv, 4)], max_mat);
-      }
-  } else {
-    for (int j = p.base; j <= p.last; ++j)
-      sc.step(j, mat[pac_base2(ref.pac, ref.l_pac, s.x0 + (int64_t)s.d * j) * 5 + min((int)s.rd[s.p0 + s.d * j], 4)],
-              max_mat);
-  }
-}
 
 __global__ void __launch_bounds__(256) spec_ungapped_kernel(DevOpt o, DevRef ref, DevBatch b, SpecArgs a, int round,
                                                             int bin0, int keep_short) {
   sel_prio();
-  __shared__ int8_t mat[25];
-  if (threadIdx.x < 25) mat[threadIdx.x] = o.mat[threadIdx.x];
+  __shared__ int8_t mat[25], mat8[32];
+  __shared__ UngSide sd[256];
+  __shared__ uint32_t plist[kUngPassCap];
+  __shared__ UngSeg16 seg[kUngPassCap];
+  __shared__ int wsum[4], listed;
+  const int tid = (int)threadIdx.x;
+  if (tid < 25) mat[tid] = o.mat[tid];
+  if (tid < 32) mat8[tid] = (tid & 7) < 5 ? o.mat[(tid >> 3) * 5 + (tid & 7)] : 0;
+  if (tid == 0) listed = 0;
   __syncthreads();
   const int bin = bin0 + (int)blockIdx.y;
   const int list = round * kSpecBins + bin;
@@ -70,46 +107,105 @@
   const int2* tl = a.tasks + off;
   const int oe_min = ungapped_oe_min(o.o_del, o.e_del, o.o_ins, o.e_ins);
   const int keep = bin == 0 ? keep_short : 0;
-  const int chunk = (n + (int)gridDim.x - 1) / (int)gridDim.x;
-  const int i0 = (int)blockIdx.x * chunk, i1 = min(n, i0 + chunk);
-  for (int k = 2 * i0 + (int)threadIdx.x; k < 2 * i1; k += 256) {
-    const int i = k >> 1, right = k & 1;
-    const FatTask f = fat_task(b, a, tl[i]);
-    const int qb = (int)(f.qls & 1023u), ln = (int)((f.qls >> 10) & 1023u), lq = (int)(f.qls >> 20);
-    const int64_t xr = f.rbeg + ln;
-    const int qlen = right ? lq - qb - ln : qb;
-    const int tlen = right ? (int)(f.rbeg + f.dhi - xr) : f.dlo;
+  for (int t0 = (int)blockIdx.x * kUngTasks; t0 < n; t0 += (int)gridDim.x * kUngTasks) {
+    const int i = t0 + (tid >> 1), right = tid & 1;
+    UngSide s{};
+    UngSeg g;
+    bool ok = false;
+    int extra = 0;
+    if (i < n) {
+      const FatTask f = fat_task(b, a, tl[i]);
+      if (right && a.ungt) a.ungt[off + i] = UngTask{f.rbeg, f.pos, f.qls};
+      const int qb = (int)(f.qls & 1023u), ln = (int)((f.qls >> 10) & 1023u), lq = (int)(f.qls >> 20);
+      const int64_t xr = f.rbeg + ln;
+      const int qlen = right ? lq - qb - ln : qb;
+      const int tlen = right ? (int)(f.rbeg + f.dhi - xr) : f.dlo;
+      ok = qlen > keep && ungapped_band_ok(o.w) &&
+           ungapped_call_ok(qlen, tlen, ln * o.a, o.w, o.zdrop, o.max_mat, oe_min);
+      if (ok) {
+        s.rd = b.seq + f.qoff;
+        s.p0 = right ? qb + ln : qb - 1;
+        s.d = right ? 1 : -1;
+        s.x0 = right ? xr : f.rbeg - 1;
+        s.qlen = qlen;
+        s.lq = lq;
+        g = ung_pass(s, ref, 0, mat, mat8, o.max_mat);
+        if (!g.dead(oe_min)) extra = (qlen - 1) >> 4;
+      }
+    }
+    int inc = extra;
+#pragma unroll
+    for (int d = 1; d < 64; d <<= 1) {
+      const int y = __shfl_up(inc, d, 64);
+      if ((tid & 63) >= d) inc += y;
+    }
+    if ((tid & 63) == 63) wsum[tid >> 6] = inc;
+    __syncthreads();
+    int pos = inc - extra;
+    for (int w = 0; w < (tid >> 6); ++w) pos += wsum[w];
+    const bool fits = pos + extra <= kUngPassCap;
+    if (extra > 0 && fits) {
+      sd[tid] = s;
+      for (int k = 1; k <= extra; ++k) plist[pos + k - 1] = (uint32_t)tid << 8 | (uint32_t)k;
+      atomicMax(&listed, pos + extra);
+    }
+    __syncthreads();
+    const int np = listed;
+    for (int p = tid; p < np; p += 256) {
+      const uint32_t e = plist[p];
+      const UngSeg x = ung_pass(sd[e >> 8], ref, (int)(e & 255u) * 16, mat, mat8, o.max_mat);
+      seg[p] = UngSeg16{(int16_t)x.c, (int16_t)x.P, (int16_t)x.M, (int16_t)x.am};
+    }
+    __syncthreads();
     UngRec::Side rec{0, {0, 0, 0}};
-    if (qlen > keep && ungapped_band_ok(o.w) &&
-        ungapped_call_ok(qlen, tlen, ln * o.a, o.w, o.zdrop, o.max_mat, oe_min)) {
-      UngSide sd;
-      sd.rd = b.seq + f.qoff;
-      sd.p0 = right ? qb + ln : qb - 1;
-      sd.d = right ? 1 : -1;
-      sd.x0 = right ? xr : f.rbeg - 1;
-      sd.qlen = qlen;
-      sd.lq = lq;
-      UngappedScan sc;
-      for (int base = 0; base < qlen && !sc.dead(oe_min); base += 16)
-        ung_eat(sd, ref, ung_load(sd, ref, base), mat, o.max_mat, sc);
-      if (!sc.dead(oe_min)) rec = UngRec::Side{1, sc.side()};
-    }
-    a.ung[off + i].side[right] = rec;
+    if (ok) {
+      for (int k = 1; k <= extra && !g.dead(oe_min); ++k) {
+        UngSeg x;
+        if (fits) {
+          const UngSeg16 y = seg[pos + k - 1];
+          x.n = min(16, s.qlen - 16 * k);
+          x.c = y.c;
+          x.P = y.P;
+          x.M = y.M;
+          x.am = y.am;
+        } else {
+          x = ung_pass(s, ref, 16 * k, mat, mat8, o.max_mat);
+        }
+        g = ungseg_combine(g, x);
+      }
+      if (!g.dead(oe_min)) rec = UngRec::Side{1, g.side()};
+    }
+    if (i < n) a.ung[off + i].side[right] = rec;
+    if (tid == 0) listed = 0;
+    __syncthreads();
   }
 }
 
 struct SideLists {
-  bool cl, cr, in_l, in_r;
+  bool cl, cr, in_l, in_r, late;
 };
 __device__ __forceinline__ SideLists side_lists(const SpecArgs& a, size_t slot, int qb, int qr) {
-  SideLists s{false, false, qb > 0, qr > 0};
+  SideLists s{false, false, qb > 0, qr > 0, false};
   if (a.ung) {
     s.cl = qb > 0 && a.ung[slot].side[0].ok;
     s.in_l = qb > 0 && !s.cl;
-    s.cr = qr > 0 && a.ung[slot].side[1].ok && !s.in_l;
-    s.in_r = qr > 0 && !s.cr;
+    const bool okr = qr > 0 && a.ung[slot].side[1].ok;
+    s.cr = okr && !s.in_l;
+    s.late = okr && s.in_l && a.ungt;
+    s.in_r = qr > 0 && !s.cr && !s.late;
   }
   return s;
+}
+
+__device__ __forceinline__ void settle_right(const DevOpt& o, SeedExt& e, int64_t rbeg, int qb, int ln, int lq,
+                                             const UngappedSide& u) {
+  const int h0 = e.score;
+  const UngappedOut x = ungapped_result(h0, lq - qb - ln, u);
+  const bool local = x.gscore <= 0 || x.gscore <= x.score - o.pen_clip3;
+  e.qe = local ? qb + ln + x.qle : lq;
+  e.re = rbeg + ln + (local ? x.tle : x.gtle);
+  e.score = x.score;
+  e.truesc += (local ? x.score : x.gscore) - h0;
 }
 
 __device__ __forceinline__ SeedExt settle_sides(const DevOpt& o, const FatTask& f, const UngRec& u, bool right) {
@@ -132,13 +228,7 @@
   e.re = f.rbeg + ln;
   e.qe = lq;
   if (right) {
-    const int h0 = e.score;
-    const UngappedOut x = ungapped_result(h0, qr, u.side[1].s);
-    const bool local = x.gscore <= 0 || x.gscore <= x.score - o.pen_clip3;
-    e.qe = local ? qb + ln + x.qle : lq;
-    e.re = f.rbeg + ln + (local ? x.tle : x.gtle);
-    e.score = x.score;
-    e.truesc += (local ? x.score : x.gscore) - h0;
+    settle_right(o, e, f.rbeg, qb, ln, lq, u.side[1].s);
     ++calls;
   } else if (qr > 0) {
     e.re = 0;
@@ -273,6 +363,42 @@
   }
   if (threadIdx.x < 2 && ung[threadIdx.x])
     atomicAdd(&a.ctr[(threadIdx.x ? SPC_UNG_Q : SPC_UNG_N) + round], ung[threadIdx.x]);
+}
+
+__global__ void __launch_bounds__(256) spec_settle_right_kernel(DevOpt o, DevBatch b, SpecArgs a, int round, int bin0) {
+  sel_prio();
+  __shared__ int tot[2];
+  __shared__ unsigned long long cel;
+  if (threadIdx.x < 2) tot[threadIdx.x] = 0;
+  if (threadIdx.x == 0) cel = 0;
+  __syncthreads();
+  const int list = round * kSpecBins + bin0 + (int)blockIdx.y;
+  const int n = __hip_atomic_load(&a.ctr[SPC_CNT + list], __ATOMIC_RELAXED, __HIP_MEMORY_SCOPE_AGENT);
+  const size_t off = spec_list_off(list, b.n_chains, b.n_seeds);
+  int sides = 0, bases = 0;
+  unsigned long long cells = 0;
+  for (int i = (int)(blockIdx.x * 256 + threadIdx.x); i < n; i += (int)gridDim.x * 256) {
+    const UngTask t = a.ungt[off + i];
+    const int qb = (int)(t.qls & 1023u), ln = (int)((t.qls >> 10) & 1023u), lq = (int)(t.qls >> 20);
+    if (!side_lists(a, off + i, qb, lq - qb - ln).late) continue;
+    SeedExt e = a.ext[t.pos];
+    settle_right(o, e, t.rbeg, qb, ln, lq, a.ung[off + i].side[1].s);
+    e.w = max(e.w, o.w);
+    e.calls += 2;
+    a.ext[t.pos] = e;
+    ++sides;
+    bases += lq - qb - ln;
+    cells += (unsigned long long)e.cells;
+  }
+  if (sides) {
+    atomicAdd(&tot[0], sides);
+    atomicAdd(&tot[1], bases);
+    atomicAdd(&cel, cells);
+  }
+  __syncthreads();
+  if (threadIdx.x < 2 && tot[threadIdx.x])
+    atomicAdd(&a.ctr[(threadIdx.x ? SPC_UNGR_Q : SPC_UNGR_N) + round], tot[threadIdx.x]);
+  if (threadIdx.x == 0 && cel) atomicAdd(reinterpret_cast<unsigned long long*>(a.ctr + SPC_SPEC64), cel);
 }
 
 struct SideTask {
@@ -611,7 +737,7 @@
 
 void launch_side_sort(const ExtRound& r, int bin0, int nbins, int short_q, int short_fill) {
   if (r.a.ung)
-    hipLaunchKernelGGL(spec_ungapped_kernel, dim3(1024, nbins), dim3(256), 0, r.st, r.o, r.ref, r.b, r.a, r.round, bin0,
+    hipLaunchKernelGGL(spec_ungapped_kernel, dim3(512, nbins), dim3(256), 0, r.st, r.o, r.ref, r.b, r.a, r.round, bin0,
                        short_fill == 0 ? short_q : 0);
   hipLaunchKernelGGL(spec_sort2_count, dim3(256, nbins), dim3(256), 0, r.st, r.b, r.a, r.round, bin0);
   hipLaunchKernelGGL(spec_sort2_scan, dim3(2 * nbins), dim3(256), 0, r.st, r.a, r.round, bin0, nbins, short_q);
@@ -626,6 +752,9 @@
   if (!(G == 16 && K8)) short_fill = 0;
   hipLaunchKernelGGL((spec_side4_kernel<G, PMAX, K8, false>), dim3(gr), dim3(kBlock), lds, r.st, r.o, r.ref, r.b, r.a,
                      list, r.tb_bytes, (int)p.wave_lds, p.short_q, p.tb_short, short_fill);
+  if (r.a.ungt)
+    hipLaunchKernelGGL(spec_settle_right_kernel, dim3(256, 1), dim3(256), 0, r.st, r.o, r.b, r.a, r.round,
+                       list % kSpecBins);
   hipLaunchKernelGGL((spec_side4_kernel<G, PMAX, K8, true>), dim3(gr), dim3(kBlock), lds, r.st, r.o, r.ref, r.b, r.a,
                      list, r.tb_bytes, (int)p.wave_lds, p.short_q, p.tb_short, short_fill);
 }
diff --git a/bwa-flow_amd/csrc/ungapped.h b/bwa-flow_amd/csrc/ungapped.h
--- a/bwa-flow_amd/csrc/ungapped.h
+++ b/bwa-flow_amd/csrc/ungapped.h
@@ -55,6 +55,31 @@
   return true;
 }
 
+struct UngSeg {
+  int32_t n = 0, c = 0, P = 0, M = 0, am = 0;
+  BWAGPU_UNG_HD bool dead(int oe_min) const { return P >= oe_min; }
+  BWAGPU_UNG_HD UngappedSide side() const { return UngappedSide{M, am, c}; }
+};
+BWAGPU_UNG_HD inline UngSeg ungseg_base(int s, int max_mat) {
+  UngSeg g;
+  g.n = 1;
+  g.c = s;
+  g.P = max_mat - s;
+  g.M = s > 0 ? s : 0;
+  g.am = s > 0 ? 1 : 0;
+  return g;
+}
+BWAGPU_UNG_HD inline UngSeg ungseg_combine(const UngSeg& a, const UngSeg& b) {
+  UngSeg g;
+  g.n = a.n + b.n;
+  g.c = a.c + b.c;
+  g.P = a.P + b.P;
+  const bool later = a.c + b.M > a.M;
+  g.M = later ? a.c + b.M : a.M;
+  g.am = later ? a.n + b.am : a.am;
+  return g;
+}
+
 BWAGPU_UNG_HD inline UngappedOut ungapped_result(int h0, int qlen, const UngappedSide& u) {
   UngappedOut x;
   x.score = h0 + u.M;
diff --git a/bwa-flow_amd/python/bwagpu/abi.py b/bwa-flow_amd/python/bwagpu/abi.py
--- a/bwa-flow_amd/python/bwagpu/abi.py
+++ b/bwa-flow_amd/python/bwagpu/abi.py
@@ -211,6 +211,8 @@
     "bwagpu_ctx_row_bound": (C.c_int, [_VP, C.c_int]),
     "bwagpu_ctx_ungapped": (C.c_int, [_VP, C.c_int]),
     "bwagpu_debug_spec_ungapped": (C.c_int, [_VP, _VP, _VP]),
+    "bwagpu_ctx_ungapped_right": (C.c_int, [_VP, C.c_int]),
+    "bwagpu_debug_spec_ungapped_right": (C.c_int, [_VP, _VP, _VP]),
     "bwagpu_ctx_emu_finish": (C.c_int, [_VP, C.c_int]),
     "bwagpu_debug_spec_finish": (C.c_int, [_VP, _VP, _VP]),
     "bwagpu_debug_ext_kernel": (C.c_int, [_VP, C.c_int32]),
@@ -267,7 +269,7 @@
         raise RuntimeError(f"bwagpu: HIP engine library missing at {p}; run __graft_entry__.build()")
     lib = C.CDLL(p)
     for name, (res, args) in PROTOS.items():
-        if (name.startswith("bwagpu_debug_") or name in ("bwagpu_ctx_light_pack", "bwagpu_ctx_ungapped", "bwagpu_ctx_emu_finish")) and not hasattr(lib, name):
+        if (name.startswith("bwagpu_debug_") or name in ("bwagpu_ctx_light_pack", "bwagpu_ctx_ungapped", "bwagpu_ctx_ungapped_right", "bwagpu_ctx_emu_finish")) and not hasattr(lib, name):
             continue
         fn = getattr(lib, name)
         fn.restype = res
diff --git a/bwa-flow_amd/python/bwagpu/engine.py b/bwa-flow_amd/python/bwagpu/engine.py
--- a/bwa-flow_amd/python/bwagpu/engine.py
+++ b/bwa-flow_amd/python/bwagpu/engine.py
@@ -318,6 +318,15 @@
     def ungapped(self, on: int = -1) -> int:
         return self.lib.bwagpu_ctx_ungapped(self.ctx, int(on))
 
+    def ungapped_right(self, on: int = -1) -> int:
+        return self.lib.bwagpu_ctx_ungapped_right(self.ctx, int(on))
+
+    def ungapped_right_counters(self, stream=None):
+        out = np.zeros(6, np.int64)
+        self._check(self.lib.bwagpu_debug_spec_ungapped_right(self.ctx, C.c_void_p(stream), _ptr(out)),
+                    "debug_spec_ungapped_right")
+        return out.reshape(3, 2)
+
     def emu_finish(self, on: int = -1) -> int:
         return self.lib.bwagpu_ctx_emu_finish(self.ctx, int(on))
 
diff --git a/include/bwagpu_debug.h b/include/bwagpu_debug.h
--- a/include/bwagpu_debug.h
+++ b/include/bwagpu_debug.h
@@ -27,6 +27,8 @@
 int bwagpu_debug_spec_short(bwagpu_ctx_t *ctx, void *stream, int64_t *out);
 int bwagpu_ctx_ungapped(bwagpu_ctx_t *ctx, int on);
 int bwagpu_debug_spec_ungapped(bwagpu_ctx_t *ctx, void *stream, int64_t *out);
+int bwagpu_ctx_ungapped_right(bwagpu_ctx_t *ctx, int on);
+int bwagpu_debug_spec_ungapped_right(bwagpu_ctx_t *ctx, void *stream, int64_t *out);
 int bwagpu_ctx_emu_finish(bwagpu_ctx_t *ctx, int on);
 int bwagpu_debug_spec_finish(bwagpu_ctx_t *ctx, void *stream, int64_t *out);
 int bwagpu_ctx_row_bound(bwagpu_ctx_t *ctx, int on);
diff --git a/tools_dev/ungapped_passes.py b/tools_dev/ungapped_passes.py
--- /dev/null
+++ b/tools_dev/ungapped_passes.py
@@ -0,0 +1,95 @@
+#!/usr/bin/env python3
+import json
+import os
+import sys
+
+import numpy as np
+
+REPO = os.path.normpath(os.path.join(os.path.dirname(os.path.abspath(__file__)), ".."))
+sys.path.insert(0, os.path.join(REPO, "bwa-flow_amd", "python"))
+from bwagpu import workload
+
+
+def cal_max_gap(opt, qlen):
+    l = max(int((qlen * opt["a"] - opt["o_del"]) / opt["e_del"]) + 1, int((qlen * opt["a"] - opt["o_ins"]) / opt["e_ins"]) + 1, 1)
+    return min(l, opt["w"] << 1)
+
+
+def fetch(ref, x0, n):
+    x = np.arange(x0, x0 + n, dtype=np.int64)
+    rev = x >= ref.l_pac
+    f = np.where(rev, 2 * ref.l_pac - 1 - x, x)
+    bs = (ref.pac[f >> 2].astype(np.int64) >> ((~f & 3) << 1)) & 3
+    return np.where(rev, 3 - bs, bs)
+
+
+def main():
+    nb = int(sys.argv[1]) if len(sys.argv) > 1 else 2
+    opt, ref, rbs = workload.load_fixture()
+    mat = np.asarray(opt["mat"], np.int64).reshape(5, 5)
+    max_mat = int(max(0, mat.max()))
+    oe_min = min(opt["o_del"] + opt["e_del"], opt["o_ins"] + opt["e_ins"])
+    opt_ok = (opt["zdrop"] <= 0 or opt["zdrop"] >= oe_min) and (opt["w"] >> 1) + (opt["w"] >> 2) > 0 and max_mat >= 1
+    l_pac = int(ref.l_pac)
+    out = {"fixture": "c2_refseed", "round": "A", "batches": []}
+    for k, rb in enumerate(rbs[:nb]):
+        b = rb.batch
+        cert_l = cert_r = settled = late = late_q = sides = call_ok = issued = serial = 0
+        for rd in range(b.n_reads):
+            lq = int(b.seq_off[rd + 1] - b.seq_off[rd])
+            seq = b.seq[b.seq_off[rd]:b.seq_off[rd + 1]]
+            for c in range(int(b.read_chain_off[rd]), int(b.read_chain_off[rd + 1])):
+                sd = b.seeds[int(b.chain_seed_off[c]):int(b.chain_seed_off[c + 1])]
+                if len(sd) == 0:
+                    continue
+                qbs, lns, rbs_ = sd["qbeg"].astype(np.int64), sd["len"].astype(np.int64), sd["rbeg"].astype(np.int64)
+                lo = min(int(r - (q + cal_max_gap(opt, int(q)))) for r, q in zip(rbs_, qbs))
+                hi = max(int(r + n + (lq - q - n) + cal_max_gap(opt, int(lq - q - n))) for r, q, n in zip(rbs_, qbs, lns))
+                lo, hi = max(lo, 0), min(hi, 2 * l_pac)
+                if lo < l_pac < hi:
+                    if int(rbs_[0]) < l_pac:
+                        hi = l_pac
+                    else:
+                        lo = l_pac
+                rid = int(b.chain_rid[c])
+                a0, al = int(ref.ann_offset[rid]), int(ref.ann_len[rid])
+                if int(rbs_[0]) >= l_pac:
+                    a0 = 2 * l_pac - (a0 + al)
+                lo, hi = max(lo, a0), min(hi, a0 + al)
+                t = max(range(len(sd)), key=lambda i: (int(sd[i]["score"]), i))
+                rbeg, qb, ln = int(rbs_[t]), int(qbs[t]), int(lns[t])
+                qr = lq - qb - ln
+                ok = [False, False]
+                for side, (q, x0, n, tlen, flip) in enumerate(((seq[:qb][::-1], rbeg - qb, qb, rbeg - lo, True),
+                                                               (seq[qb + ln:], rbeg + ln, qr, hi - (rbeg + ln), False))):
+                    if n == 0:
+                        continue
+                    sides += 1
+                    if not (opt_ok and ln * opt["a"] >= oe_min and tlen >= n):
+                        continue
+                    call_ok += 1
+                    tg = fetch(ref, x0, n)
+                    if flip:
+                        tg = tg[::-1]
+                    loss = np.cumsum(max_mat - mat[tg, np.minimum(q, 4)])
+                    ends = loss[np.minimum(np.arange(16, n + 16, 16), n) - 1]
+                    passes = len(ends)
+                    dead = np.nonzero(ends >= oe_min)[0]
+                    serial += int(dead[0]) + 1 if len(dead) else passes
+                    issued += 1 if ends[0] >= oe_min else passes
+                    ok[side] = len(dead) == 0
+                cert_l += ok[0]
+                cert_r += ok[1]
+                in_l = qb > 0 and not ok[0]
+                settled += int(ok[0]) + int(ok[1] and not in_l)
+                late += int(ok[1] and in_l)
+                late_q += qr if ok[1] and in_l else 0
+        out["batches"].append({"batch": k, "reads": b.n_reads, "chains": b.n_chains, "sides": sides, "sides_call_ok": call_ok,
+                               "certificate_holds": cert_l + cert_r, "settled_at_sort_time": settled, "late_right": late,
+                               "late_right_bases": late_q, "passes_issued_dense": issued, "passes_serial_needs": serial,
+                               "issued_over_serial": round(issued / max(serial, 1), 4)})
+    print(json.dumps(out))
+
+
+if __name__ == "__main__":
+    main()
diff --git a/tools_dev/ungapped_share.py b/tools_dev/ungapped_share.py
--- a/tools_dev/ungapped_share.py
+++ b/tools_dev/ungapped_share.py
@@ -17,7 +17,8 @@
 eng = Engine(0, opt, ref.l_pac, ref.ann_offset, ref.ann_len, pac=ref.pac)
 dev = torch.device("cuda:0")
 fields = ("seq_off", "seq", "read_chain_off", "chain_seed_off", "chain_rid", "chain_frac_rep", "seeds")
-out = {"fixture": "c2_refseed", "batches": []}
+out = {"fixture": "c2_refseed", "ungapped_right": eng.ungapped_right() if hasattr(eng.lib, "bwagpu_ctx_ungapped_right") else None,
+       "batches": []}
 for k, rb in enumerate(rbs[:nb]):
     b = rb.batch
     t = {f: torch.from_numpy(np.ascontiguousarray(getattr(b, f)).view(np.uint8).copy()).to(dev) for f in fields}
@@ -33,11 +34,21 @@
     torch.cuda.synchronize()
     ctr = np.zeros(12, np.int64)
     assert eng.lib.bwagpu_debug_spec_ungapped(eng.ctx, C.c_void_p(st.cuda_stream), ctr.ctypes.data_as(C.c_void_p)) == 0
+    late = eng.ungapped_right_counters(st.cuda_stream) if hasattr(eng.lib, "bwagpu_debug_spec_ungapped_right") else None
+    sh = np.zeros(9, np.int64)
+    assert eng.lib.bwagpu_debug_spec_short(eng.ctx, C.c_void_p(st.cuda_stream), sh.ctypes.data_as(C.c_void_p)) == 0
     ok = rb.check(regs.cpu().numpy().view(abi.ALNREG_DTYPE)[:b.n_seeds], nn.cpu().numpy()[:b.n_reads])
     rounds = {}
     for r, name in enumerate("AB"):
         settled, bases, left, right = (int(x) for x in ctr[4 * r:4 * r + 4])
         rounds[name] = {"settled_sides": settled, "settled_bases": bases, "listed_left": left, "listed_right": right,
                         "settled_share_of_sides": round(settled / max(settled + left + right, 1), 4)}
-    out["batches"].append({"batch": k, "reads": b.n_reads, "regions_match_reference": bool(ok), "rounds": rounds})
+        ll, llong, rl, rlong = (int(x) for x in sh[1 + 4 * r:5 + 4 * r])
+        rounds[name].update({"left_short_run": ll - llong, "right_short_run": rl - rlong})
+        if late is not None:
+            ln, lb = int(late[r, 0]), int(late[r, 1])
+            rounds[name].update({"late_settled_right": ln, "late_settled_bases": lb,
+                                 "late_share_of_right_sides_needing_a_left_dp": round(ln / max(ln + right, 1), 4),
+                                 "late_share_of_side_calls": round(ln / max(ln + left + right, 1), 4)})
+    out["batches"].append({"batch": k, "reads": b.n_reads, "sides_run_sixteen_per_wave": int(sh[0]), "regions_match_reference": bool(ok), "rounds": rounds})
 print(json.dumps(out))
```

After: 71.76, median of 6. 1.03x the previous value.
